# frankyeh/UNet-Studio

Hardware: AMD Instinct MI355X
Metric: voxels/sec 3D U-Net train step @128^3 bf16 (higher is better)
Workload: dtype bf16

## Files before the change

### include/unet_hip.h

```cpp
#ifndef UNET_HIP_H
#define UNET_HIP_H
#include <stddef.h>
#include <stdint.h>

#ifdef __cplusplus
extern "C" {
#endif

#define UNET_DTYPE_F32 0
#define UNET_DTYPE_BF16 1

#define UNET_IMPL_AUTO 0
#define UNET_IMPL_DIRECT 1

typedef struct unet_plan unet_plan;

const char* unet_last_error(void);
void unet_set_error(const char* msg);

int unet_init(int* n_devices);
int unet_device_info(int device, char* name, size_t name_len, size_t* total_mem, int* compute_units, int* gcn_arch_is_gfx950);

int unet_plan_create(const char* arch_dsl, int in_c, int out_c, int D, int H, int W, int dtype, int device, int impl,
                     unet_plan** out);
void unet_plan_destroy(unet_plan* plan);

int unet_plan_param_count(const unet_plan* plan, int* n);
int unet_plan_param_shape(const unet_plan* plan, int i, int64_t dims[5], int* ndim);
int unet_plan_param_name(const unet_plan* plan, int i, char* name, size_t name_len);
int unet_plan_param_decay(const unet_plan* plan, int i, int* decay);
int unet_plan_param_fan_in(const unet_plan* plan, int i, int64_t* fan_in, int* is_norm_weight);
int unet_plan_buffer_count(const unet_plan* plan, int* n);
int unet_plan_buffer_shape(const unet_plan* plan, int i, int64_t* numel);
int unet_plan_output_count(const unet_plan* plan, int* n);
int unet_plan_output_shape(const unet_plan* plan, int level, int64_t dims[5]);
int unet_plan_workspace_bytes(const unet_plan* plan, size_t* bytes);
int unet_plan_flops(const unet_plan* plan, double* fwd, double* bwd);
size_t unet_plan_describe(const unet_plan* plan, char* buf, size_t len);

int unet_plan_op_count(const unet_plan* plan, int* n);
int unet_plan_op_info(const unet_plan* plan, int i, int* kind, int* cin, int* cout, int* ks, int* stride, int64_t in_dims[3],
                      int64_t out_dims[3], char* name, size_t name_len);

#define UNET_PROF_CONV_FWD 0
#define UNET_PROF_DGRAD 1
#define UNET_PROF_WGRAD 2
#define UNET_PROF_NORM_FWD 3
#define UNET_PROF_NORM_BWD 4
#define UNET_PROF_OTHER 5
int unet_profile_begin(void);
int unet_profile_end(int max_records, int* op_index, int* category, float* ms, int* n_records);

#define UNET_MODE_PACKS_CURRENT 2
int unet_forward(const unet_plan* plan, const float* const* params, float* const* buffers, const float* x,
                 float* const* outs, void* workspace, int mode, void* stream);

int unet_backward(const unet_plan* plan, const float* const* params, const float* const* grad_outs,
                  float* const* grad_params, float* grad_x, void* workspace, void* stream);

int unet_plan_backward_buckets(const unet_plan* plan, int max_buckets, int* n_buckets, int* op_lo, int64_t* elem_lo);
int unet_backward_part(const unet_plan* plan, const float* const* params, const float* const* grad_outs, float* const* grad_params,
                       float* grad_x, void* workspace, int op_hi, int op_lo, void* stream);

int unet_loss_scratch_bytes(const unet_plan* plan, size_t* bytes);
int unet_loss(const unet_plan* plan, const float* const* outs, const int64_t* target, int cost_mask, int collapse_before,
              float* const* grad_outs, float* losses_out, void* scratch, void* stream);

int unet_forward_loss(const unet_plan* plan, const float* const* params, float* const* buffers, const float* x, float* const* outs,
                      const int64_t* target, int cost_mask, int collapse_before, float* const* grad_outs, float* losses_out,
                      void* loss_scratch, void* workspace, void* stream);
int unet_forward_loss_mode(const unet_plan* plan, const float* const* params, float* const* buffers, const float* x, float* const* outs,
                           const int64_t* target, int cost_mask, int collapse_before, float* const* grad_outs, float* losses_out,
                           void* loss_scratch, void* workspace, int mode, void* stream);

int unet_stream_create_cu_range(int device, int cu_first, int cu_count, void** stream);
int unet_stream_destroy(void* stream);
int unet_plan_side_cu_range(unet_plan* plan, int cu_first, int cu_count);

int unet_pack_filters(const unet_plan* plan, const float* const* params, void* workspace, int with_dgrad, int* made, void* stream);

#define UNET_SUM_MAX_BUFFERS 64
int unet_sum_buffers(const float* const* bufs, int n, float* out, int64_t count, int zero_inputs, void* stream);

int unet_sgd_step(const unet_plan* plan, float* params_flat, float* grads_flat, float* momentum_flat, float lr,
                  float momentum, int nesterov, float weight_decay, float clip_norm, float grad_scale, float* norm_out,
                  void* scratch, void* stream);

int unet_sgd_step_packed(const unet_plan* plan, float* params_flat, float* grads_flat, float* momentum_flat, float lr,
                         float momentum, int nesterov, float weight_decay, float clip_norm, float grad_scale, float* norm_out,
                         void* workspace, int with_dgrad, int* made, void* scratch, void* stream);

int unet_op_scratch_bytes(int cin, int cout, int D, int H, int W, size_t* bytes);
int unet_op_conv_choice(int dtype, int impl, int cin, int cout, int D, int H, int W, int ks, int stride, int transposed, int out[3]);
int unet_op_conv3d_fwd(int dtype, int impl, const void* x, const float* w, const float* b, void* y, int cin, int cout, int D,
                       int H, int W, int ks, int stride, void* scratch, void* stream);
int unet_op_conv3d_fwd_fused(int dtype, int impl, const void* x, const float* scale, const float* shift, int act, const float* w,
                             const float* b, void* y, float* stats, int cin, int cout, int D, int H, int W, int ks, int stride,
                             void* scratch, void* stream);
int unet_op_conv3d_pack(int dtype, const float* w, void* wpacked, int cin, int cout, int D, int H, int W, int ks, int stride,
                        void* stream);
int unet_op_conv3d_fwd_packed(int dtype, const void* x, const void* wpacked, const float* b, void* y, float* stats_partials,
                              int cin, int cout, int D, int H, int W, int ks, int stride, void* stream);
int unet_op_conv3d_bwd_data(int dtype, int impl, const void* dy, const float* w, void* dx, int cin, int cout, int D, int H,
                            int W, int ks, int stride, void* scratch, void* stream);
int unet_op_conv3d_fwd_norm(const void* x0, const void* x1, int cin0, int cin1, const float* w, const float* b, const float* gamma,
                            const float* beta, double eps, float* rm, float* rv, double momentum, int use_running, int act, void* y,
                            void* y_act, float* stat, int cout, int D, int H, int W, int stride, void* scratch, void* stream);
int unet_op_conv3d_bwd_data_norm(int transposed, const void* dy, const float* w, void* dx, int accumulate, const void* u, const float* stat,
                                 const float* gamma, int act, float* coef, float* dgamma, float* dbeta, int cin, int cout, int D, int H,
                                 int W, void* scratch, void* stream);
int unet_op_conv3d_bwd_weight(int dtype, int impl, const void* x, const void* dy, float* dw, float* db, int cin, int cout,
                              int D, int H, int W, int ks, int stride, void* scratch, void* stream);
int unet_op_convt_fwd(int dtype, int impl, const void* x, const float* w, const float* b, void* y, int cin, int cout, int D,
                      int H, int W, void* scratch, void* stream);
int unet_op_convt_bwd_data(int dtype, int impl, const void* dy, const float* w, void* dx, int cin, int cout, int D, int H,
                           int W, void* scratch, void* stream);
int unet_op_convt_bwd_weight(int dtype, int impl, const void* x, const void* dy, float* dw, float* db, int cin, int cout,
                             int D, int H, int W, void* scratch, void* stream);
int unet_op_pack_ndhwc(int dtype, const float* x_ncdhw, void* y_ndhwc, int C, int64_t S, void* stream);
int unet_op_unpack_ncdhw(int dtype, const void* x_ndhwc, float* y_ncdhw, int C, int64_t S, void* stream);

#define UNET_COMM_ID_BYTES 128
typedef struct unet_comm unet_comm;
int unet_comm_unique_id(void* id_bytes );
int unet_comm_create(int rank, int world, const void* id_bytes, int device, unet_comm** out);
int unet_comm_create_all(int n, const int* devices, unet_comm** out );
int unet_comm_destroy(unet_comm* comm);
int unet_comm_rank(const unet_comm* comm, int* rank, int* world);
int unet_allreduce_grads(unet_comm* comm, float* flat, int64_t elem_lo, int64_t elem_hi, void* stream);
int unet_allreduce_grads_all(unet_comm* const* comms, int n, float* const* flats, int64_t elem_lo, int64_t elem_hi, void* const* streams);
int unet_comm_broadcast(unet_comm* comm, float* buf, int64_t n, int root, void* stream);
int unet_comm_join(unet_comm* comm, void* stream);

#ifdef __cplusplus
}
#endif
#endif
```

### unet-studio_amd/csrc/conv_select.h

```cpp
#pragma once
#include "kernels.h"

namespace unet {

enum class Fwd : unsigned char { deep, mfma, head, first_mfma, first_f32_mfma, f32_mfma, direct };
enum class Dgrad : unsigned char { mfma, f32_mfma, direct };
enum class Wgrad : unsigned char { first_mfma, mfma, f32_mfma, small, direct };

struct ConvChoice {
    Fwd fwd = Fwd::direct;
    Dgrad dgrad = Dgrad::direct;
    Wgrad wgrad = Wgrad::direct;
    bool mfma_fwd() const { return fwd == Fwd::deep || fwd == Fwd::mfma; }
};

inline ConvChoice choose_conv(int dtype, int impl, const ConvGeom& g, const SrcDesc* src, int nsrc, bool is_head, bool transposed) {
    ConvChoice c;
    if (impl != UNET_IMPL_AUTO) return c;
    if (transposed) {
        if (mfma_convt_supported(dtype, g, src, nsrc)) c.fwd = Fwd::mfma, c.dgrad = Dgrad::mfma;
        else if (convt_f32_mfma_supported(dtype, g, src, nsrc)) c.fwd = Fwd::f32_mfma;
        if (mfma_convt_wgrad_supported(dtype, g, src, nsrc)) c.wgrad = Wgrad::mfma;
        return c;
    }
    if (is_head) { if (head_supported(g, nsrc)) c.fwd = Fwd::head; }
    else if (mfma_conv_fwd_supported(dtype, g, src, nsrc))
        c.fwd = deep_conv_applies(dtype, (int64_t)g.Do * g.Ho * g.Wo, g.Cin, g.Cout) ? Fwd::deep : Fwd::mfma;
    else if (conv_first_mfma_supported(dtype, g, src, nsrc)) c.fwd = Fwd::first_mfma;
    else if (conv_first_f32_mfma_supported(dtype, g, src, nsrc)) c.fwd = Fwd::first_f32_mfma;
    else if (conv_f32_mfma_supported(dtype, g, src, nsrc)) c.fwd = Fwd::f32_mfma;

    DstGrad dst[2];
    for (int k = 0; k < nsrc; ++k) dst[k].C = src[k].C;
    if (!is_head && mfma_conv_dgrad_supported(dtype, g, src, nsrc)) c.dgrad = Dgrad::mfma;
    else if (conv_f32_mfma_dgrad_supported(dtype, g, dst, nsrc)) c.dgrad = Dgrad::f32_mfma;

    if (conv_first_wgrad_mfma_supported(dtype, g, src, nsrc)) c.wgrad = Wgrad::first_mfma;
    else if (mfma_wgrad_supported(dtype, g, src, nsrc)) c.wgrad = Wgrad::mfma;
    else if (wgrad_f32_mfma_supported(dtype, g, src, nsrc)) c.wgrad = Wgrad::f32_mfma;
    else if (wgrad_small_supported(g, nsrc)) c.wgrad = Wgrad::small;
    return c;
}

}
```

### unet-studio_amd/csrc/engine.cpp

```cpp
#include <hip/hip_runtime.h>

#include <algorithm>
#include <atomic>
#include <cmath>
#include <cstdio>
#include <cstring>
#include <functional>
#include <stdexcept>
#include <string>
#include <mutex>
#include <random>
#include <unordered_map>
#include <vector>

#include "../../include/unet_hip.h"
#include "conv_select.h"
#include "graph.hpp"
#include "kernels.h"

using namespace unet;

namespace {

thread_local std::string g_err;
// ... 153 lines not shown
                if (op.src[k] != (int)t) continue;
                if (conv[i].fwd != Fwd::head) return false;
                ++readers;
            }
        }
        return readers > 0;
    }
    void layout() {
        choose_polite();
        conv.assign(g.ops.size(), ConvChoice());
        for (size_t i = 0; i < g.ops.size(); ++i) {
            const Op& op = g.ops[i];
            if (op.kind != OP_CONV && op.kind != OP_CONVT) continue;
            SrcDesc sd[2];
            src_chans(op, sd);
            conv[i] = choose_conv(dtype, impl, op_geom_of(op), sd, op.nsrc, op.out_level >= 0, op.kind == OP_CONVT);
        }
        size_t off = 0;
        auto take = [&](size_t bytes) { size_t o = off; off = align_up(off + bytes); return o; };
        t_off.assign(g.tensors.size(), SIZE_MAX);
        g_off.assign(g.tensors.size(), SIZE_MAX);
        n_consumers.assign(g.tensors.size(), 0);
        first_consumer.assign(g.tensors.size(), -1);
        for (size_t oi = 0; oi < g.ops.size(); ++oi) {
            const Op& op = g.ops[oi];
            for (int k = 0; k < op.nsrc && op.kind != OP_NORM; ++k)
                if (op.src[k] >= 0) { ++n_consumers[op.src[k]]; if (first_consumer[op.src[k]] < 0) first_consumer[op.src[k]] = (int)oi; }
        }
        a_off.assign(g.tensors.size(), SIZE_MAX);
        for (size_t i = 0; i < g.tensors.size(); ++i) {
            t_off[i] = take((size_t)g.tensors[i].numel() * elsize);
            if (g.tensors[i].needs_grad) g_off[i] = take((size_t)g.tensors[i].numel() * elsize);
            if (impl == UNET_IMPL_AUTO && (g.tensors[i].norm >= 0 || g.tensors[i].act != ACT_NONE) && !head_only(i))
                a_off[i] = take((size_t)g.tensors[i].numel() * elsize);
        }
        n_stat.resize(g.norms.size()); n_coef.resize(g.norms.size());
        size_t pmax = 0;
        for (size_t i = 0; i < g.norms.size(); ++i) {
            n_stat[i] = take(4 * (size_t)g.norms[i].C * 4);
            n_coef[i] = take(3 * (size_t)g.norms[i].C * 4);
            size_t pb = (size_t)stats_blocks(g.tensors[g.norms[i].tensor].voxels()) * g.norms[i].C * 2 * (dtype == UNET_DTYPE_F32 ? 8 : 4);
            if (pb > pmax) pmax = pb;
        }
        w_fwd.assign(g.ops.size(), SIZE_MAX); w_dgrad.assign(g.ops.size(), SIZE_MAX);
        wm_fwd.assign(g.ops.size(), SIZE_MAX); wm_dgrad.assign(g.ops.size(), SIZE_MAX);
        auto grow = [](size_t& m, size_t b) { if (b > m) m = b; };
        for (size_t i = 0; i < g.ops.size(); ++i) {
            const Op& op = g.ops[i];
            if (op.kind != OP_CONV && op.kind != OP_CONVT) continue;
            const ConvChoice& c = conv[i];
            const ConvGeom cg = op_geom_of(op);
            int k3 = op.kind == OP_CONV ? op.ks * op.ks * op.ks : 8;
            w_fwd[i] = take((size_t)k3 * op.cin * round_up(op.cout, 8) * 4);
            w_dgrad[i] = take((size_t)k3 * op.cout * round_up(op.cin, 8) * 4);
            if (op.kind == OP_CONVT) {
                if (c.mfma_fwd()) { wm_fwd[i] = take(mfma_convt_w_bytes(cg)); wm_dgrad[i] = take(mfma_convt_dgrad_w_bytes(cg)); }
                continue;
            }
            const bool stats = g.tensors[op.dst].norm >= 0;
            SrcDesc sd[2];
            src_chans(op, sd);
            if (c.mfma_fwd()) {
                wm_fwd[i] = take(mfma_conv_w_bytes(cg));
                if (stats) grow(pmax, (size_t)mfma_conv_blocks(cg) * op.cout * 2 * 4);
            }
            if (c.fwd == Fwd::first_f32_mfma && stats) grow(pmax, (size_t)conv_first_f32_mfma_blocks(cg) * op.cout * 2 * 8);
            if (c.fwd == Fwd::f32_mfma && stats) grow(pmax, (size_t)conv_f32_mfma_stat_rows(cg, sd) * op.cout * 2 * 8);
            if (c.dgrad == Dgrad::mfma) {
                wm_dgrad[i] = take(mfma_conv_dgrad_w_bytes(cg));
                if (op.stride == 2) grow(pmax, (size_t)s2_conv_dgrad_rows_max() * op.cin * 2 * 4);
            }
        }
        partial_bytes = pmax ? pmax : 256;
        partial_off = take(partial_bytes);
        size_t wmax = 0, hmax = 0;
        for (size_t i = 0; i < g.ops.size(); ++i) {
            const Op& op = g.ops[i];
            if (op.kind != OP_CONV && op.kind != OP_CONVT) continue;
            const ConvChoice& c = conv[i];
            const ConvGeom cg = op_geom_of(op);
            grow(wmax, wgrad_direct_scratch_bytes(cg, op.kind == OP_CONVT));
            if (op.kind == OP_CONVT) {
                if (c.wgrad == Wgrad::mfma) {
                    grow(wmax, mfma_convt_wgrad_scratch_bytes(cg));
                    grow(wmax, bias_grad_scratch_bytes(cg.Cout, (int64_t)cg.Do * cg.Ho * cg.Wo));
                }
                continue;
            }
            if (c.wgrad == Wgrad::mfma) grow(wmax, mfma_wgrad_scratch_bytes(cg, side_polite[i]));
            if (c.wgrad == Wgrad::f32_mfma) grow(wmax, wgrad_f32_mfma_scratch_bytes(cg));
            if (wgrad_small_supported(cg, op.nsrc)) grow(wmax, wgrad_small_scratch_bytes(cg));
            if (cg.Cin == 1 && (cg.Cout == 16 || cg.Cout == 32)) grow(wmax, conv_first_wgrad_mfma_scratch_bytes(cg));
            if (head_supported(cg, op.nsrc)) grow(hmax, head_bwd_scratch_bytes(cg));
        }
        wgrad_off = take(wmax ? wmax : 256);
        head_off = take(hmax ? hmax : 256);
        if (dtype == UNET_DTYPE_BF16 && impl == UNET_IMPL_AUTO) {
            deep_part_bytes = (size_t)8 << 20;
            deep_part_off = take(deep_part_bytes);
            deep_cnt_off = take((size_t)deep_ncnt * 4);
        }
        head_op_off.assign(g.ops.size(), SIZE_MAX);
        for (size_t i = 0; i < g.ops.size(); ++i)
            if (conv[i].fwd == Fwd::head) head_op_off[i] = take(head_bwd_scratch_bytes(op_geom_of(g.ops[i])));
        wz_off.assign(g.ops.size(), SIZE_MAX);
        for (size_t i = 0; i < g.ops.size(); ++i) {
            const Op& op = g.ops[i];
            const Wgrad w = conv[i].wgrad;
            if (op.out_level >= 0 || (w != Wgrad::first_mfma && w != Wgrad::mfma)) continue;
            const ConvGeom cg = op_geom_of(op);
            if (w == Wgrad::first_mfma) wz_off[i] = take(conv_first_wgrad_mfma_scratch_bytes(cg));
            else if (op.kind == OP_CONV) { if (!mfma_conv_wgrad_direct(cg)) wz_off[i] = take(mfma_wgrad_scratch_bytes(cg, side_polite[i])); }
            else if (!mfma_convt_wgrad_direct(cg)) wz_off[i] = take(mfma_convt_wgrad_scratch_bytes(cg));
        }
        ws_bytes = off;
        p_off.assign(g.params.size() + 1, 0);
        for (size_t i = 0; i < g.params.size(); ++i) {
            int64_t n = 1;
            for (auto d : g.params[i].shape) n *= d;
            p_off[i + 1] = p_off[i] + n;
        }
        wz_jobs.clear();
        wz_job_of_op.assign(g.ops.size(), -1);
        int wz_blk = 0;
        for (size_t i = 0; i < g.ops.size(); ++i) {
            if (wz_off[i] == SIZE_MAX) continue;
            const Op& op = g.ops[i];
            ConvGeom cg = op_geom_of(op);
            WgradReduceJob j;
            j.op = (int)i;
            j.slab_off = (long long)(wz_off[i] / 4);
            j.dw_off = p_off[op.weight];
            j.Cb = op.cout;
            if (op.kind == OP_CONVT) {
                j.nsplit = mfma_convt_wgrad_splits(cg);
                j.n = (long long)8 * op.cin * op.cout;
                j.bias_off = op.bias >= 0 ? j.slab_off + (long long)j.nsplit * j.n : -1;
                j.db_off = op.bias >= 0 ? p_off[op.bias] : -1;
            } else {
                j.nsplit = conv[i].wgrad == Wgrad::first_mfma ? conv_first_wgrad_splits(cg) : mfma_conv_wgrad_splits(cg, side_polite[i]);
                j.n = (long long)27 * op.cin * op.cout;
                j.bias_off = op.bias >= 0 ? j.slab_off + (long long)j.nsplit * j.n : -1;
                j.db_off = op.bias >= 0 ? p_off[op.bias] : -1;
            }
            wz_blk += wgrad_reduce_job_blocks(j, wz_blk);
            wz_job_of_op[i] = (int)wz_jobs.size();
            wz_jobs.push_back(j);
        }
        pack_jobs.clear();
        pack_blocks = 0;
        pack_split_op = -1; pack_split_blocks = 0; pack_fwd_blocks = 0;
        for (int which = 0; which < 2; ++which) {
            for (size_t i = 0; i < g.ops.size(); ++i) {
                const Op& op = g.ops[i];
                if (!conv[i].mfma_fwd()) continue;
                if (which == 0 && pack_split_op < 0 && g.tensors[op.dst].voxels() <= (int64_t)16 * 16 * 16) { pack_split_op = (int)i; pack_split_blocks = pack_blocks; }
                PackJob jb[2];
                int n = op.kind == OP_CONV ? mfma_conv_pack_jobs(op_geom_of(op), conv[i].dgrad == Dgrad::mfma, jb) : mfma_convt_pack_jobs(op_geom_of(op), jb);
                if (which >= n) continue;
                jb[which].src_off = p_off[op.weight];
                jb[which].dst_off = (int64_t)(which == 0 ? wm_fwd[i] : wm_dgrad[i]);
                jb[which].blk0 = pack_blocks;
                pack_blocks += jb[which].total;
                pack_jobs.push_back(jb[which]);
            }
            if (which == 0) pack_fwd_blocks = pack_blocks;
        }
        build_sgd_tiles();
    }

    void build_sgd_tiles() {
        sgd_tiles.clear();
        if (pack_jobs.empty()) return;
        const size_t np = g.params.size();
        std::vector<int> jf(np, -1), jd(np, -1), d0(np, 0), d1(np, 0), taps(np, 0);
        {
            size_t j = 0;
            for (int which = 0; which < 2; ++which)
                for (size_t i = 0; i < g.ops.size(); ++i) {
                    const Op& op = g.ops[i];
                    if (!conv[i].mfma_fwd()) continue;
                    const bool convt = op.kind != OP_CONV;
                    if (which >= (convt ? 2 : (conv[i].dgrad == Dgrad::mfma ? 2 : 1))) continue;
                    const ConvGeom cg = op_geom_of(op);
                    int& slot = which == 0 ? jf[op.weight] : jd[op.weight];
                    if (j >= pack_jobs.size() || pack_jobs[j].src_off != p_off[op.weight] || slot >= 0) return;
                    slot = (int)j++;
                    d0[op.weight] = convt ? cg.Cin : cg.Cout; d1[op.weight] = convt ? cg.Cout : cg.Cin; taps[op.weight] = convt ? 8 : 27;
                }
            if (j != pack_jobs.size()) return;
        }
        std::vector<int64_t> units(pack_jobs.size(), 0);
        bool ok = true;
        for (size_t i = 0; i < np && ok; ++i) {
            SgdTile t{};
            t.wd = g.params[i].decay ? 1.f : 0.f;
            t.job_fwd = jf[i]; t.job_dgrad = jd[i];
            const int64_t n = p_off[i + 1] - p_off[i];
            if (jf[i] < 0) {
                if (jd[i] >= 0) { ok = false; break; }
                constexpr int64_t chunk = 8192;
                for (int64_t o = 0; o < n; o += chunk) { t.off = p_off[i] + o; t.count = std::min(chunk, n - o); sgd_tiles.push_back(t); }
                continue;
            }
            if ((int64_t)d0[i] * d1[i] * taps[i] != n) { ok = false; break; }
            t.off = p_off[i]; t.D1 = d1[i]; t.T = taps[i];
            for (int a = 0; a < d0[i] && ok; a += SGD_TILE_MAX)
                for (int b = 0; b < d1[i] && ok; b += SGD_TILE_MAX) {
                    t.d0 = a; t.n0 = std::min(SGD_TILE_MAX, d0[i] - a); t.d1 = b; t.n1 = std::min(SGD_TILE_MAX, d1[i] - b);
                    t.count = (int64_t)t.n0 * t.n1 * t.T;
                    for (int j : {jf[i], jd[i]}) {
                        if (j < 0) continue;
                        const int64_t u = sgd_tile_units(t, pack_jobs[j]);
                        if (u < 0) ok = false; else units[j] += u;
                    }
                    sgd_tiles.push_back(t);
                }
        }
// ... 662 lines not shown

int unet_backward(const unet_plan* p, const float* const* params, const float* const* grad_outs, float* const* grad_params,
                  float* grad_x, void* workspace, void* stream) {
    try {
        if (!p || !params || !grad_params || !workspace) throw std::runtime_error("unet_backward: null argument");
        if (grad_x) throw std::runtime_error("unet_backward: grad_x must be NULL -- dL/dx is not computed (the input carries no gradient, as in train.cpp:619-628)");
        DeviceGuard dg(p->device);
        Exec ex(*p, workspace, stream);
        ex.backward(params, grad_outs, grad_params, grad_x);
        check_launch();
        return 0;
    } catch (const std::exception& e) { return fail(e.what()); }
}

int unet_backward_part(const unet_plan* p, const float* const* params, const float* const* grad_outs, float* const* grad_params,
                       float* grad_x, void* workspace, int op_hi, int op_lo, void* stream) {
    try {
        if (!p || !params || !grad_params || !workspace) throw std::runtime_error("unet_backward_part: null argument");
        if (op_lo < 0 || op_hi < op_lo) throw std::runtime_error("unet_backward_part: invalid op range");
        if (grad_x) throw std::runtime_error("unet_backward_part: grad_x must be NULL -- dL/dx is not computed");
        DeviceGuard dg(p->device);
        Exec ex(*p, workspace, stream);
        ex.backward(params, grad_outs, grad_params, grad_x, op_hi, op_lo);
        check_launch();
        return 0;
    } catch (const std::exception& e) { return fail(e.what()); }
}

int unet_plan_backward_buckets(const unet_plan* p, int max_buckets, int* n_buckets, int* op_lo, int64_t* elem_lo) {
    try {
        if (!p || !n_buckets || !op_lo || !elem_lo || max_buckets < 1) throw std::runtime_error("unet_plan_backward_buckets: bad argument");
        const Graph& g = p->g;
        const int nops = (int)g.ops.size();
        std::vector<int64_t> first(nops, INT64_MAX);
        bool monotone = true;
        int64_t prev = -1;
        for (int i = 0; i < nops; ++i) {
            const Op& op = g.ops[i];
            if (op.kind != OP_CONV && op.kind != OP_CONVT) continue;
            int64_t f = p->p_off[op.weight];
            if (op.bias >= 0 && p->p_off[op.bias] < f) f = p->p_off[op.bias];
            first[i] = f;
            if (f <= prev) monotone = false;
            prev = f;
            const Tensor& T = g.tensors[op.dst];
            if (T.norm >= 0) {
                const Norm& n = g.norms[T.norm];
                if (p->p_off[n.gamma] < f || p->p_off[n.beta] < f) monotone = false;
            }
        }
        int nb = 0;
        if (monotone && max_buckets > 1) {
            const double thr = (double)p->n_param_elems / ((double)max_buckets - 0.5);
            int64_t hi = p->n_param_elems;
            for (int i = nops - 1; i > 0 && nb < max_buckets - 1; --i) {
                if (first[i] == INT64_MAX) continue;
                if ((double)(hi - first[i]) >= thr) { op_lo[nb] = i; elem_lo[nb] = first[i]; hi = first[i]; ++nb; }
            }
        }
        op_lo[nb] = 0; elem_lo[nb] = 0; ++nb;
        *n_buckets = nb;
        return 0;
    } catch (const std::exception& e) { return fail(e.what()); }
}

int unet_plan_op_count(const unet_plan* p, int* n) { *n = (int)p->g.ops.size(); return 0; }
int unet_plan_op_info(const unet_plan* p, int i, int* kind, int* cin, int* cout, int* ks, int* stride, int64_t in_dims[3],
                      int64_t out_dims[3], char* name, size_t name_len) {
    if (i < 0 || i >= (int)p->g.ops.size()) return fail("op index out of range");
    const Op& op = p->g.ops[i];
    if (kind) *kind = (int)op.kind;
    if (cin) *cin = op.cin;
    if (cout) *cout = op.cout;
    if (ks) *ks = op.ks;
    if (stride) *stride = op.stride;
    const Tensor* a = op.nsrc > 0 && op.src[0] >= 0 ? &p->g.tensors[op.src[0]] : nullptr;
    const Tensor* o = op.dst >= 0 ? &p->g.tensors[op.dst] : nullptr;
    if (in_dims) { in_dims[0] = a ? a->D : 0; in_dims[1] = a ? a->H : 0; in_dims[2] = a ? a->W : 0; }
    if (out_dims) { out_dims[0] = o ? o->D : 0; out_dims[1] = o ? o->H : 0; out_dims[2] = o ? o->W : 0; }
    if (name && name_len) { std::strncpy(name, op.name.c_str(), name_len - 1); name[name_len - 1] = 0; }
    return 0;
}

int unet_profile_begin(void) {
    if (g_prof) return fail("unet_profile_begin: a profile is already open on this thread");
    g_prof = new ProfSink();
    return 0;
}
int unet_profile_end(int max_records, int* op_index, int* category, float* ms, int* n_records) {
    if (!g_prof) return fail("unet_profile_end: no open profile on this thread");
    ProfSink* ps = g_prof;
    g_prof = nullptr;
    int n = 0, rc = 0;
    for (auto& r : ps->recs) {
        float t = 0.f;
        hipError_t e = hipEventSynchronize(r.e1);
        if (e == hipSuccess) e = hipEventElapsedTime(&t, r.e0, r.e1);
        if (e != hipSuccess) rc = fail(std::string("unet_profile_end: ") + hipGetErrorString(e));
        if (r.op != -2 && n < max_records && op_index && category && ms) { op_index[n] = r.op; category[n] = r.cat; ms[n] = t; ++n; }
        (void)hipEventDestroy(r.e0); (void)hipEventDestroy(r.e1);
    }
    if (n_records) *n_records = n;
    delete ps;
    return rc;
}

int unet_loss_scratch_bytes(const unet_plan* p, size_t* bytes) { *bytes = p->loss_bytes; return 0; }

namespace {
struct LossRun {
    const unet_plan* p;
    const float* const* outs; const int64_t* target; float* const* grad_outs; float* losses_out;
    int C, oc, collapse, cost_mask;
    float inv;
    std::vector<int64_t*> tgt;
    std::vector<float*> lvl;
    float* partial[2];
    LossRun(const unet_plan* plan, const float* const* outs_, const int64_t* target_, int cost_mask_, int collapse_before, float* const* grad_outs_,
            float* losses_out_, void* scratch)
        : p(plan), outs(outs_), target(target_), grad_outs(grad_outs_), losses_out(losses_out_), collapse(collapse_before), cost_mask(cost_mask_) {
        if (!p || !outs || !target || !losses_out || !scratch) throw std::runtime_error("unet_loss: null argument");
        const Graph& g = p->g;
        C = g.out_c;
        if (collapse_before < 0 || collapse_before >= C) throw std::runtime_error("invalid collapse_before");
        oc = collapse_before ? C - collapse_before + 1 : C;
        const size_t nl = g.outputs.size();
        float wsum = 0.f;
        for (size_t k = 0; k < nl; ++k) wsum += 1.0f / (float)(1 << k);
        inv = 1.0f / wsum;
        char* sc = (char*)scratch;
        size_t off = 0;
        tgt.resize(nl); lvl.resize(nl);
        for (size_t l = 0; l < nl; ++l) {
            int64_t S = (int64_t)(g.D >> l) * (g.H >> l) * (g.W >> l);
            if (S <= 0) S = 1;
            tgt[l] = (int64_t*)(sc + off); off = align_up(off + (size_t)S * 8);
            lvl[l] = (float*)(sc + off); off = align_up(off + (size_t)(4 + 2 * C) * 4);
        }
        partial[0] = (float*)(sc + off); off = align_up(off + (size_t)1024 * (3 + 2 * C) * 4);
        partial[1] = (float*)(sc + off);
        int D = g.D, H = g.H, W = g.W;
        for (size_t k = 0; k < nl; ++k) {
            if (k > 0) {
                if ((D >> 1) <= 0 || (H >> 1) <= 0 || (W >> 1) <= 0) throw std::runtime_error("deep supervision target size became zero");
                D >>= 1; H >>= 1; W >>= 1;
            }
            const auto& o = g.outputs[k];
            if (o.C == 0 || !outs[k]) throw std::runtime_error("undefined deep supervision output at level " + std::to_string(k));
            if (o.C != C)
                throw std::runtime_error("output channel mismatch at level " + std::to_string(k) + ": tensor has " + std::to_string(o.C) +
                                         ", out_count is " + std::to_string(C));
            if (o.D != D || o.H != H || o.W != W) throw std::runtime_error("deep supervision output/target size mismatch at level " + std::to_string(k));
        }
    }
    size_t levels() const { return p->g.outputs.size(); }
    const int64_t* target_of(size_t k) const { return k == 0 ? target : tgt[k]; }
    int64_t voxels(size_t k) const { const auto& o = p->g.outputs[k]; return (int64_t)o.D * o.H * o.W; }
    void prepare(hipStream_t s) {
        HIP_OK(hipMemsetAsync(losses_out, 0, 4 * sizeof(float), s));
        const Graph& g = p->g;
        int D = g.D, H = g.H, W = g.W;
        for (size_t k = 1; k < levels(); ++k) {
            launch_target_half(target_of(k - 1), tgt[k], D, H, W, s);
            D >>= 1; H >>= 1; W >>= 1;
        }
    }
// ... 136 lines not shown
        if (!bufs || !out || n < 1 || n > UNET_SUM_MAX_BUFFERS || count < 0) throw std::runtime_error("unet_sum_buffers: bad argument");
        for (int k = 0; k < n; ++k)
            if (!bufs[k] || (reinterpret_cast<uintptr_t>(bufs[k]) & 15)) throw std::runtime_error("unet_sum_buffers: null or misaligned buffer");
        if (reinterpret_cast<uintptr_t>(out) & 15) throw std::runtime_error("unet_sum_buffers: misaligned output");
        if (count == 0) return 0;
        launch_sum_buffers(bufs, n, out, count, zero_inputs, (hipStream_t)stream);
        check_launch();
        return 0;
    } catch (const std::exception& e) { return fail(e.what()); }
}

int unet_sgd_step(const unet_plan* p, float* params, float* grads, float* mom, float lr, float momentum, int nesterov, float wd,
                  float clip_norm, float grad_scale, float* norm_out, void* scratch, void* stream) {
    try {
        if (!p || !params || !grads || !mom || !scratch) throw std::runtime_error("unet_sgd_step: null argument");
        if (!p->segs_dev) throw std::runtime_error("unet_sgd_step: plan was created without a device");
        DeviceGuard dg(p->device);
        hipStream_t s = (hipStream_t)stream;
        const int nblk = 1024;
        float* partial = (float*)scratch;
        launch_sumsq_partial(grads, p->n_param_elems, grad_scale, partial, nblk, s);
        launch_sgd(params, grads, mom, p->n_param_elems, p->segs_dev, p->nseg, partial, nblk, lr, momentum, nesterov, wd, clip_norm,
                   grad_scale, norm_out, s);
        check_launch();
        return 0;
    } catch (const std::exception& e) { return fail(e.what()); }
}

int unet_sgd_step_packed(const unet_plan* p, float* params, float* grads, float* mom, float lr, float momentum, int nesterov, float wd,
                         float clip_norm, float grad_scale, float* norm_out, void* workspace, int with_dgrad, int* made, void* scratch,
                         void* stream) {
    try {
        if (!p || !params || !grads || !mom || !scratch || !made) throw std::runtime_error("unet_sgd_step_packed: null argument");
        *made = 0;
        if (!p->tiles_dev || !p->jobs_dev || !workspace)
            return unet_sgd_step(p, params, grads, mom, lr, momentum, nesterov, wd, clip_norm, grad_scale, norm_out, scratch, stream);
        if ((reinterpret_cast<uintptr_t>(params) | reinterpret_cast<uintptr_t>(grads) | reinterpret_cast<uintptr_t>(mom)) & 15)
            throw std::runtime_error("unet_sgd_step_packed: misaligned buffer");
        DeviceGuard dg(p->device);
        hipStream_t s = (hipStream_t)stream;
        const int nblk = 1024;
        float* partial = (float*)scratch;
        launch_sumsq_partial(grads, p->n_param_elems, grad_scale, partial, nblk, s);
        launch_sgd_pack(params, grads, mom, p->tiles_dev, (int)p->sgd_tiles.size(), p->jobs_dev, workspace, with_dgrad,
                        p->deep_part_bytes ? (int*)((char*)workspace + p->deep_cnt_off) : nullptr, p->deep_ncnt, partial, nblk, lr, momentum,
                        nesterov, wd, clip_norm, grad_scale, norm_out, s);
        check_launch();
        *made = 1;
        return 0;
    } catch (const std::exception& e) { return fail(e.what()); }
}

struct OpScratch {
    size_t half, pack, partials;
    OpScratch(int cin, int cout)
        : half(align_up((size_t)27 * round_up(cin, 8) * round_up(cout, 8) * 4)), pack(2 * half),
          partials(pack + align_up((size_t)160 * round_up(cin, 32) * round_up(cout, 32))) {}
};
int unet_op_scratch_bytes(int cin, int cout, int D, int H, int W, size_t* bytes) {
    size_t b = OpScratch(cin, cout).partials + 4096;
    if (D > 0 && H > 0 && W > 0) {
        int64_t S = (int64_t)D * H * W;
        size_t blocks = (size_t)(S / 32 + 4096);
        b += align_up(blocks * cout * 2 * 8);
    }
    if ((int64_t)cin * cout <= 1024) {
        size_t w = ((size_t)1024 * 1024 + (size_t)1024 * cout) * 4 + 1024;
        if (w > b) b = w;
    }
    if (cout <= 8 || cin == 1) {
        size_t w = (size_t)512 * ((size_t)27 * cin * cout + cout) * 4 + 1024;
        if (w > b) b = w;
    }
    if (cin % 16 == 0 && cout % 16 == 0 && D > 0 && H > 0 && W > 0) {
        ConvGeom g;
        g.Cin = cin; g.Cout = cout; g.D = g.Do = D; g.H = g.Ho = H; g.W = g.Wo = W; g.ks = 3; g.stride = 1;
        b = std::max(b, wgrad_f32_mfma_scratch_bytes(g));
        size_t w = std::max(mfma_wgrad_scratch_bytes(g, 0), mfma_wgrad_scratch_bytes(g, 1));
        if (w > b) b = w;
        g.stride = 2; g.Do = (D - 1) / 2 + 1; g.Ho = (H - 1) / 2 + 1; g.Wo = (W - 1) / 2 + 1;
        w = std::max(mfma_wgrad_scratch_bytes(g, 0), mfma_wgrad_scratch_bytes(g, 1));
        if (w > b) b = w;
        g.Do = 2 * D; g.Ho = 2 * H; g.Wo = 2 * W;
        w = mfma_convt_wgrad_scratch_bytes(g);
        if (w > b) b = w;
    }
    *bytes = b;
    return 0;
}

static ConvGeom op_geom(int cin, int cout, int D, int H, int W, int ks, int stride, bool transposed) {
    ConvGeom g;
    g.Cin = cin; g.Cout = cout; g.D = D; g.H = H; g.W = W; g.ks = ks; g.stride = stride;
    if (transposed) { g.Do = 2 * D; g.Ho = 2 * H; g.Wo = 2 * W; }
    else {
        int pad = (ks - 1) / 2;
        g.Do = (D + 2 * pad - ks) / stride + 1; g.Ho = (H + 2 * pad - ks) / stride + 1; g.Wo = (W + 2 * pad - ks) / stride + 1;
    }
    return g;
}
static void op_pack(const float* w, int cin, int cout, int k3, bool transposed, void* scratch, float** wf, float** wd, hipStream_t s) {
    *wf = (float*)scratch; *wd = (float*)((char*)scratch + OpScratch(cin, cout).half);
    if (transposed) launch_pack_convt_w(w, *wf, *wd, cin, cout, s);
    else launch_pack_conv_w(w, *wf, *wd, cin, cout, k3, s);
}
#define OP_TRY(...) try { __VA_ARGS__; check_launch(); return 0; } catch (const std::exception& e) { return fail(e.what()); }
static DeepScratch op_deep() {
    static std::mutex mu;
    static std::unordered_map<int, DeepScratch> per_dev;
    int dev = 0;
    HIP_OK(hipGetDevice(&dev));
    std::lock_guard<std::mutex> lk(mu);
    auto it = per_dev.find(dev);
    if (it != per_dev.end()) return it->second;
    DeepScratch d;
    d.part_bytes = (size_t)8 << 20; d.ncnt = 4096;
    char* base = nullptr;
    HIP_OK(hipMalloc((void**)&base, d.part_bytes + (size_t)d.ncnt * 4));
    HIP_OK(hipMemset(base + d.part_bytes, 0, (size_t)d.ncnt * 4));
    d.part = (float*)base; d.cnt = (int*)(base + d.part_bytes);
    per_dev[dev] = d;
    return d;
}

int unet_op_conv_choice(int dtype, int impl, int cin, int cout, int D, int H, int W, int ks, int stride, int transposed, int out[3]) {
    try {
        if (!out) throw std::runtime_error("unet_op_conv_choice: null output");
        if (cin < 1 || cout < 1 || D < 1 || H < 1 || W < 1) throw std::runtime_error("unet_op_conv_choice: sizes must be positive");
        const ConvGeom g = transposed ? op_geom(cin, cout, D, H, W, 2, 2, true) : op_geom(cin, cout, D, H, W, ks, stride, false);
        SrcDesc sd; sd.C = cin;
        const ConvChoice c = choose_conv(dtype, impl, g, &sd, 1, false, transposed != 0);
        out[0] = (int)c.fwd; out[1] = (int)c.dgrad; out[2] = (int)c.wgrad;
        return 0;
    } catch (const std::exception& e) { return fail(e.what()); }
}

int unet_op_conv3d_fwd(int dtype, int impl, const void* x, const float* w, const float* b, void* y, int cin, int cout, int D, int H,
                       int W, int ks, int stride, void* scratch, void* stream) {
    OP_TRY({
        hipStream_t s = (hipStream_t)stream;
        ConvGeom g = op_geom(cin, cout, D, H, W, ks, stride, false);
        float *wf, *wd;
        SrcDesc sd; sd.ptr = x; sd.C = cin;
        const ConvChoice c = choose_conv(dtype, impl, g, &sd, 1, false, false);
        if (c.mfma_fwd()) {
            void* wm = (char*)scratch + OpScratch(cin, cout).pack;
            launch_mfma_pack_conv_w(w, wm, nullptr, g, s);
            if (!launch_deep_conv_fwd(g, &sd, 1, wm, b, y, nullptr, op_deep(), s)) launch_mfma_conv_fwd(g, &sd, 1, wm, b, y, nullptr, s);
        } else if (c.fwd == Fwd::first_mfma) {
            launch_conv_first_mfma(g, &sd, w, b, y, nullptr, s);
        } else if (c.fwd == Fwd::first_f32_mfma) {
            (void)launch_conv_first_f32_mfma(g, &sd, w, b, (float*)y, nullptr, s);
        } else {
            op_pack(w, cin, cout, ks * ks * ks, false, scratch, &wf, &wd, s);
            if (c.fwd == Fwd::f32_mfma) (void)launch_conv_f32_mfma(g, &sd, 1, wf, b, (float*)y, s);
            else launch_conv_fwd_direct(dtype, g, &sd, 1, wf, b, y, nullptr, s);
        }
    })
}
int unet_op_conv3d_fwd_fused(int dtype, int impl, const void* x, const float* scale, const float* shift, int act, const float* w,
                             const float* b, void* y, float* stats, int cin, int cout, int D, int H, int W, int ks, int stride,
                             void* scratch, void* stream) {
    OP_TRY({
        hipStream_t s = (hipStream_t)stream;
        ConvGeom g = op_geom(cin, cout, D, H, W, ks, stride, false);
        float *wf, *wd;
        SrcDesc sd; sd.ptr = x; sd.C = cin; sd.scale = scale; sd.shift = shift; sd.act = act;
// ... 44 lines not shown
        launch_mfma_conv_fwd(g, &sd, 1, wpacked, b, y, stats_partials, (hipStream_t)stream);
    })
}
int unet_op_conv3d_bwd_data(int dtype, int impl, const void* dy, const float* w, void* dx, int cin, int cout, int D, int H, int W,
                            int ks, int stride, void* scratch, void* stream) {
    OP_TRY({
        hipStream_t s = (hipStream_t)stream;
        ConvGeom g = op_geom(cin, cout, D, H, W, ks, stride, false);
        float *wf, *wd;
        DstGrad d; d.ptr = dx; d.C = cin; d.accumulate = 0;
        SrcDesc sd; sd.C = cin;
        const Dgrad c = choose_conv(dtype, impl, g, &sd, 1, false, false).dgrad;
        if (c == Dgrad::mfma) {
            void* wm = (char*)scratch + OpScratch(cin, cout).pack;
            launch_mfma_pack_conv_w(w, nullptr, wm, g, s);
            mfma_dgrad(g, false, dy, wm, &d, 1, nullptr, nullptr, op_deep(), s);
        } else {
            op_pack(w, cin, cout, ks * ks * ks, false, scratch, &wf, &wd, s);
            if (c == Dgrad::f32_mfma) launch_conv_f32_mfma_dgrad(g, (const float*)dy, wd, &d, 1, s);
            else launch_conv_dgrad_direct(dtype, g, dy, wd, &d, 1, s);
        }
    })
}
int unet_op_conv3d_fwd_norm(const void* x0, const void* x1, int cin0, int cin1, const float* w, const float* b, const float* gamma,
                            const float* beta, double eps, float* rm, float* rv, double momentum, int use_running, int act, void* y,
                            void* y_act, float* stat, int cout, int D, int H, int W, int stride, void* scratch, void* stream) {
    OP_TRY({
        hipStream_t s = (hipStream_t)stream;
        const int cin = cin0 + cin1, nsrc = x1 ? 2 : 1;
        ConvGeom g = op_geom(cin, cout, D, H, W, 3, stride, false);
        SrcDesc sd[2];
        sd[0].ptr = x0; sd[0].C = cin0;
        if (x1) { sd[1].ptr = x1; sd[1].C = cin1; }
        const ConvChoice c = choose_conv(UNET_DTYPE_BF16, UNET_IMPL_AUTO, g, sd, nsrc, false, false);
        if (!c.mfma_fwd() || (use_running && (!rm || !rv)))
            throw std::runtime_error("unet_op_conv3d_fwd_norm: shape not covered by the MFMA kernels, or eval mode without running statistics");
        const OpScratch L(cin, cout);
        void* wm = (char*)scratch + L.pack;
        float* part = (float*)((char*)scratch + L.partials);
        launch_mfma_pack_conv_w(w, wm, nullptr, g, s);
        const DeepNormFwd nf = {gamma, beta, eps, stat, rm, rv, momentum, use_running ? 1 : 0, act, y_act};
        if (!(c.fwd == Fwd::deep && launch_deep_conv_fwd(g, sd, nsrc, wm, b, y, &nf, op_deep(), s))) {
            const int rows = launch_mfma_conv_fwd(g, sd, nsrc, wm, b, y, use_running ? nullptr : part, s);
            norm_fwd_passes(UNET_DTYPE_BF16, y, cout, (int64_t)g.Do * g.Ho * g.Wo, part, rows, false, use_running != 0, gamma, beta, eps,
                            stat, rm, rv, act, y_act, s);
        }
    })
}
int unet_op_conv3d_bwd_data_norm(int transposed, const void* dy, const float* w, void* dx, int accumulate, const void* u, const float* stat,
                                 const float* gamma, int act, float* coef, float* dgamma, float* dbeta, int cin, int cout, int D, int H,
                                 int W, void* scratch, void* stream) {
    OP_TRY({
        hipStream_t s = (hipStream_t)stream;
        ConvGeom g = op_geom(cin, cout, D, H, W, transposed ? 2 : 3, transposed ? 2 : 1, transposed != 0);
        SrcDesc sd; sd.C = cin;
        if (choose_conv(UNET_DTYPE_BF16, UNET_IMPL_AUTO, g, &sd, 1, false, transposed != 0).dgrad != Dgrad::mfma)
            throw std::runtime_error("unet_op_conv3d_bwd_data_norm: shape not covered by the MFMA kernels");
        const OpScratch L(cin, cout);
        void* wm = (char*)scratch + L.pack;
        float* part = (float*)((char*)scratch + L.partials);
        DstGrad d; d.ptr = dx; d.C = cin; d.accumulate = accumulate ? 1 : 0;
        const DeepNormBwd nb = {u, stat, gamma, coef, dgamma, dbeta, act};
        if (transposed) launch_mfma_pack_convt_w(w, nullptr, wm, g, s);
        else launch_mfma_pack_conv_w(w, nullptr, wm, g, s);
        const DgradOutcome o = mfma_dgrad(g, transposed != 0, dy, wm, &d, 1, &nb, part, op_deep(), s);
        if (!o.norm_done) norm_bwd_passes(UNET_DTYPE_BF16, dx, u, cin, (int64_t)D * H * W, stat, act, gamma, coef, dgamma, dbeta, part, o.rows, false, s);
    })
}
int unet_op_conv3d_bwd_weight(int dtype, int impl, const void* x, const void* dy, float* dw, float* db, int cin, int cout, int D,
                              int H, int W, int ks, int stride, void* scratch, void* stream) {
    OP_TRY({
        hipStream_t s = (hipStream_t)stream;
        ConvGeom g = op_geom(cin, cout, D, H, W, ks, stride, false);
        SrcDesc sd; sd.ptr = x; sd.C = cin;
        switch (choose_conv(dtype, impl, g, &sd, 1, false, false).wgrad) {
            case Wgrad::first_mfma: launch_conv_first_wgrad_mfma(g, &sd, dy, dw, db, scratch, s); break;
            case Wgrad::mfma: launch_mfma_conv_wgrad(g, &sd, 1, dy, dw, db, scratch, s, false, env().op_polite ? 1 : 0); break;
            case Wgrad::f32_mfma: launch_wgrad_f32_mfma(g, &sd, 1, (const float*)dy, dw, db, scratch, s); break;
            case Wgrad::small: launch_conv_wgrad_small(dtype, g, &sd, 1, dy, dw, db, scratch, s); break;
            case Wgrad::direct: launch_conv_wgrad_direct(dtype, g, &sd, 1, dy, dw, db, nullptr, s);
        }
    })
}
int unet_op_convt_fwd(int dtype, int impl, const void* x, const float* w, const float* b, void* y, int cin, int cout, int D, int H,
                      int W, void* scratch, void* stream) {
    OP_TRY({
        hipStream_t s = (hipStream_t)stream;
        ConvGeom g = op_geom(cin, cout, D, H, W, 2, 2, true);
        float *wf, *wd;
        SrcDesc sd; sd.ptr = x; sd.C = cin;
        const Fwd f = choose_conv(dtype, impl, g, &sd, 1, false, true).fwd;
        if (f == Fwd::mfma) {
            void* wm = (char*)scratch + OpScratch(cin, cout).pack;
            launch_mfma_pack_convt_w(w, wm, nullptr, g, s);
            if (!launch_deep_convt_fwd(g, &sd, 1, wm, b, y, op_deep(), s)) launch_mfma_convt_fwd(g, &sd, 1, wm, b, y, s);
        } else {
            op_pack(w, cin, cout, 8, true, scratch, &wf, &wd, s);
            if (f == Fwd::f32_mfma) launch_convt_f32_mfma(g, &sd, wf, b, (float*)y, s);
            else launch_convt_fwd_direct(dtype, g, &sd, 1, wf, b, y, s);
        }
    })
}
int unet_op_convt_bwd_data(int dtype, int impl, const void* dy, const float* w, void* dx, int cin, int cout, int D, int H, int W,
                           void* scratch, void* stream) {
    OP_TRY({
        hipStream_t s = (hipStream_t)stream;
        ConvGeom g = op_geom(cin, cout, D, H, W, 2, 2, true);
        float *wf, *wd;
        DstGrad d; d.ptr = dx; d.C = cin; d.accumulate = 0;
        SrcDesc sd; sd.C = cin;
        if (choose_conv(dtype, impl, g, &sd, 1, false, true).dgrad == Dgrad::mfma) {
            void* wm = (char*)scratch + OpScratch(cin, cout).pack;
            launch_mfma_pack_convt_w(w, nullptr, wm, g, s);
            mfma_dgrad(g, true, dy, wm, &d, 1, nullptr, nullptr, op_deep(), s);
        } else {
            op_pack(w, cin, cout, 8, true, scratch, &wf, &wd, s);
            launch_convt_dgrad_direct(dtype, g, dy, wd, &d, 1, s);
        }
    })
}
int unet_op_convt_bwd_weight(int dtype, int impl, const void* x, const void* dy, float* dw, float* db, int cin, int cout, int D, int H,
                             int W, void* scratch, void* stream) {
    OP_TRY({
        ConvGeom g = op_geom(cin, cout, D, H, W, 2, 2, true);
        SrcDesc sd; sd.ptr = x; sd.C = cin;
        if (choose_conv(dtype, impl, g, &sd, 1, false, true).wgrad == Wgrad::mfma)
            launch_mfma_convt_wgrad(g, &sd, dy, dw, scratch, (hipStream_t)stream, false, db);
        else
            launch_convt_wgrad_direct(dtype, g, &sd, 1, dy, dw, db, nullptr, (hipStream_t)stream);
    })
}
int unet_op_pack_ndhwc(int dtype, const float* x, void* y, int C, int64_t S, void* stream) {
    OP_TRY({ launch_pack_input(dtype, x, y, C, S, (hipStream_t)stream); })
}
int unet_op_unpack_ncdhw(int dtype, const void* x, float* y, int C, int64_t S, void* stream) {
    OP_TRY({ launch_unpack_ncdhw(dtype, x, y, C, S, (hipStream_t)stream); })
}


static const char* augment_recipe_error(const UnetAugmentRecipe* r) {
    if (!r) return "unet_augment: null recipe";
    for (int d = 0; d < 3; ++d)
        if (r->dims[d] < 1) return "unet_augment: dims must be positive";
    if (r->channels < 1 || r->channels > UNET_AUG_MAX_CHANNELS) return "unet_augment: channels out of range (1..UNET_AUG_MAX_CHANNELS)";
    if (r->n_foci < 0 || r->n_foci > UNET_AUG_MAX_FOCI) return "unet_augment: n_foci out of range (0..UNET_AUG_MAX_FOCI)";
    if (r->trunc_top < 0 || r->trunc_bottom < 0) return "unet_augment: negative truncation";
    if (r->downsample)
        for (int d = 0; d < 3; ++d)
            if (r->low_dims[d] < 1 || r->low_dims[d] > r->dims[d]) return "unet_augment: low_dims must be in 1..dims";
    for (int k = 0; k < r->n_foci; ++k)
        if (!(r->foci_radius[k] > 0.f)) return "unet_augment: distortion radius must be positive";
    return nullptr;
}
int unet_augment_scratch_bytes(const UnetAugmentRecipe* recipe, size_t* bytes) {
    if (const char* e = augment_recipe_error(recipe)) return fail(e);
    if (!bytes) return fail("unet_augment_scratch_bytes: null output");
    *bytes = augment_scratch_bytes(*recipe);
    return 0;
}
int unet_augment_run(const UnetAugmentRecipe* recipe, float* image, float* label, void* scratch, size_t scratch_bytes, void* stream) {
    if (const char* e = augment_recipe_error(recipe)) return fail(e);
    if (!image || !label || !scratch) return fail("unet_augment_run: null device pointer");
    if (scratch_bytes < augment_scratch_bytes(*recipe)) return fail("unet_augment_run: scratch too small (see unet_augment_scratch_bytes)");
    OP_TRY({
        hipPointerAttribute_t at;
        HIP_OK(hipPointerGetAttributes(&at, image));
        DeviceGuard guard(at.device);
        launch_augment(*recipe, image, label, scratch, (hipStream_t)stream);
    })
}

static const char* simulate_recipe_error(const UnetSimulateRecipe* r) {
    if (!r) return "unet_simulate_modality: null recipe";
    for (int d = 0; d < 3; ++d)
        if (r->dims[d] < 1) return "unet_simulate_modality: dims must be positive";
    if (r->with_label && (r->max_label < 0 || r->max_label >= UNET_SIM_MAX_LABELS)) return "unet_simulate_modality: max_label out of range";
    for (int k = 0; k < UNET_SIM_TERMS; ++k)
        if (r->term_a[k] > 3 || r->term_b[k] > 3 || r->term_c[k] > 3 || r->term_d[k] > 3) return "unet_simulate_modality: exponents must be 0..3";
    return nullptr;
}
int unet_simulate_modality_scratch_bytes(const UnetSimulateRecipe* recipe, size_t* bytes) {
    if (const char* e = simulate_recipe_error(recipe)) return fail(e);
    if (!bytes) return fail("unet_simulate_modality_scratch_bytes: null output");
    *bytes = simulate_scratch_bytes(*recipe);
    return 0;
}
int unet_simulate_modality_run(const UnetSimulateRecipe* recipe, float* t1w, const float* label, void* scratch, size_t scratch_bytes,
                               void* stream) {
    if (const char* e = simulate_recipe_error(recipe)) return fail(e);
    if (!t1w || !scratch || (recipe->with_label && !label)) return fail("unet_simulate_modality_run: null device pointer");
    if (scratch_bytes < simulate_scratch_bytes(*recipe)) return fail("unet_simulate_modality_run: scratch too small");
    OP_TRY({
        hipPointerAttribute_t at;
        HIP_OK(hipPointerGetAttributes(&at, t1w));
        DeviceGuard guard(at.device);
        launch_simulate_modality(*recipe, t1w, label, scratch, (hipStream_t)stream);
    })
}

static const char* qc_args_error(int out_c, int64_t voxels, int collapse_before) {
    if (out_c < 1) return "unet_qc: out_c must be positive";
    if (collapse_before < 0 || collapse_before >= out_c) return "invalid collapse_before";
    if (voxels <= 0) return "unet_qc: voxels must be positive";
    if (voxels > ((int64_t)1 << 40)) return "unet_qc: too many voxels";
    return nullptr;
}
int unet_qc_scratch_bytes(int out_c, int64_t voxels, int collapse_before, size_t* bytes) {
    if (const char* e = qc_args_error(out_c, voxels, collapse_before)) return fail(e);
    if (!bytes) return fail("unet_qc_scratch_bytes: null output");
    *bytes = qc_scratch_bytes(out_c, voxels, collapse_before);
// ... 983 lines not shown
```

### unet-studio_amd/csrc/kernels.h

```cpp
#pragma once
#include <hip/hip_runtime.h>
#include <cstdint>

#include "../../include/unet_atlas.h"
#include "../../include/unet_augment.h"
#include "../../include/unet_components.h"
#include "../../include/unet_connectivity.h"
#include "../../include/unet_distance.h"
#include "../../include/unet_ensemble.h"
#include "../../include/unet_feed.h"
#include "../../include/unet_hip.h"
#include "../../include/unet_instances.h"
#include "../../include/unet_morph.h"
#include "../../include/unet_postproc.h"
#include "../../include/unet_preproc.h"
#include "../../include/unet_qc.h"
#include "../../include/unet_register.h"
#include "../../include/unet_space.h"
#include "../../include/unet_stats.h"
#include "../../include/unet_table.h"
#include "../../include/unet_mirror.h"
#include "../../include/unet_tiles.h"

namespace unet {
// ... 41 lines not shown
void launch_convt_wgrad_direct(int dtype, const ConvGeom& g, const SrcDesc* src, int nsrc, const void* dy, float* dw, float* db,
                               void* scratch, hipStream_t s);

int stats_blocks(int64_t S);
void launch_stats_partial(int dtype, const void* x, int C, int64_t S, float* partial, hipStream_t s);
void launch_norm_finalize(const float* partial, int nblk, int C, int64_t S, const float* gamma, const float* beta, double eps,
                          float* stat, float* running_mean, float* running_var, double momentum, hipStream_t s, bool dbl = false);
void launch_stats_sum(const float* partial, int nblk, int C, float* out, hipStream_t s, bool dbl = false);
void launch_norm_eval(int C, const float* gamma, const float* beta, const float* rm, const float* rv, double eps, float* stat,
                      hipStream_t s);

void launch_act_bwd(int dtype, void* g, const void* u, int act, int64_t n, hipStream_t s);
void launch_norm_bwd_partial(int dtype, void* g, const void* u, int C, int64_t S, const float* stat, int act, float* partial,
                             hipStream_t s);
void launch_norm_bwd_finalize(const float* partial, int nblk, int C, int64_t S, const float* gamma, const float* stat, float* coef,
                              float* dgamma, float* dbeta, hipStream_t s, bool dbl = false);
bool launch_norm_finalize_apply(int dtype, const float* partial, int nblk, int C, int64_t S, const float* gamma, const float* beta, double eps,
                                float* stat, float* running_mean, float* running_var, double momentum, const void* raw, int act, void* out,
                                hipStream_t s);
bool launch_norm_bwd_finalize_apply(int dtype, const float* partial, int nblk, int C, int64_t S, const float* gamma, const float* stat,
                                    float* coef, float* dgamma, float* dbeta, void* g, const void* u, int act, hipStream_t s);
void launch_norm_bwd_apply(int dtype, void* g, const void* u, int C, int64_t S, const float* stat, const float* coef, int act,
                           hipStream_t s);

void launch_maxpool_fwd(int dtype, SrcDesc src, void* out, int D, int H, int W, hipStream_t s);
void launch_maxpool_bwd(int dtype, SrcDesc src, const void* gout, DstGrad dst, int D, int H, int W, hipStream_t s);
void launch_upsample_fwd(int dtype, SrcDesc src, void* out, int D, int H, int W, hipStream_t s);
void launch_upsample_bwd(int dtype, const void* gout, DstGrad dst, int D, int H, int W, hipStream_t s);
void launch_materialize(int dtype, const SrcDesc* src, int nsrc, void* out, int64_t S, hipStream_t s);
void launch_apply_view(int dtype, SrcDesc src, void* out, int64_t S, hipStream_t s);
void launch_materialize_bwd(int dtype, const void* gout, const DstGrad* dst, int ndst, int64_t S, hipStream_t s);
void launch_export_bwd(int dtype, const float* g_ncdhw, DstGrad dst, int64_t S, hipStream_t s);
void launch_unpack_ncdhw(int dtype, const void* g, float* out_ncdhw, int C, int64_t S, hipStream_t s);

void launch_target_half(const int64_t* t, int64_t* o, int D, int H, int W, hipStream_t s);
int loss_blocks(int64_t S);
void launch_loss_partial(const float* logits, const int64_t* target, int C, int64_t S, int collapse, float* partial, hipStream_t s);
void launch_loss_finalize(const float* partial, int nblk, int oc, float level_weight, int cost_mask, float* level_out, float* totals,
                          int set_stats, hipStream_t s);
void launch_loss_grad(const float* logits, const int64_t* target, int C, int64_t S, int collapse, const float* level_out,
                      float level_weight, int cost_mask, float* dlogits, hipStream_t s);

void launch_sum_buffers(const float* const* bufs, int n, float* out, int64_t count, int zero_inputs, hipStream_t s);

struct SgdSeg { int64_t offset, count; float wd; };
void launch_sumsq_partial(const float* g, int64_t n, float scale, float* partial, int nblk, hipStream_t s);
void launch_sgd(float* p, float* g, float* m, int64_t n, const SgdSeg* segs_dev, int nseg, const float* partial, int nblk,
                float lr, float momentum, int nesterov, float weight_decay, float clip_norm, float grad_scale, float* norm_out,
                hipStream_t s);

struct PackJob;
struct SgdTile { int64_t off, count; float wd; int job_fwd, job_dgrad, D1, T, d0, n0, d1, n1, pad; };
constexpr int SGD_TILE_MAX = 32;
int64_t sgd_tile_units(const SgdTile& t, const PackJob& job);
void launch_sgd_pack(float* p, float* g, float* m, const SgdTile* tiles_dev, int ntiles, const PackJob* jobs_dev, void* ws, int with_dgrad,
                     int* zero, int nzero, const float* partial, int nblk, float lr, float momentum, int nesterov, float weight_decay,
                     float clip_norm, float grad_scale, float* norm_out, hipStream_t s);

struct PackJob { int64_t src_off, dst_off, total, blk0; int Ci, Co, CK, T, mode, A, B, pad; };
enum PackMode {
    PK_CONV_FWD = 0,
    PK_CONV_DGRAD = 1,
    PK_CONVT_DGRAD = 2,
    PK_CONVT_FWD = 3,
    PK_CONV_S2_DGRAD = 4
};
int mfma_conv_pack_jobs(const ConvGeom& g, bool want_dgrad, PackJob* out2);
int mfma_convt_pack_jobs(const ConvGeom& g, PackJob* out2);
void launch_mfma_pack_batched(const float* params_base, void* ws, const PackJob* jobs_dev, int njobs, int64_t nblocks, hipStream_t s,
                              int64_t blk_base = 0, int max_grid = 0, int* zero = nullptr, int nzero = 0);
bool mfma_conv_fwd_supported(int dtype, const ConvGeom& g, const SrcDesc* src, int nsrc);
size_t mfma_conv_w_bytes(const ConvGeom& g);
void launch_mfma_pack_conv_w(const float* w, void* w_mfma_fwd, void* w_mfma_dgrad, const ConvGeom& g, hipStream_t s);
int launch_mfma_conv_fwd(const ConvGeom& g, const SrcDesc* src, int nsrc, const void* w_mfma, const float* bias, void* out,
                         float* stats_partial, hipStream_t s);
bool conv_first_mfma_supported(int dtype, const ConvGeom& g, const SrcDesc* src, int nsrc);
int conv_first_mfma_blocks(const ConvGeom& g);
int launch_conv_first_mfma(const ConvGeom& g, const SrcDesc* src, const float* w, const float* bias, void* out, float* stats_partial,
                           hipStream_t s);
int mfma_conv_blocks(const ConvGeom& g);
bool mfma_wgrad_z_supported(int dtype, const ConvGeom& g, const SrcDesc* src, int nsrc);
size_t mfma_wgrad_z_scratch_bytes(const ConvGeom& g, int polite = 0);
int mfma_wgrad_z_splits(const ConvGeom& g, int polite = 0);
int launch_mfma_wgrad_z(const ConvGeom& g, const SrcDesc* src, int nsrc, const void* dy, bool want_bias, void* scratch, hipStream_t s,
                        int polite = 0);
void wgrad_reduce(const float* slab, const float* bias_slab, int nsplit, int64_t n, int Cb, float* dw, float* db, hipStream_t s);
struct WgradReduceJob { long long slab_off, bias_off, dw_off, db_off, n; int nsplit, Cb, ly, blk0, nblk, op; };
int wgrad_reduce_job_blocks(WgradReduceJob& j, int blk0);
void launch_wgrad_reduce_batched(const WgradReduceJob* jobs_dev, int job0, int njobs, int blk_base, int nblocks, const void* ws, float* gflat,
                                 hipStream_t s);
bool mfma_wgrad_supported(int dtype, const ConvGeom& g, const SrcDesc* src, int nsrc);
size_t mfma_wgrad_scratch_bytes(const ConvGeom& g, int polite = 0);
int mfma_conv_wgrad_splits(const ConvGeom& g, int polite = 0);
int mfma_convt_wgrad_splits(const ConvGeom& g);
bool mfma_conv_wgrad_direct(const ConvGeom& g);
bool mfma_convt_wgrad_direct(const ConvGeom& g);
int conv_first_wgrad_splits(const ConvGeom& g);
void launch_mfma_conv_wgrad(const ConvGeom& g, const SrcDesc* src, int nsrc, const void* dy, float* dw, float* db, void* scratch,
                            hipStream_t s, bool defer_reduce = false, int polite = 0);
bool head_supported(const ConvGeom& g, int nsrc);
size_t head_bwd_scratch_bytes(const ConvGeom& g);
void launch_head_fwd(int dtype, const ConvGeom& g, const SrcDesc& src, const float* w, const float* bias, void* y, float* out_ncdhw,
                     hipStream_t s);
void launch_head_bwd(int dtype, const ConvGeom& g, const SrcDesc& src, const float* dy_ncdhw, const void* dy_cl, const float* w,
                     DstGrad dst, float* dw, float* db, void* scratch, hipStream_t s, bool defer_reduce = false);
void launch_head_bwd_reduce(const ConvGeom& g, float* dw, float* db, const void* scratch, hipStream_t s);
bool conv_first_wgrad_mfma_supported(int dtype, const ConvGeom& g, const SrcDesc* src, int nsrc);
size_t conv_first_wgrad_mfma_scratch_bytes(const ConvGeom& g);
struct NormBwdFuse { const void* u; const float* stat; const float* coef; int act; };
void launch_conv_first_wgrad_mfma(const ConvGeom& g, const SrcDesc* src, const void* dy, float* dw, float* db, void* scratch, hipStream_t s,
                                  bool defer_reduce = false, const NormBwdFuse* nb_fuse = nullptr);
bool wgrad_small_supported(const ConvGeom& g, int nsrc);
size_t wgrad_small_scratch_bytes(const ConvGeom& g);
void launch_conv_wgrad_small(int dtype, const ConvGeom& g, const SrcDesc* src, int nsrc, const void* dy, float* dw, float* db,
                             void* scratch, hipStream_t s);
bool mfma_convt_wgrad_supported(int dtype, const ConvGeom& g, const SrcDesc* src, int nsrc);
size_t mfma_convt_wgrad_scratch_bytes(const ConvGeom& g);
void launch_mfma_convt_wgrad(const ConvGeom& g, const SrcDesc* src, const void* dy, float* dw, void* scratch, hipStream_t s,
                             bool defer_reduce = false, float* db = nullptr, int polite = 0);
int launch_colsum_partial8(int dtype, const void* x, int C, int64_t S, float* partial, hipStream_t s);
size_t bias_grad_scratch_bytes(int C, int64_t S);
void launch_bias_grad(int dtype, const void* dy, int C, int64_t S, float* db, void* scratch, hipStream_t s);
bool mfma_conv_dgrad_supported(int dtype, const ConvGeom& g, const SrcDesc* src, int nsrc);
size_t mfma_conv_dgrad_w_bytes(const ConvGeom& g);
struct DgradOutcome {
    bool served = false;
    bool norm_done = false;
    int rows = 0;
    bool operator==(const DgradOutcome& o) const { return served == o.served && norm_done == o.norm_done && rows == o.rows; }
};
struct BnBwdStats { const void* u; const float* stat; float* partial; int act, C; };
DgradOutcome mfma_conv_dgrad_outcome(const ConvGeom& g, const DstGrad* dst, int ndst, bool norm);
DgradOutcome launch_mfma_conv_dgrad(const ConvGeom& g, const void* dy, const void* w_mfma_dgrad, const DstGrad* dst, int ndst, hipStream_t s,
                                    const BnBwdStats* bn = nullptr);
int launch_s2_conv_fwd(const ConvGeom& g, const SrcDesc* src, int nsrc, const void* w_mfma, const float* bias, void* out, float* stats_partial,
                       hipStream_t s);
DgradOutcome s2_conv_dgrad_outcome(const ConvGeom& g, const DstGrad* dst, int ndst, bool norm);
DgradOutcome launch_s2_conv_dgrad(const ConvGeom& g, const void* dy, const void* w_s2_dgrad, const DstGrad* dst, int ndst, hipStream_t s,
                                  const BnBwdStats* bn);
int s2_conv_dgrad_rows_max();
bool launch_s2_convt_fwd(const ConvGeom& g, const SrcDesc* src, int nsrc, const void* w_mfma, const float* bias, void* out, hipStream_t s);
bool launch_s2_convt_dgrad(const ConvGeom& g, const void* dy, const void* w_mfma_dgrad, const DstGrad* dst, int ndst, hipStream_t s);
int s2_wgrad_splits(int Ca, int Cb, int cD, int cH, int cW);
int launch_s2_wgrad(int ks, const void* fine, const void* fine2, int C0, int Ca, int fD, int fH, int fW, const void* coarse, int Cb, int cD, int cH,
                    int cW, bool want_bias, int bias_from_a, void* scratch, hipStream_t s, int polite);
constexpr int64_t DEEP_MAX_VOXELS = 512;
struct DeepScratch { float* part = nullptr; size_t part_bytes = 0; int* cnt = nullptr; int ncnt = 0; };
struct DeepNormFwd {
    const float* gamma; const float* beta; double eps; float* stat; float* rm; float* rv; double momentum; int use_running; int act;
    void* act_out;
};
struct DeepNormBwd {
    const void* u; const float* stat; const float* gamma; float* coef; float* dgamma; float* dbeta; int act;
};
bool deep_conv_applies(int dtype, int64_t out_voxels, int cin, int cout);
bool launch_deep_conv_fwd(const ConvGeom& g, const SrcDesc* src, int nsrc, const void* w_mfma, const float* bias, void* out,
                          const DeepNormFwd* nf, const DeepScratch& sc, hipStream_t s);
bool launch_deep_convt_fwd(const ConvGeom& g, const SrcDesc* src, int nsrc, const void* w_mfma, const float* bias, void* out,
                           const DeepScratch& sc, hipStream_t s);
DgradOutcome deep_dgrad_outcome(const ConvGeom& g, bool transposed, const DstGrad* dst, int ndst, bool norm, const DeepScratch& sc);
DgradOutcome launch_deep_dgrad(const ConvGeom& g, bool transposed, const void* dy, const void* w_mfma_dgrad, const DstGrad* dst, int ndst,
                               const DeepNormBwd* nb, const DeepScratch& sc, hipStream_t s);
bool mfma_convt_supported(int dtype, const ConvGeom& g, const SrcDesc* src, int nsrc);
size_t mfma_convt_w_bytes(const ConvGeom& g);
size_t mfma_convt_dgrad_w_bytes(const ConvGeom& g);
void launch_mfma_pack_convt_w(const float* w, void* w_mfma_fwd, void* w_mfma_dgrad, const ConvGeom& g, hipStream_t s);
void launch_mfma_convt_fwd(const ConvGeom& g, const SrcDesc* src, int nsrc, const void* w_mfma, const float* bias, void* out, hipStream_t s);
void launch_mfma_convt_dgrad(const ConvGeom& g, const void* dy, const void* w_mfma_dgrad, const DstGrad* dst, int ndst, hipStream_t s);

bool conv_f32_mfma_supported(int dtype, const ConvGeom& g, const SrcDesc* src, int nsrc);
int conv_f32_mfma_stat_rows(const ConvGeom& g, const SrcDesc* src);
int launch_conv_f32_mfma(const ConvGeom& g, const SrcDesc* src, int nsrc, const float* w_fwd, const float* bias, float* out,
                         hipStream_t s, double* stats_partial = nullptr);
bool conv_first_f32_mfma_supported(int dtype, const ConvGeom& g, const SrcDesc* src, int nsrc);
int conv_first_f32_mfma_blocks(const ConvGeom& g);
int launch_conv_first_f32_mfma(const ConvGeom& g, const SrcDesc* src, const float* w, const float* bias, float* out, double* stats_partial,
                               hipStream_t s);
bool convt_f32_mfma_supported(int dtype, const ConvGeom& g, const SrcDesc* src, int nsrc);
void launch_convt_f32_mfma(const ConvGeom& g, const SrcDesc* src, const float* w_fwd, const float* bias, float* out, hipStream_t s);
bool wgrad_f32_mfma_supported(int dtype, const ConvGeom& g, const SrcDesc* src, int nsrc);
size_t wgrad_f32_mfma_scratch_bytes(const ConvGeom& g);
void launch_wgrad_f32_mfma(const ConvGeom& g, const SrcDesc* src, int nsrc, const float* dy, float* dw, float* db, void* scratch,
                           hipStream_t s);
void slab_reduce_public(const float* slab, int nsplit, int64_t n, float* out, hipStream_t s);
bool conv_f32_mfma_dgrad_supported(int dtype, const ConvGeom& g, const DstGrad* dst, int ndst);
void launch_conv_f32_mfma_dgrad(const ConvGeom& g, const float* dy, const float* w_dgrad, const DstGrad* dst, int ndst, hipStream_t s);

size_t augment_scratch_bytes(const UnetAugmentRecipe& r);
void launch_augment(const UnetAugmentRecipe& r, float* image, float* label, void* scratch, hipStream_t st);
size_t simulate_scratch_bytes(const UnetSimulateRecipe& r);
void launch_simulate_modality(const UnetSimulateRecipe& r, float* t1w, const float* label, void* scratch, hipStream_t st);

size_t qc_scratch_bytes(int out_c, int64_t S, int collapse);
void launch_qc_counts(const float* logits, const float* label, const float* image0, int out_c, int64_t S, int collapse, int shift,
                      uint64_t* counts, void* scratch, hipStream_t s);

size_t feed_scratch_bytes(int64_t S);
void launch_feed_label_max(const float* label, int64_t S, int* out_max, void* scratch, hipStream_t s);
void launch_feed_prepare(const float* image0, float* label, int64_t S, int normalize, int shift, int* label_max, void* scratch,
                         hipStream_t s);
void launch_feed_target(const float* label, int64_t S, int normalize, int64_t* target, void* scratch, hipStream_t s);

size_t postproc_scratch_bytes(int planes, int64_t S);
void launch_postproc_softmax(const float* logits, int C, int64_t S, float thr, float* lp, float* fg, uint16_t* lab, hipStream_t s);
void launch_postproc_argmax_planes(const float* lp, int np, int64_t S, const float* fg, float thr, uint16_t* lab, hipStream_t s);
void launch_postproc_defragment(int W, int H, int D, int each, float thr, double ratio, float* fg, float* lp, int np, uint16_t* lab,
                                void* scratch, hipStream_t s);
void launch_postproc_plane_op(int op, float t, int W, int H, int D, float* lp, int np, void* scratch, hipStream_t s);

int64_t space_bricks(int w, int h, int d);
size_t space_scratch_bytes(int64_t dst_voxels, int channels);
void launch_space_resample(const float* src, int sw, int sh, int sd, float* dst, int dw, int dh, int dd, int channels,
                           const UnetSpaceMap& map, int mode, int normalize, void* scratch, hipStream_t s);
void launch_space_postproc(const float* logits, int C, int mw, int mh, int md, const UnetSpaceMap& map, int nw, int nh, int nd, float thr,
                           float* lp, float* fg, uint16_t* lab, hipStream_t s);

void launch_tiles_blend(const float* tiles, int C, int tw, int th, int td, const UnetTilePlan& plan, int cw, int ch, int cd, float* canvas,
                        hipStream_t s);
void launch_tiles_postproc(const float* tiles, int C, int tw, int th, int td, const UnetTilePlan& plan, int cw, int ch, int cd, float thr,
                           float* lp, float* fg, uint16_t* lab, hipStream_t s);

void launch_mirror_combine(const float* stack, int C, int W, int H, int D, int n_members, const int* masks, int swap_axis, const int* pairs,
                           int n_pairs, float* mean, uint8_t* agreement, hipStream_t s);
void launch_mirror_postproc(const float* stack, int C, int W, int H, int D, int n_members, const int* masks, int swap_axis,
                            const int* pairs, int n_pairs, float thr, float* lp, float* fg, uint16_t* lab, uint8_t* agreement,
                            hipStream_t s);
// ... 87 lines not shown
```

### unet-studio_amd/csrc/kernels_mfma_s2_wgrad.hip

```cpp
#include <cstdio>
#include <cstdlib>
#include <type_traits>

#include "mfma_util.h"

namespace unet {

__device__ __attribute__((aligned(16))) unsigned g_s2w_zero[4] = {0u, 0u, 0u, 0u};

typedef __attribute__((ext_vector_type(4))) short ws16x4;
typedef __attribute__((address_space(3))) ws16x4 wlds_s16x4;
__device__ __forceinline__ bf16x8 wtr_read2(const char* p0, const char* p1) {
    ws16x4 a = __builtin_amdgcn_ds_read_tr16_b64_v4i16((wlds_s16x4*)p0);
    ws16x4 b = __builtin_amdgcn_ds_read_tr16_b64_v4i16((wlds_s16x4*)p1);
    return __builtin_bit_cast(bf16x8, __builtin_shufflevector(a, b, 0, 1, 2, 3, 4, 5, 6, 7));
}

struct S2WgradArgs {
    const void* fine;
    const void* fine2;
    int C0;
    const void* coarse;
    int Ca, Cb;
    int fD, fH, fW, cD, cH, cW;
    float* slab;
    float* bias_slab;
    int bias_from_a;
    int cols_x, cols_y, nseg, zlen;
};

#define S2W_DMA(src, dst)                                                                                                    \
    do {                                                                                                                     \
        unsigned keep_;                                                                                                      \
        asm volatile("s_mov_b32 %0, m0\n\ts_mov_b32 m0, %2\n\ts_nop 0\n\tglobal_load_lds_dwordx4 %1, off\n\ts_mov_b32 m0, %0" \
                     : "=&s"(keep_) : "v"(src), "s"(__builtin_amdgcn_readfirstlane((int)(dst))) : "memory");                      \
    } while (0)

template <int KS, int PA, int PB, int WK>
__global__ void __launch_bounds__(256, 2) k_s2_wgrad(S2WgradArgs a) {
    constexpr int T = KS * KS * KS, PAD = KS == 3 ? 1 : 0, P = PA * PB;
    static_assert(P * WK == 4, "four waves");
    constexpr int R = WK == 1 ? 2 : 1, BYC = WK * R;
    constexpr int HYF = 2 * BYC + PAD, NODD = KS == 3 ? 33 : 32, HXF = NODD + 32;
    constexpr int FVS = PA * 32, CVS = PB * 32;
    constexpr int FSLOT = HYF * HXF * FVS, CSLOT = BYC * 32 * CVS;
    constexpr int NF = KS == 3 ? 5 : 4, NC = 2;
    constexpr int FUNITS = HYF * HXF * PA * 2, CUNITS = BYC * 32 * PB * 2;
    constexpr int ITF = (FUNITS + 255) / 256, ITC = (CUNITS + 255) / 256;
    constexpr int GA = PA * 2, GB = PB * 2;
    constexpr int LDS_BYTES = NF * FSLOT + NC * CSLOT;
    extern __shared__ __attribute__((aligned(16))) char smem[];
    char* const fring = smem;
    char* const cring = smem + NF * FSLOT;

    const int tid = threadIdx.x, lane = tid & 63, il = lane & 15, gq = lane >> 4, q4 = il >> 2, p4 = il & 3;
    const int wave = __builtin_amdgcn_readfirstlane(tid >> 6), pw = wave % P, kw = wave / P, ia = pw / PB, ib = pw % PB;
    const int CBG = (a.Cb / 16) / PB;
    const int caB = ((int)blockIdx.y / CBG) * PA, cbB = ((int)blockIdx.y % CBG) * PB;
    const unsigned lds0 = (unsigned)(size_t)(__attribute__((address_space(3))) char*)smem;

    const int item = xcd_remap((int)blockIdx.x, (int)gridDim.x);
    const int ncols = a.cols_x * a.cols_y, seg = item / ncols, col = item % ncols;
    const int x0 = (col % a.cols_x) * 32, y0 = (col / a.cols_x) * BYC;
    const int zs = seg * a.zlen, ze = zs + a.zlen < a.cD ? zs + a.zlen : a.cD, len = ze - zs;

    f32x4 acc[T];
#pragma unroll
    for (int t = 0; t < T; ++t) acc[t] = f32x4{0.f, 0.f, 0.f, 0.f};
    float bsum[8];
#pragma unroll
    for (int e = 0; e < 8; ++e) bsum[e] = 0.f;
    const bool do_bias_b = a.bias_slab != nullptr && !a.bias_from_a && caB == 0;
    const bool do_bias_a = a.bias_slab != nullptr && a.bias_from_a && cbB == 0;

    unsigned foff[ITF], coff[ITC];
    unsigned fpiece[ITF], cpiece[ITC];
    const int fch = caB * 16 + (tid % GA) * 8;
    const bool f2 = a.fine2 != nullptr && fch >= a.C0;
    const char* const fptr = (const char*)(f2 ? a.fine2 : a.fine);
    const int fC = a.fine2 ? (f2 ? a.Ca - a.C0 : a.C0) : a.Ca, fc0 = f2 ? fch - a.C0 : fch;
#pragma unroll
    for (int it = 0; it < ITF; ++it) {
        const int u = it * 256 + tid, hv = u / GA, hy = hv / HXF, sl = hv % HXF;
        const int t = sl < NODD ? 2 * sl : 2 * (sl - NODD) + 1;
        const int gy = 2 * y0 - PAD + hy, gx = 2 * x0 - PAD + t;
        const bool ok = u < FUNITS && (unsigned)gy < (unsigned)a.fH && (unsigned)gx < (unsigned)a.fW;
// ... 90 lines not shown
            for (int t = 0; t < T; ++t) {
                __builtin_amdgcn_sched_barrier(0);
                acc[t] = __builtin_amdgcn_mfma_f32_16x16x32_bf16(ring[t % RD], Bf, acc[t], 0, 0, 0);
                __builtin_amdgcn_sched_barrier(0);
                if (t + RD < T) ring[t % RD] = afrag(t + RD);
            }
        }
    }
    asm volatile("s_waitcnt vmcnt(0)" ::: "memory");
    __syncthreads();

    constexpr int TCH = (P * T * 1024 <= LDS_BYTES) ? T : ((P * 9 * 1024 <= LDS_BYTES && T % 9 == 0) ? 9 : (T % 3 == 0 ? 3 : 1));
    static_assert(P * TCH * 1024 <= LDS_BYTES && T % TCH == 0, "reduction scratch");
    float* red = (float*)smem;
    if constexpr (WK > 1) {
#pragma unroll 1
        for (int kk = 1; kk < WK; ++kk) {
#pragma unroll
            for (int c0 = 0; c0 < T; c0 += TCH) {
                if (kw == kk) {
#pragma unroll
                    for (int t = 0; t < TCH; ++t) *(f32x4*)(red + ((pw * TCH + t) * 64 + lane) * 4) = acc[c0 + t];
                }
                __syncthreads();
                if (kw == 0) {
#pragma unroll
                    for (int t = 0; t < TCH; ++t) {
                        const f32x4 o = *(const f32x4*)(red + ((pw * TCH + t) * 64 + lane) * 4);
                        acc[c0 + t][0] += o[0]; acc[c0 + t][1] += o[1]; acc[c0 + t][2] += o[2]; acc[c0 + t][3] += o[3];
                    }
                }
                __syncthreads();
            }
        }
    }
    {
        constexpr int RP = 16 * T + 4;
        static_assert(16 * RP * 4 <= LDS_BYTES, "slab staging");
        float* stg = (float*)smem;
#pragma unroll 1
        for (int pr = 0; pr < P; ++pr) {
            __syncthreads();
            if (kw == 0 && pw == pr) {
#pragma unroll
                for (int t = 0; t < T; ++t)
#pragma unroll
                    for (int r = 0; r < 4; ++r) stg[il * RP + (gq * 4 + r) * T + t] = acc[t][r];
            }
            __syncthreads();
            float* base = a.slab + (size_t)blockIdx.x * T * a.Ca * a.Cb + ((size_t)(cbB + pr % PB) * 16 * a.Ca + (size_t)(caB + pr / PB) * 16) * T;
            for (int q = tid; q < 16 * 4 * T; q += 256) {
                const int row = q / (4 * T), c4 = q % (4 * T);
                *(f32x4*)(base + (size_t)row * a.Ca * T + c4 * 4) = *(const f32x4*)(stg + row * RP + c4 * 4);
            }
        }
    }
    if (do_bias_a || do_bias_b) {
        const int G = do_bias_a ? GA : GB;
#pragma unroll
        for (int e = 0; e < 8; ++e) {
            float v = bsum[e];
            for (int m = G; m < 64; m <<= 1) v += __shfl_xor(v, m);
            bsum[e] = v;
        }
        __syncthreads();
        float* bred = (float*)smem;
        if (lane < G) {
#pragma unroll
            for (int e = 0; e < 8; ++e) bred[(wave * G + lane) * 8 + e] = bsum[e];
        }
        __syncthreads();
        if (tid < G * 8) {
            const int u = tid / 8, e = tid % 8;
            float sacc = 0.f;
#pragma unroll
            for (int w = 0; w < 4; ++w) sacc += bred[(w * G + u) * 8 + e];
            const int C = do_bias_a ? a.Ca : a.Cb, tB = do_bias_a ? caB : cbB;
            a.bias_slab[(size_t)blockIdx.x * C + (tB + (u >> 1)) * 16 + (u & 1) * 8 + e] = sacc;
        }
    }
}

struct S2WCfg { int pa, pb, wk, byc, cols_x, cols_y, nseg, zlen, gx, gy; };
static bool s2w_cfg(int Ca, int Cb, int cD, int cH, int cW, S2WCfg& c) {
    if (sliding_window_off() || Ca % 16 || Cb % 16 || cW < 24 || cD < 4) return false;
    if ((size_t)(2 * cH + 1) * (2 * cW + 1) * Ca * 2 >= ((size_t)1 << 31) || (size_t)cH * cW * Cb * 2 >= ((size_t)1 << 31)) return false;
    const int cat = Ca / 16, cbt = Cb / 16;
    if (cat % 2 == 0 && cbt % 2 == 0) { c.pa = 2; c.pb = 2; c.wk = 1; }
    else if (cbt % 2 == 0) { c.pa = 1; c.pb = 2; c.wk = 2; }
    else if (cat % 2 == 0) { c.pa = 2; c.pb = 1; c.wk = 2; }
    else return false;
    c.byc = 2;
    c.cols_x = (cW + 31) / 32; c.cols_y = (cH + c.byc - 1) / c.byc;
    c.gy = (cat / c.pa) * (cbt / c.pb);
    const int cols = c.cols_x * c.cols_y;
    int want = 512 / c.gy;
    if (want < 1) want = 1;
    int nseg = (want + cols - 1) / cols;
    if (nseg < 1) nseg = 1;
    int zlen = (cD + nseg - 1) / nseg;
    if (zlen < 4) zlen = 4;
    if (zlen > cD) zlen = cD;
    c.nseg = (cD + zlen - 1) / zlen; c.zlen = zlen;
    c.gx = cols * c.nseg;
    return true;
}
int s2_wgrad_splits(int Ca, int Cb, int cD, int cH, int cW) {
    S2WCfg c;
    return s2w_cfg(Ca, Cb, cD, cH, cW, c) ? c.gx : 0;
}
template <int KS, int PA, int PB, int WK>
static void launch_s2w_t(const S2WgradArgs& a, const S2WCfg& c, hipStream_t s, int polite) {
    constexpr int PAD = KS == 3 ? 1 : 0, R = WK == 1 ? 2 : 1, BYC = WK * R, HYF = 2 * BYC + PAD, HXF = (KS == 3 ? 33 : 32) + 32;
    constexpr int lds = (KS == 3 ? 5 : 4) * HYF * HXF * PA * 32 + 2 * BYC * 32 * PB * 32;
    static_assert(BYC == 2 && lds <= 160 * 1024, "footprint / LDS");
    static std::atomic<uint64_t> attr_done{0};
    const int want = lds > 83000 ? lds : polite_lds(lds, 1);
    set_max_lds_once(attr_done, (const void*)k_s2_wgrad<KS, PA, PB, WK>, want);
    k_s2_wgrad<KS, PA, PB, WK><<<dim3((unsigned)c.gx, (unsigned)c.gy), 256, polite_lds(lds, polite), s>>>(a);
}
int launch_s2_wgrad(int ks, const void* fine, const void* fine2, int C0, int Ca, int fD, int fH, int fW, const void* coarse, int Cb, int cD, int cH,
                    int cW, bool want_bias, int bias_from_a, void* scratch, hipStream_t s, int polite) {
    S2WCfg c;
    if (!s2w_cfg(Ca, Cb, cD, cH, cW, c)) return 0;
    S2WgradArgs a;
    a.fine = fine; a.fine2 = fine2; a.C0 = C0; a.coarse = coarse; a.Ca = Ca; a.Cb = Cb; a.fD = fD; a.fH = fH; a.fW = fW; a.cD = cD; a.cH = cH; a.cW = cW;
    const int T = ks * ks * ks;
    a.slab = (float*)scratch;
    a.bias_slab = want_bias ? a.slab + (size_t)c.gx * T * Ca * Cb : nullptr;
    a.bias_from_a = bias_from_a;
    a.cols_x = c.cols_x; a.cols_y = c.cols_y; a.nseg = c.nseg; a.zlen = c.zlen;
    if (ks == 3) {
        if (c.pa == 2 && c.pb == 2) launch_s2w_t<3, 2, 2, 1>(a, c, s, polite);
        else if (c.pb == 2) launch_s2w_t<3, 1, 2, 2>(a, c, s, polite);
        else launch_s2w_t<3, 2, 1, 2>(a, c, s, polite);
    } else {
        if (c.pa == 2 && c.pb == 2) launch_s2w_t<2, 2, 2, 1>(a, c, s, polite);
        else if (c.pb == 2) launch_s2w_t<2, 1, 2, 2>(a, c, s, polite);
        else launch_s2w_t<2, 2, 1, 2>(a, c, s, polite);
    }
    return c.gx;
}

}
```

### unet-studio_amd/csrc/kernels_mfma_wgrad.hip

```cpp
#include <type_traits>
#include "mfma_util.h"

namespace unet {

typedef __attribute__((ext_vector_type(4))) short s16x4;
typedef __attribute__((address_space(3))) s16x4 lds_s16x4;

struct MfmaWgradArgs {
    ConvGeom g;
    SrcDesc asrc[2];
    int nasrc;
    SrcDesc bsrc;
    float* slab;
    float* bias_slab;
    int tiles_x, tiles_y, tiles_z;
    int direct;
    int bias_from_a;
};

__device__ __forceinline__ bf16x8 tr_read2(const char* p0, const char* p1) {
    s16x4 a = __builtin_amdgcn_ds_read_tr16_b64_v4i16((lds_s16x4*)p0);
    s16x4 b = __builtin_amdgcn_ds_read_tr16_b64_v4i16((lds_s16x4*)p1);
    return __builtin_bit_cast(bf16x8, __builtin_shufflevector(a, b, 0, 1, 2, 3, 4, 5, 6, 7));
}

template <int S, int KD, int PAD, int BZ, int BY, int BX, int PI, int PJ>
__global__ void __launch_bounds__(256, 2) k_mfma_wgrad(MfmaWgradArgs a) {
    constexpr int HZ = (BZ - 1) * S + KD, HY = (BY - 1) * S + KD, HX = (BX - 1) * S + KD;
    constexpr int NVA = HZ * HY * HX, NVB = BZ * BY * BX, T = KD * KD * KD;
    constexpr int PLANE_A = NVA * 32, PLANE_B = NVB * 32, B_OFF = PI * PLANE_A;
    constexpr int P = PI * PJ, WPP = 4 / P;
    constexpr int GPR = BX / 4;
    constexpr int KSTEPS = NVB / 32;
    static_assert(P == 1 || P == 2 || P == 4, "pairs per block");
    static_assert(NVB % 32 == 0 && BX % 4 == 0, "tile must hold whole K-steps");
    extern __shared__ __attribute__((aligned(16))) char smem[];

    const ConvGeom& g = a.g;
    const int tid = threadIdx.x, wave = tid >> 6, lane = tid & 63, il = lane & 15, gq = lane >> 4;
    const int q4 = il >> 2, p4 = il & 3;
    const int pw = wave % P, kw = wave / P;
    const int it_ = pw / PJ, jt = pw % PJ;
    const int COTB = (g.Cout / 16) / PJ;
    const int ciB = (blockIdx.y / COTB) * PI, coB = (blockIdx.y % COTB) * PJ;
    const int ntiles = a.tiles_x * a.tiles_y * a.tiles_z;
    const int C0 = a.asrc[0].C;

    constexpr bool TS = P == 1;
    constexpr int TW = (T + 3) / 4, NACC = TS ? TW : T;
    f32x4 acc[NACC];
#pragma unroll
    for (int t = 0; t < NACC; ++t) acc[t] = f32x4{0.f, 0.f, 0.f, 0.f};
    float bsum[8];
#pragma unroll
    for (int e = 0; e < 8; ++e) bsum[e] = 0.f;

    constexpr int GA = PI * 2, GB = PJ * 2;
    const int ua = tid % GA, ub = tid % GB;
    const int ca = (ciB + (ua >> 1)) * 16 + (ua & 1) * 8;
    const int sa = (a.nasrc > 1 && ca >= C0) ? 1 : 0;
    const int cla = ca - (sa ? C0 : 0);
    const int aC = sa ? a.asrc[1].C : C0;
    const char* abase = (const char*)(sa ? a.asrc[1].ptr : a.asrc[0].ptr) + (size_t)cla * 2;
    const int cb = (coB + (ub >> 1)) * 16 + (ub & 1) * 8;
    const char* bbase = (const char*)a.bsrc.ptr + (size_t)cb * 2;
    const bool do_bias = a.bias_slab != nullptr && ciB == 0 && !a.bias_from_a;
    const bool do_bias_a = a.bias_slab != nullptr && coB == 0 && a.bias_from_a;

    constexpr int UNITS_A = NVA * GA, ITERS_A = (UNITS_A + 255) / 256;
    constexpr int UNITS_B = NVB * GB, ITERS_B = (UNITS_B + 255) / 256;
    static_assert(HZ <= 16 && HY <= 32 && HX <= 64, "staging unit packing");
    int ua_pk[ITERS_A], ub_pk[ITERS_B];
    unsigned ua_vox[ITERS_A], ub_vox[ITERS_B];
#pragma unroll
    for (int itr = 0; itr < ITERS_A; ++itr) {
        const int u = tid + itr * 256, hv = u / GA;
        const int hz = hv / (HY * HX), hr = hv % (HY * HX), hy = hr / HX, hx = hr % HX;
        const int lds_off = (ua >> 1) * PLANE_A + hv * 32 + (ua & 1) * 16;
        ua_pk[itr] = u < UNITS_A ? (hz | (hy << 4) | (hx << 9) | ((lds_off >> 4) << 15)) : -1;
        ua_vox[itr] = (unsigned)((hz * g.H + hy) * g.W + hx);
    }
#pragma unroll
    for (int itr = 0; itr < ITERS_B; ++itr) {
// ... 82 lines not shown
        }
    };

    const char* pa = smem + it_ * PLANE_A + p4 * 8;
    const char* pb = smem + B_OFF + jt * PLANE_B + p4 * 8;
    constexpr bool PREF = KD == 2 || (S == 1 && PI == 1 && ITERS_A + ITERS_B <= 8);
    auto ts_phase = [&](auto wc) {
        constexpr int W = decltype(wc)::value;
        constexpr int NTW = (T - W + 3) / 4, NIT = KSTEPS * NTW, RD = 4;
        const int lr = gq / GPR, lxg = gq % GPR;
        const char* pal = pa + ((lr * S) * HX + (4 * lxg + q4) * S) * 32;
        const char* pbl = pb + (lr * BX + 4 * lxg + q4) * 32;
        auto aoff = [](int s, int r, int t) {
            const int cr = (8 * s + 4 * r) / GPR, z = cr / BY, y = cr % BY;
            return ((z * S * HY + y * S) * HX) * 32 + (((t / (KD * KD)) * HY + (t / KD) % KD) * HX + t % KD) * 32;
        };
        auto boff = [](int s, int r) {
            const int cr = (8 * s + 4 * r) / GPR, z = cr / BY, y = cr % BY;
            return ((z * BY + y) * BX) * 32;
        };
        bf16x8 ring[RD], bfr[2];
        bfr[0] = tr_read2(pbl + boff(0, 0), pbl + boff(0, 1));
#pragma unroll
        for (int n = 0; n < RD; ++n)
            if (n < NIT) ring[n] = tr_read2(pal + aoff(n / NTW, 0, W + 4 * (n % NTW)), pal + aoff(n / NTW, 1, W + 4 * (n % NTW)));
#pragma unroll
        for (int n = 0; n < NIT; ++n) {
            const int s = n / NTW, i = n % NTW;
            if (i == 0 && s + 1 < KSTEPS) bfr[(s + 1) & 1] = tr_read2(pbl + boff(s + 1, 0), pbl + boff(s + 1, 1));
            __builtin_amdgcn_sched_barrier(0);
            acc[i] = __builtin_amdgcn_mfma_f32_16x16x32_bf16(ring[n % RD], bfr[s & 1], acc[i], 0, 0, 0);
            __builtin_amdgcn_sched_barrier(0);
            if (n + RD < NIT) {
                const int m = n + RD;
                ring[m % RD] = tr_read2(pal + aoff(m / NTW, 0, W + 4 * (m % NTW)), pal + aoff(m / NTW, 1, W + 4 * (m % NTW)));
            }
        }
    };
    if (PREF && (int)blockIdx.x < ntiles) prefetch(blockIdx.x, std::false_type{});
    for (int tile = blockIdx.x; tile < ntiles; tile += gridDim.x) {
        __syncthreads();
        if constexpr (PREF) commit(); else prefetch(tile, std::true_type{});
        __syncthreads();
        if (PREF && tile + (int)gridDim.x < ntiles) prefetch(tile + gridDim.x, std::false_type{});
        if constexpr (TS) {
            switch (wave) {
                case 0: ts_phase(std::integral_constant<int, 0>{}); break;
                case 1: ts_phase(std::integral_constant<int, 1>{}); break;
                case 2: ts_phase(std::integral_constant<int, 2>{}); break;
                default: ts_phase(std::integral_constant<int, 3>{}); break;
            }
            continue;
        }
        if constexpr (!TS) {
#pragma unroll 1
        for (int s = kw; s < KSTEPS; s += WPP) {
            int ao[2], bo[2];
#pragma unroll
            for (int r = 0; r < 2; ++r) {
                int grp = 8 * s + 4 * r + gq;
                int row = grp / GPR, xg = grp % GPR;
                int z = row / BY, y = row % BY, x = 4 * xg + q4;
                ao[r] = ((z * S * HY + y * S) * HX + x * S) * 32;
                bo[r] = ((z * BY + y) * BX + x) * 32;
            }
            const bf16x8 bfrag = tr_read2(pb + bo[0], pb + bo[1]);
            bf16x8 abuf[2];
            abuf[0] = tr_read2(pa + ao[0], pa + ao[1]);
#pragma unroll
            for (int t = 0; t < T; ++t) {
                if (t + 1 < T) {
                    const int t1 = t + 1, toff = (((t1 / (KD * KD)) * HY + (t1 / KD) % KD) * HX + t1 % KD) * 32;
                    abuf[t1 & 1] = tr_read2(pa + ao[0] + toff, pa + ao[1] + toff);
                }
                __builtin_amdgcn_sched_barrier(0);
                acc[t] = __builtin_amdgcn_mfma_f32_16x16x32_bf16(abuf[t & 1], bfrag, acc[t], 0, 0, 0);
                __builtin_amdgcn_sched_barrier(0);
            }
        }
        }
    }

    constexpr int RP = 16 * T + 4, ROW4 = 4 * T;
    if constexpr (TS) {
        __syncthreads();
        float* stg = (float*)smem;
#pragma unroll
        for (int i = 0; i < TW; ++i)
            if (wave + 4 * i < T) {
#pragma unroll
                for (int r = 0; r < 4; ++r) stg[il * RP + (gq * 4 + r) * T + wave + 4 * i] = acc[i][r];
            }
        __syncthreads();
        float* base = a.slab + (size_t)blockIdx.x * T * g.Cin * g.Cout + ((size_t)coB * 16 * g.Cin + (size_t)ciB * 16) * T;
        if (a.direct) {
            if ((reinterpret_cast<uintptr_t>(base) & 15) == 0) {
                for (int q = tid; q < 16 * ROW4; q += 256) {
                    const int row = q / ROW4, c4 = q % ROW4;
                    f32x4* d = (f32x4*)(base + (size_t)row * g.Cin * T + c4 * 4);
                    const f32x4 o = *d, v = *(const f32x4*)(stg + row * RP + c4 * 4);
                    *d = f32x4{o[0] + v[0], o[1] + v[1], o[2] + v[2], o[3] + v[3]};
                }
            } else {
                for (int q = tid; q < 16 * 16 * T; q += 256) {
                    const int row = q / (16 * T), c = q % (16 * T);
                    base[(size_t)row * g.Cin * T + c] += stg[row * RP + c];
                }
            }
        } else {
        for (int q = tid; q < 16 * ROW4; q += 256) {
            const int row = q / ROW4, c4 = q % ROW4;
            *(f32x4*)(base + (size_t)row * g.Cin * T + c4 * 4) = *(const f32x4*)(stg + row * RP + c4 * 4);
        }
        }
    }
    if constexpr (!TS) {
    __syncthreads();
    float* red = (float*)smem;
#pragma unroll 1
    for (int kk = 1; kk < WPP; ++kk) {
        if (kw == kk) {
#pragma unroll
            for (int t = 0; t < T; ++t) *(f32x4*)(red + ((pw * T + t) * 64 + lane) * 4) = acc[t];
        }
        __syncthreads();
        if (kw == 0) {
#pragma unroll
            for (int t = 0; t < T; ++t) {
                f32x4 o = *(const f32x4*)(red + ((pw * T + t) * 64 + lane) * 4);
                acc[t][0] += o[0]; acc[t][1] += o[1]; acc[t][2] += o[2]; acc[t][3] += o[3];
            }
        }
        __syncthreads();
    }
    {
        float* stg = (float*)smem;
#pragma unroll 1
        for (int pr = 0; pr < P; ++pr) {
            __syncthreads();
            if (kw == 0 && pw == pr) {
#pragma unroll
                for (int t = 0; t < T; ++t)
#pragma unroll
                    for (int r = 0; r < 4; ++r) stg[il * RP + (gq * 4 + r) * T + t] = acc[t][r];
            }
            __syncthreads();
            float* base = a.slab + (size_t)blockIdx.x * T * g.Cin * g.Cout +
                          ((size_t)(coB + pr % PJ) * 16 * g.Cin + (size_t)(ciB + pr / PJ) * 16) * T;
            for (int q = tid; q < 16 * ROW4; q += 256) {
                const int row = q / ROW4, c4 = q % ROW4;
                *(f32x4*)(base + (size_t)row * g.Cin * T + c4 * 4) = *(const f32x4*)(stg + row * RP + c4 * 4);
            }
        }
    }
    }
    if (do_bias || do_bias_a) {
        const int GU = do_bias_a ? GA : GB;
#pragma unroll
        for (int e = 0; e < 8; ++e) {
            float v = bsum[e];
            for (int m = GU; m < 64; m <<= 1) v += __shfl_xor(v, m);
            bsum[e] = v;
        }
        __syncthreads();
        float* bred = (float*)smem;
        if (lane < GU) {
#pragma unroll
            for (int e = 0; e < 8; ++e) bred[(wave * GU + lane) * 8 + e] = bsum[e];
        }
        __syncthreads();
        if (tid < GU * 8) {
            int u = tid / 8, e = tid % 8;
            float sacc = 0.f;
#pragma unroll
            for (int w = 0; w < 4; ++w) sacc += bred[(w * GU + u) * 8 + e];
            const int nC = do_bias_a ? g.Cin : g.Cout;
            int c = ((do_bias_a ? ciB : coB) + (u >> 1)) * 16 + (u & 1) * 8 + e;
            if (a.direct) a.bias_slab[c] += sacc;
            else a.bias_slab[(size_t)blockIdx.x * nC + c] = sacc;
        }
    }
}

template <int LX, int LY>
__global__ void __launch_bounds__(256) k_mfma_wgrad_reduce(const float* __restrict__ slab, const float* __restrict__ bias_slab, int nsplit,
                                                           int64_t n, int Cb, float* __restrict__ dw, float* __restrict__ db) {
    static_assert(LX * LY == 256, "block shape");
    __shared__ double red[LY > 1 ? LY : 1][LX][4];
    const int64_t ntot = n + (db && bias_slab ? Cb : 0);
    const int lx = threadIdx.x % LX, ly = threadIdx.x / LX;
    const int64_t i = ((int64_t)blockIdx.x * LX + lx) * 4;
    double s0 = 0.0, s1 = 0.0, s2 = 0.0, s3 = 0.0;
    if (i < ntot) {
        const float* base = i < n ? slab + i : bias_slab + (i - n);
        const int64_t stride = i < n ? n : Cb;
        int k = ly;
        for (; k + 7 * LY < nsplit; k += 8 * LY) {
            float4 v[8];
#pragma unroll
            for (int u = 0; u < 8; ++u) v[u] = *(const float4*)(base + (int64_t)(k + u * LY) * stride);
#pragma unroll
            for (int u = 0; u < 8; ++u) { s0 += v[u].x; s1 += v[u].y; s2 += v[u].z; s3 += v[u].w; }
        }
        for (; k < nsplit; k += LY) {
            const float4 v = *(const float4*)(base + (int64_t)k * stride);
            s0 += v.x; s1 += v.y; s2 += v.z; s3 += v.w;
        }
    }
    if (LY > 1) {
        red[ly][lx][0] = s0; red[ly][lx][1] = s1; red[ly][lx][2] = s2; red[ly][lx][3] = s3;
        __syncthreads();
        if (ly == 0) {
            s0 = s1 = s2 = s3 = 0.0;
#pragma unroll
            for (int k = 0; k < LY; ++k) { s0 += red[k][lx][0]; s1 += red[k][lx][1]; s2 += red[k][lx][2]; s3 += red[k][lx][3]; }
        }
    }
    if (ly == 0 && i < ntot) {
        float* d = i < n ? dw + i : db + (i - n);
        d[0] += (float)s0; d[1] += (float)s1; d[2] += (float)s2; d[3] += (float)s3;
    }
}
void wgrad_reduce(const float* slab, const float* bias_slab, int nsplit, int64_t n, int Cb, float* dw, float* db, hipStream_t s) {
    const int64_t ntot = n + (db && bias_slab ? Cb : 0), quads = (ntot + 3) / 4;
    if (nsplit <= 8) k_mfma_wgrad_reduce<256, 1><<<cdiv64(quads, 256), 256, 0, s>>>(slab, bias_slab, nsplit, n, Cb, dw, db);
    else if (nsplit <= 64) k_mfma_wgrad_reduce<64, 4><<<cdiv64(quads, 64), 256, 0, s>>>(slab, bias_slab, nsplit, n, Cb, dw, db);
    else k_mfma_wgrad_reduce<16, 16><<<cdiv64(quads, 16), 256, 0, s>>>(slab, bias_slab, nsplit, n, Cb, dw, db);
}

__global__ void __launch_bounds__(256) k_wgrad_reduce_batched(const WgradReduceJob* __restrict__ jobs, int job0, int njobs, int blk_base,
                                                              const float* __restrict__ ws, float* __restrict__ gflat) {
    __shared__ double red[256][4];
    __shared__ int sj;
    if (threadIdx.x == 0) {
        const int b = (int)blockIdx.x + blk_base;
// ... 188 lines not shown
            const int rz = row / TY, ry = row % TY;
            const int roff = (rz * HY + ry) * TX * 2;
            bf16x8 af[2];
#pragma unroll
            for (int rt = 0; rt < 2; ++rt) af[rt] = *(const bf16x8*)(sm + abase[rt] + roff);
            if (ones_row) af[1] = ones;
#pragma unroll
            for (int n = 0; n < NT; ++n) {
                unsigned d[4];
                const char* pb = sm + DY_OFF + (row * TX + gq * 8) * VSB + (n * 16 + j) * 2;
#pragma unroll
                for (int e = 0; e < 4; ++e) {
                    const unsigned lo = *(const unsigned short*)(pb + (2 * e) * VSB), hi = *(const unsigned short*)(pb + (2 * e + 1) * VSB);
                    d[e] = lo | (hi << 16);
                }
                const bf16x8 bf = __builtin_bit_cast(bf16x8, make_uint4(d[0], d[1], d[2], d[3]));
#pragma unroll
                for (int rt = 0; rt < 2; ++rt) acc[rt][n] = __builtin_amdgcn_mfma_f32_16x16x32_bf16(af[rt], bf, acc[rt][n], 0, 0, 0);
            }
        }
    }
    __syncthreads();
    float* red = (float*)sm;
#pragma unroll
    for (int rt = 0; rt < 2; ++rt)
#pragma unroll
        for (int n = 0; n < NT; ++n) *(f32x4*)(red + (((wave * 2 + rt) * NT + n) * 64 + lane) * 4) = acc[rt][n];
    __syncthreads();
    const int O = 27 * g.Cout;
    float* sl = a.slab + (size_t)blockIdx.x * O;
    for (int e = tid; e < 2 * NT * 256; e += 256) {
        float v = 0.f;
#pragma unroll
        for (int w = 0; w < 4; ++w) v += red[w * 2 * NT * 256 + e];
        const int reg = e & 3, l2 = (e >> 2) & 63, rn = e >> 8, n = rn % NT, rt = rn / NT;
        const int tap = rt * 16 + 4 * (l2 >> 4) + reg, co = n * 16 + (l2 & 15);
        if (tap < 27) sl[co * 27 + tap] = v;
        else if (tap == 27) a.bslab[(size_t)blockIdx.x * g.Cout + co] = v;
    }
}
bool conv_first_wgrad_mfma_supported(int dtype, const ConvGeom& g, const SrcDesc* src, int nsrc) {
    return dtype == 1 && nsrc == 1 && g.Cin == 1 && g.ks == 3 && g.stride == 1 && (g.Cout == 16 || g.Cout == 32) && !src[0].scale &&
           src[0].act == 0;
}
static int first_wgrad_blocks(const ConvGeom& g) {
    int tiles = ((g.W + 31) / 32) * ((g.H + 7) / 8) * ((g.D + 1) / 2);
    return tiles < 512 ? tiles : 512;
}
size_t conv_first_wgrad_mfma_scratch_bytes(const ConvGeom& g) { return (size_t)first_wgrad_blocks(g) * (27 * g.Cout + g.Cout) * 4 + 256; }
int conv_first_wgrad_splits(const ConvGeom& g) { return first_wgrad_blocks(g); }
void launch_conv_first_wgrad_mfma(const ConvGeom& g, const SrcDesc* src, const void* dy, float* dw, float* db, void* scratch, hipStream_t s,
                                  bool defer_reduce, const NormBwdFuse* nb_fuse) {
    FirstWgradArgs a;
    a.g = g; a.x = src[0].ptr; a.dy = dy; a.slab = (float*)scratch;
    a.u = nb_fuse ? nb_fuse->u : nullptr; a.stat = nb_fuse ? nb_fuse->stat : nullptr; a.coef = nb_fuse ? nb_fuse->coef : nullptr;
    a.act = nb_fuse ? nb_fuse->act : 0;
    a.tiles_x = (g.W + 31) / 32; a.tiles_y = (g.H + 7) / 8; a.tiles_z = (g.D + 1) / 2;
    const int nb = first_wgrad_blocks(g);
    const int64_t O = 27 * g.Cout;
    a.bslab = a.slab + (size_t)nb * O;
    if (nb_fuse) {
        if (g.Cout == 16) k_wgrad_first_mfma<1, true><<<nb, 256, 0, s>>>(a);
        else k_wgrad_first_mfma<2, true><<<nb, 256, 0, s>>>(a);
    } else {
        if (g.Cout == 16) k_wgrad_first_mfma<1, false><<<nb, 256, 0, s>>>(a);
        else k_wgrad_first_mfma<2, false><<<nb, 256, 0, s>>>(a);
    }
    if (!defer_reduce) wgrad_reduce(a.slab, db ? a.bslab : nullptr, nb, O, g.Cout, dw, db, s);
}

static bool chan16(const ConvGeom& g, const SrcDesc* src, int nsrc) {
    if (g.Cin % 16 || g.Cout % 16) return false;
    for (int s = 0; s < nsrc; ++s)
        if (src[s].C % 16 || src[s].scale || src[s].act) return false;
    return true;
}
bool mfma_wgrad_supported(int dtype, const ConvGeom& g, const SrcDesc* src, int nsrc) {
    return dtype == 1 && g.ks == 3 && (g.stride == 1 || g.stride == 2) && chan16(g, src, nsrc);
}
bool mfma_convt_wgrad_supported(int dtype, const ConvGeom& g, const SrcDesc* src, int nsrc) {
    return dtype == 1 && nsrc == 1 && chan16(g, src, nsrc);
}

struct WgradCfg { int bz, by, bx, pi, pj, nsplit, gy, direct, polite = 0; };
static bool wgrad_direct_cfg(int kind, int bD, int bH, int bW, WgradCfg& c) {
    if (bD != bH || bH != bW) return false;
    if (bW == 4) { c.bz = 4; c.by = 4; c.bx = 4; }
    else if (bW == 8 && kind == 0) { c.bz = 8; c.by = 8; c.bx = 8; }
    else if (bW == 8) { c.bz = 2; c.by = 8; c.bx = 8; }
    else return false;
    c.pi = c.pj = 1; c.nsplit = 1; c.direct = 1;
    return true;
}
static WgradCfg wgrad_cfg(int kind, int Ca, int Cb, int bD, int bH, int bW) {
    WgradCfg c;
    c.direct = 0;
    int cat = Ca / 16, cbt = Cb / 16;
    if (wgrad_direct_cfg(kind, bD, bH, bW, c)) { c.gy = cat * cbt; return c; }
    if (kind == 0) {
        c.pi = cat % 2 == 0 ? 2 : 1; c.pj = cbt % 2 == 0 ? 2 : 1;
        if (bW >= 12) { c.pi = 1; c.pj = 1; }
        if (bW >= 12) { c.bz = 2; c.by = 8; c.bx = 16; }
        else if (bW > 4) { c.bz = 4; c.by = 8; c.bx = 8; }
        else { c.bz = 4; c.by = 8; c.bx = 4; }
    } else {
        c.pi = 1; c.pj = cbt % 4 == 0 ? 4 : (cbt % 2 == 0 ? 2 : 1);
        if (bW >= 12) { c.bz = 2; c.by = 4; c.bx = 16; }
        else if (bW > 4) { c.bz = 2; c.by = 8; c.bx = 8; }
        else { c.bz = 4; c.by = 8; c.bx = 4; }
    }
    c.gy = (cat / c.pi) * (cbt / c.pj);
    int tiles = ((bW + c.bx - 1) / c.bx) * ((bH + c.by - 1) / c.by) * ((bD + c.bz - 1) / c.bz);
    int want = 512 / c.gy;
    if (want < 1) want = 1;
    c.nsplit = tiles < want ? tiles : want;
    return c;
}
static int s2w_rows_conv(const ConvGeom& g) { return (g.ks == 3 && g.stride == 2) ? s2_wgrad_splits(g.Cin, g.Cout, g.Do, g.Ho, g.Wo) : 0; }
static int s2w_rows_convt(const ConvGeom& g) { return s2_wgrad_splits(g.Cout, g.Cin, g.D, g.H, g.W); }
size_t mfma_wgrad_scratch_bytes(const ConvGeom& g, int polite) {
    if (size_t z = mfma_wgrad_z_scratch_bytes(g, polite)) return z;
    if (int r = s2w_rows_conv(g)) return ((size_t)r * 27 * g.Cin * g.Cout + (size_t)r * g.Cout) * 4 + 256;
    WgradCfg c = wgrad_cfg(g.stride == 1 ? 0 : 1, g.Cin, g.Cout, g.Do, g.Ho, g.Wo);
    return ((size_t)c.nsplit * 27 * g.Cin * g.Cout + (size_t)c.nsplit * g.Cout) * 4 + 256;
}
size_t mfma_convt_wgrad_scratch_bytes(const ConvGeom& g) {
    if (int r = s2w_rows_convt(g)) return ((size_t)r * 8 * g.Cin * g.Cout + (size_t)r * g.Cout) * 4 + 256;
    WgradCfg c = wgrad_cfg(2, g.Cout, g.Cin, g.D, g.H, g.W);
    return ((size_t)c.nsplit * 8 * g.Cin * g.Cout + (size_t)c.nsplit * g.Cout) * 4 + 256;
}

template <int S, int KD, int PAD, int BZ, int BY, int BX, int PI, int PJ>
static void launch_wgrad_cfg(const MfmaWgradArgs& a0, const WgradCfg& c, hipStream_t s) {
    MfmaWgradArgs a = a0;
    a.tiles_x = (a.g.Wo + BX - 1) / BX; a.tiles_y = (a.g.Ho + BY - 1) / BY; a.tiles_z = (a.g.Do + BZ - 1) / BZ;
    constexpr int HZ = (BZ - 1) * S + KD, HY = (BY - 1) * S + KD, HX = (BX - 1) * S + KD, T = KD * KD * KD;
    constexpr size_t tile_lds = (size_t)PI * HZ * HY * HX * 32 + (size_t)PJ * BZ * BY * BX * 32;
    constexpr size_t red_lds = PI * PJ < 4 ? (size_t)(PI * PJ) * T * 64 * 16 : 0;
    constexpr size_t stg_lds = (size_t)16 * (16 * T + 4) * 4;
    constexpr size_t lds0 = tile_lds > red_lds ? (tile_lds > 8192 ? tile_lds : 8192) : red_lds;
    constexpr size_t lds = lds0 > stg_lds ? lds0 : stg_lds;
    static_assert(lds <= 80 * 1024, "two blocks per CU");
    static std::atomic<uint64_t> attr_done{0};
    const int lds_launch = polite_lds((int)lds, c.polite);
    set_max_lds_once(attr_done, (const void*)k_mfma_wgrad<S, KD, PAD, BZ, BY, BX, PI, PJ>, polite_lds((int)lds, 1));
    dim3 grid((unsigned)c.nsplit, (unsigned)c.gy);
    a.direct = c.direct;
    k_mfma_wgrad<S, KD, PAD, BZ, BY, BX, PI, PJ><<<grid, 256, lds_launch, s>>>(a);
}
template <int S, int KD, int PAD, int BZ, int BY, int BX>
static void launch_wgrad_p(const MfmaWgradArgs& a, const WgradCfg& c, hipStream_t s) {
    if constexpr (S == 1) {
        if (c.pi == 2 && c.pj == 2) launch_wgrad_cfg<S, KD, PAD, BZ, BY, BX, 2, 2>(a, c, s);
        else if (c.pi == 2) launch_wgrad_cfg<S, KD, PAD, BZ, BY, BX, 2, 1>(a, c, s);
        else if (c.pj == 2) launch_wgrad_cfg<S, KD, PAD, BZ, BY, BX, 1, 2>(a, c, s);
        else launch_wgrad_cfg<S, KD, PAD, BZ, BY, BX, 1, 1>(a, c, s);
    } else {
        if (c.pj == 4) launch_wgrad_cfg<S, KD, PAD, BZ, BY, BX, 1, 4>(a, c, s);
        else if (c.pj == 2) launch_wgrad_cfg<S, KD, PAD, BZ, BY, BX, 1, 2>(a, c, s);
        else launch_wgrad_cfg<S, KD, PAD, BZ, BY, BX, 1, 1>(a, c, s);
    }
}

int mfma_conv_wgrad_splits(const ConvGeom& g, int polite) {
    if (int z = mfma_wgrad_z_splits(g, polite)) return z;
    if (int r = s2w_rows_conv(g)) return r;
    return wgrad_cfg(g.stride == 1 ? 0 : 1, g.Cin, g.Cout, g.Do, g.Ho, g.Wo).nsplit;
}
int mfma_convt_wgrad_splits(const ConvGeom& g) {
    if (int r = s2w_rows_convt(g)) return r;
    return wgrad_cfg(2, g.Cout, g.Cin, g.D, g.H, g.W).nsplit;
}
bool mfma_conv_wgrad_direct(const ConvGeom& g) {
    if (mfma_wgrad_z_splits(g) || s2w_rows_conv(g)) return false;
    return wgrad_cfg(g.stride == 1 ? 0 : 1, g.Cin, g.Cout, g.Do, g.Ho, g.Wo).direct != 0;
}
bool mfma_convt_wgrad_direct(const ConvGeom& g) { return !s2w_rows_convt(g) && wgrad_cfg(2, g.Cout, g.Cin, g.D, g.H, g.W).direct != 0; }
void launch_mfma_conv_wgrad(const ConvGeom& g, const SrcDesc* src, int nsrc, const void* dy, float* dw, float* db, void* scratch,
                            hipStream_t s, bool defer_reduce, int polite) {
    if (mfma_wgrad_z_supported(1, g, src, nsrc)) {
        const int ns = launch_mfma_wgrad_z(g, src, nsrc, dy, db != nullptr, scratch, s, polite);
        const float* slab = (const float*)scratch;
        if (!defer_reduce)
            wgrad_reduce(slab, db ? slab + (size_t)ns * 27 * g.Cin * g.Cout : nullptr, ns, (int64_t)27 * g.Cin * g.Cout, g.Cout, dw, db, s);
        return;
    }
    if (s2w_rows_conv(g)) {
        const int ns = launch_s2_wgrad(3, src[0].ptr, nsrc > 1 ? src[1].ptr : nullptr, src[0].C, g.Cin, g.D, g.H, g.W, dy, g.Cout, g.Do, g.Ho, g.Wo,
                                       db != nullptr, 0, scratch, s, polite);
        const float* slab = (const float*)scratch;
        if (!defer_reduce)
            wgrad_reduce(slab, db ? slab + (size_t)ns * 27 * g.Cin * g.Cout : nullptr, ns, (int64_t)27 * g.Cin * g.Cout, g.Cout, dw, db, s);
        return;
    }
    WgradCfg c = wgrad_cfg(g.stride == 1 ? 0 : 1, g.Cin, g.Cout, g.Do, g.Ho, g.Wo);
    c.polite = polite;
    MfmaWgradArgs a;
    a.g = g; a.nasrc = nsrc; a.asrc[0] = src[0]; if (nsrc > 1) a.asrc[1] = src[1];
    a.bsrc = SrcDesc(); a.bsrc.ptr = dy; a.bsrc.C = g.Cout;
    a.bias_from_a = 0;
    a.slab = (float*)scratch;
    a.bias_slab = db ? a.slab + (size_t)c.nsplit * 27 * g.Cin * g.Cout : nullptr;
    a.tiles_x = a.tiles_y = a.tiles_z = 0;
    if (c.direct) {
        a.slab = dw; a.bias_slab = db;
        if (g.stride == 1 && c.bx == 4) launch_wgrad_cfg<1, 3, 1, 4, 4, 4, 1, 1>(a, c, s);
        else if (g.stride == 1) launch_wgrad_cfg<1, 3, 1, 8, 8, 8, 1, 1>(a, c, s);
        else if (c.bx == 4) launch_wgrad_cfg<2, 3, 1, 4, 4, 4, 1, 1>(a, c, s);
        else launch_wgrad_cfg<2, 3, 1, 2, 8, 8, 1, 1>(a, c, s);
        return;
    }
    if (g.stride == 1) {
        if (g.Wo >= 12) launch_wgrad_p<1, 3, 1, 2, 8, 16>(a, c, s);
        else if (g.Wo > 4) launch_wgrad_p<1, 3, 1, 4, 8, 8>(a, c, s);
        else launch_wgrad_p<1, 3, 1, 4, 8, 4>(a, c, s);
    } else {
        if (g.Wo >= 12) launch_wgrad_p<2, 3, 1, 2, 4, 16>(a, c, s);
        else if (g.Wo > 4) launch_wgrad_p<2, 3, 1, 2, 8, 8>(a, c, s);
        else launch_wgrad_p<2, 3, 1, 4, 8, 4>(a, c, s);
    }
    if (!defer_reduce) wgrad_reduce(a.slab, a.bias_slab, c.nsplit, (int64_t)27 * g.Cin * g.Cout, g.Cout, dw, db, s);
}

void launch_mfma_convt_wgrad(const ConvGeom& g, const SrcDesc* src, const void* dy, float* dw, void* scratch, hipStream_t s, bool defer_reduce,
                             float* db, int polite) {
    if (s2w_rows_convt(g)) {
        const int ns = launch_s2_wgrad(2, dy, nullptr, g.Cout, g.Cout, g.Do, g.Ho, g.Wo, src[0].ptr, g.Cin, g.D, g.H, g.W, db != nullptr, 1, scratch, s, polite);
        const float* slab = (const float*)scratch;
        if (!defer_reduce)
            wgrad_reduce(slab, db ? slab + (size_t)ns * 8 * g.Cin * g.Cout : nullptr, ns, (int64_t)8 * g.Cin * g.Cout, g.Cout, dw, db, s);
        return;
    }
    WgradCfg c = wgrad_cfg(2, g.Cout, g.Cin, g.D, g.H, g.W);
    c.polite = polite;
    MfmaWgradArgs a;
    a.bias_from_a = 1;
    a.g.Cin = g.Cout; a.g.Cout = g.Cin; a.g.D = g.Do; a.g.H = g.Ho; a.g.W = g.Wo; a.g.Do = g.D; a.g.Ho = g.H; a.g.Wo = g.W;
    a.g.ks = 2; a.g.stride = 2;
    a.nasrc = 1; a.asrc[0] = SrcDesc(); a.asrc[0].ptr = dy; a.asrc[0].C = g.Cout;
    a.bsrc = src[0];
    a.slab = (float*)scratch;
    a.bias_slab = db ? a.slab + (size_t)c.nsplit * 8 * g.Cin * g.Cout : nullptr;
    a.tiles_x = a.tiles_y = a.tiles_z = 0;
    if (c.direct) {
        a.slab = dw; a.bias_slab = db;
        if (c.bx == 4) launch_wgrad_cfg<2, 2, 0, 4, 4, 4, 1, 1>(a, c, s);
        else launch_wgrad_cfg<2, 2, 0, 2, 8, 8, 1, 1>(a, c, s);
        return;
    }
    if (g.W >= 12) launch_wgrad_p<2, 2, 0, 2, 4, 16>(a, c, s);
    else if (g.W > 4) launch_wgrad_p<2, 2, 0, 2, 8, 8>(a, c, s);
    else launch_wgrad_p<2, 2, 0, 4, 8, 4>(a, c, s);
    if (!defer_reduce) wgrad_reduce(a.slab, a.bias_slab, c.nsplit, (int64_t)8 * g.Cin * g.Cout, g.Cout, dw, db, s);
}

}
```

### unet-studio_amd/csrc/kernels_mfma_wgrad_z.hip

```cpp
#include <cstdio>
#include <type_traits>

#include "mfma_util.h"
#ifndef WZ_RD
#define WZ_RD 4
#endif

namespace unet {

typedef __attribute__((ext_vector_type(4))) short zs16x4;
typedef __attribute__((address_space(3))) zs16x4 zlds_s16x4;

struct WgradZArgs {
    ConvGeom g;
    SrcDesc asrc[2];
    int nasrc;
    const void* dy;
    float* slab;
    float* bias_slab;
    int cols_x, cols_y, nseg, zlen;
};

__device__ __forceinline__ bf16x8 ztr_read2(const char* p0, const char* p1) {
    zs16x4 a = __builtin_amdgcn_ds_read_tr16_b64_v4i16((zlds_s16x4*)p0);
    zs16x4 b = __builtin_amdgcn_ds_read_tr16_b64_v4i16((zlds_s16x4*)p1);
    return __builtin_bit_cast(bf16x8, __builtin_shufflevector(a, b, 0, 1, 2, 3, 4, 5, 6, 7));
}

template <int BX, int WK, int PA, int PB>
__global__ void __launch_bounds__(64 * WK * PA * PB, (WK * PA * PB) == 4 ? 2 : 2) k_mfma_wgrad_z(WgradZArgs a) {
    constexpr int NW = WK * PA * PB, NT = 64 * NW, P = PA * PB;
    constexpr int RPK = 32 / BX;
    constexpr int R = 2;
    constexpr int BY = R * WK * RPK, HY = BY + 2, HX = BX + 2;
    constexpr int AROW = HX * 32, APLANE = HY * AROW, BROW = BX * 32, BPLANE = BY * BROW;
    constexpr int BUF = PA * APLANE + PB * BPLANE;
    constexpr int T = 27;
    constexpr int NA = RPK * (R - 1) + 3;
    static_assert(BX == 32 || BX == 16, "row width");
    extern __shared__ __attribute__((aligned(16))) char smem[];

    const ConvGeom& g = a.g;
    const int tid = threadIdx.x, wave = tid >> 6, lane = tid & 63, il = lane & 15, gq = lane >> 4;
    const int q4 = il >> 2, p4 = il & 3;
    const int pw = wave % P, kw = wave / P;
    const int ia = pw / PB, ib = pw % PB;
    const int CBG = (g.Cout / 16) / PB;
    const int caB = ((int)blockIdx.y / CBG) * PA, cbB = ((int)blockIdx.y % CBG) * PB;
    const int C0 = a.asrc[0].C;

    const int item = xcd_remap((int)blockIdx.x, (int)gridDim.x);
    const int ncols = a.cols_x * a.cols_y;
    const int seg = item / ncols, col = item % ncols;
    const int x0 = (col % a.cols_x) * BX, y0 = (col / a.cols_x) * BY;
    const int zs = seg * a.zlen, ze = zs + a.zlen < g.D ? zs + a.zlen : g.D, len = ze - zs;

    f32x4 acc[T];
#pragma unroll
    for (int t = 0; t < T; ++t) acc[t] = f32x4{0.f, 0.f, 0.f, 0.f};
    float bsum[8];
#pragma unroll
    for (int e = 0; e < 8; ++e) bsum[e] = 0.f;

    constexpr int GA = PA * 2, GB = PB * 2;
    static_assert(NT % GA == 0 && NT % GB == 0, "fixed staging roles");
    const int ua = tid % GA, ub = tid % GB;
    const int ca = (caB + (ua >> 1)) * 16 + (ua & 1) * 8;
    const int sa = (a.nasrc > 1 && ca >= C0) ? 1 : 0;
    const int aC = sa ? a.asrc[1].C : C0;
    const char* abase = (const char*)(sa ? a.asrc[1].ptr : a.asrc[0].ptr) + (size_t)(ca - (sa ? C0 : 0)) * 2;
    const int cb = (cbB + (ub >> 1)) * 16 + (ub & 1) * 8;
    const char* bbase = (const char*)a.dy + (size_t)cb * 2;
    const bool do_bias = a.bias_slab != nullptr && caB == 0;
    const unsigned avs = (unsigned)aC * 2, bvs = (unsigned)g.Cout * 2;
    const size_t aplane_b = (size_t)g.H * g.W * avs, bplane_b = (size_t)g.H * g.W * bvs;

    constexpr int UNITS_A = PA * HY * HX * 2, ITERS_A = (UNITS_A + NT - 1) / NT;
    constexpr int UNITS_B = PB * BY * BX * 2, ITERS_B = (UNITS_B + NT - 1) / NT;
    int la[ITERS_A], lb[ITERS_B];
    unsigned ga[ITERS_A], gb[ITERS_B];
    unsigned amask = 0, bmask = 0;
#pragma unroll
    for (int it = 0; it < ITERS_A; ++it) {
        const int u = tid + it * NT, hv = u / GA, hy = hv / HX, hx = hv % HX;
        const int gy = y0 - 1 + hy, gx = x0 - 1 + hx;
// ... 157 lines not shown
            step(c0, c1, c0, n);
            if (n + 1 > len + 1) break;
            step(c1, c2, c1, n + 1);
            if (n + 2 > len + 1) break;
            step(c2, c0, c2, n + 2);
        }
    }
    asm volatile("s_waitcnt vmcnt(0)" ::: "memory");

    constexpr int LDS_BYTES = 2 * BUF;
    constexpr int TCH = (P * 27 * 1024 <= LDS_BYTES) ? 27 : ((P * 9 * 1024 <= LDS_BYTES) ? 9 : 3);
    static_assert(P * TCH * 1024 <= LDS_BYTES, "reduction scratch");
    float* red = (float*)smem;
    if constexpr (WK > 1) {
#pragma unroll 1
        for (int kk = 1; kk < WK; ++kk) {
#pragma unroll
            for (int c0 = 0; c0 < T; c0 += TCH) {
                if (kw == kk) {
#pragma unroll
                    for (int t = 0; t < TCH; ++t) *(f32x4*)(red + ((pw * TCH + t) * 64 + lane) * 4) = acc[c0 + t];
                }
                __syncthreads();
                if (kw == 0) {
#pragma unroll
                    for (int t = 0; t < TCH; ++t) {
                        const f32x4 o = *(const f32x4*)(red + ((pw * TCH + t) * 64 + lane) * 4);
                        acc[c0 + t][0] += o[0]; acc[c0 + t][1] += o[1]; acc[c0 + t][2] += o[2]; acc[c0 + t][3] += o[3];
                    }
                }
                __syncthreads();
            }
        }
    }
    {
        constexpr int RP = 436;
        static_assert(16 * RP * 4 <= LDS_BYTES, "slab staging");
        float* stg = (float*)smem;
        const bool store = a.nseg >= 0;
#pragma unroll 1
        for (int pr = 0; pr < P; ++pr) {
            __syncthreads();
            if (kw == 0 && pw == pr) {
#pragma unroll
                for (int t = 0; t < T; ++t)
#pragma unroll
                    for (int r = 0; r < 4; ++r) stg[il * RP + (gq * 4 + r) * T + t] = acc[t][r];
            }
            __syncthreads();
            float* base = a.slab + (size_t)blockIdx.x * T * g.Cin * g.Cout +
                          ((size_t)(cbB + pr % PB) * 16 * g.Cin + (size_t)(caB + pr / PB) * 16) * T;
            if (store)
                for (int q = tid; q < 16 * 108; q += NT) {
                    const int row = q / 108, c4 = q % 108;
                    *(f32x4*)(base + (size_t)row * g.Cin * T + c4 * 4) = *(const f32x4*)(stg + row * RP + c4 * 4);
                }
        }
    }
    if (do_bias) {
#pragma unroll
        for (int e = 0; e < 8; ++e) {
            float v = bsum[e];
#pragma unroll
            for (int m = GB; m < 64; m <<= 1) v += __shfl_xor(v, m);
            bsum[e] = v;
        }
        __syncthreads();
        float* bred = (float*)smem;
        if (lane < GB) {
#pragma unroll
            for (int e = 0; e < 8; ++e) bred[(wave * GB + lane) * 8 + e] = bsum[e];
        }
        __syncthreads();
        if (tid < GB * 8) {
            const int u = tid / 8, e = tid % 8;
            float sacc = 0.f;
#pragma unroll
            for (int w = 0; w < NW; ++w) sacc += bred[(w * GB + u) * 8 + e];
            a.bias_slab[(size_t)blockIdx.x * g.Cout + (cbB + (u >> 1)) * 16 + (u & 1) * 8 + e] = sacc;
        }
    }
}

struct WgradZCfg { int bx, wk, pa, pb, by, cols_x, cols_y, nseg, zlen, gx, gy; };

static bool wgrad_z_cfg(const ConvGeom& g, WgradZCfg& c, int polite = 0) {
    if (sliding_window_off() || g.ks != 3 || g.stride != 1 || g.Cin % 16 || g.Cout % 16) return false;
    if (g.W < 24 || g.D < 4) return false;
    const int cat = g.Cin / 16, cbt = g.Cout / 16;
    c.bx = 32;
    if (cat % 2 == 0 && cbt % 2 == 0) { c.pa = 2; c.pb = 2; c.wk = 2; }
    else if (cat % 2 == 0) { c.pa = 2; c.pb = 1; c.wk = 4; }
    else if (cbt % 2 == 0) { c.pa = 1; c.pb = 2; c.wk = 4; }
    else { c.pa = 1; c.pb = 1; c.wk = 4; }
    if ((int64_t)g.D * g.H * g.W <= (int64_t)32768) { c.pa = 1; c.pb = 1; c.wk = 4; }
    else if (polite) {
        if (cat % 2 == 0) { c.pa = 2; c.pb = 1; c.wk = 2; }
        else if (cbt % 2 == 0) { c.pa = 1; c.pb = 2; c.wk = 2; }
        else { c.pa = 1; c.pb = 1; c.wk = 4; }
    }
    c.by = 2 * c.wk;
    c.cols_x = (g.W + c.bx - 1) / c.bx; c.cols_y = (g.H + c.by - 1) / c.by;
    c.gy = (cat / c.pa) * (cbt / c.pb);
    const int cols = c.cols_x * c.cols_y;
    const int nwaves = c.wk * c.pa * c.pb;
    int want = nwaves == 4 ? (polite ? 256 : 512) : 256;
    want /= c.gy;
    if (want < 1) want = 1;
    int nseg = (want + cols - 1) / cols;
    if (nseg < 1) nseg = 1;
    int zlen = (g.D + nseg - 1) / nseg;
    if (zlen < 4) zlen = 4;
    if (zlen > g.D) zlen = g.D;
    c.nseg = (g.D + zlen - 1) / zlen; c.zlen = zlen;
    c.gx = cols * c.nseg;
    return true;
}
bool mfma_wgrad_z_supported(int dtype, const ConvGeom& g, const SrcDesc* src, int nsrc) {
    WgradZCfg c;
    if (dtype != 1 || !wgrad_z_cfg(g, c)) return false;
    for (int s = 0; s < nsrc; ++s)
        if (src[s].C % 16 || src[s].scale || src[s].act) return false;
    return true;
}
int mfma_wgrad_z_splits(const ConvGeom& g, int polite) {
    WgradZCfg c;
    return wgrad_z_cfg(g, c, polite) ? c.gx : 0;
}
size_t mfma_wgrad_z_scratch_bytes(const ConvGeom& g, int polite) {
    WgradZCfg c;
    if (!wgrad_z_cfg(g, c, polite)) return 0;
    return ((size_t)c.gx * 27 * g.Cin * g.Cout + (size_t)c.gx * g.Cout) * 4 + 256;
}

template <int BX, int WK, int PA, int PB>
static void launch_wz(const WgradZArgs& a, const WgradZCfg& c, hipStream_t s, int polite) {
    constexpr int RPK = 32 / BX, BY = 2 * WK * RPK, HY = BY + 2, HX = BX + 2;
    constexpr int lds = 2 * (PA * HY * HX * 32 + PB * BY * BX * 32);
    static_assert(lds <= 80 * 1024, "LDS budget");
    static_assert(WK * PA * PB == 8, "the 4-wave work splits run on k_mfma_wgrad_zd");
    static std::atomic<uint64_t> attr_done{0};
    set_max_lds_once(attr_done, (const void*)k_mfma_wgrad_z<BX, WK, PA, PB>, lds);
    (void)polite;
    k_mfma_wgrad_z<BX, WK, PA, PB><<<dim3((unsigned)c.gx, (unsigned)c.gy), 64 * WK * PA * PB, lds, s>>>(a);
}

int launch_mfma_wgrad_z(const ConvGeom& g, const SrcDesc* src, int nsrc, const void* dy, bool want_bias, void* scratch, hipStream_t s,
                        int polite) {
    WgradZCfg c;
    if (!wgrad_z_cfg(g, c, polite)) return 0;
    WgradZArgs a;
    a.g = g; a.nasrc = nsrc; a.asrc[0] = src[0]; if (nsrc > 1) a.asrc[1] = src[1];
    a.dy = dy;
    a.slab = (float*)scratch;
    a.bias_slab = want_bias ? a.slab + (size_t)c.gx * 27 * g.Cin * g.Cout : nullptr;
    a.cols_x = c.cols_x; a.cols_y = c.cols_y; a.nseg = c.nseg; a.zlen = c.zlen;
    if (launch_wgrad_zd(g, src, nsrc, dy, a.slab, a.bias_slab, c.wk, c.pa, c.pb, c.cols_x, c.cols_y, c.nseg, c.zlen, c.gx, c.gy, s, polite)) return c.gx;
    if (c.pa == 2 && c.pb == 2) launch_wz<32, 2, 2, 2>(a, c, s, polite);
    else if (c.pa == 2) launch_wz<32, 4, 2, 1>(a, c, s, polite);
    else launch_wz<32, 4, 1, 2>(a, c, s, polite);
    return c.gx;
}

}
```

### unet-studio_amd/csrc/kernels_mfma_wgrad_zd.hip

```cpp
#include <cstdio>
#include <cstdlib>
#include <type_traits>

#include "mfma_util.h"

namespace unet {

__device__ __attribute__((aligned(16))) unsigned g_wzd_zero[4] = {0u, 0u, 0u, 0u};

typedef __attribute__((ext_vector_type(4))) short zd16x4;
typedef __attribute__((address_space(3))) zd16x4 zdlds_s16x4;
__device__ __forceinline__ bf16x8 zdtr_read2(const char* p0, const char* p1) {
    zd16x4 a = __builtin_amdgcn_ds_read_tr16_b64_v4i16((zdlds_s16x4*)p0);
    zd16x4 b = __builtin_amdgcn_ds_read_tr16_b64_v4i16((zdlds_s16x4*)p1);
    return __builtin_bit_cast(bf16x8, __builtin_shufflevector(a, b, 0, 1, 2, 3, 4, 5, 6, 7));
}

struct WgradZdArgs {
    ConvGeom g;
    SrcDesc asrc[2];
    int nasrc;
    const void* dy;
    float* slab;
    float* bias_slab;
    int cols_x, cols_y, nseg, zlen;
};

#define WZD_DMA(src, dst)                                                                                                    \
    do {                                                                                                                     \
        unsigned keep_;                                                                                                      \
        asm volatile("s_mov_b32 %0, m0\n\ts_mov_b32 m0, %2\n\ts_nop 0\n\tglobal_load_lds_dwordx4 %1, off\n\ts_mov_b32 m0, %0" \
                     : "=&s"(keep_) : "v"(src), "s"(__builtin_amdgcn_readfirstlane((int)(dst))) : "memory");                 \
    } while (0)

template <int WK, int PA, int PB>
__global__ void __launch_bounds__(256, 2) k_mfma_wgrad_zd(WgradZdArgs a) {
    constexpr int P = PA * PB, T = 27, BX = 32, R = 2, BY = R * WK, HY = BY + 2, HX = BX + 2;
    static_assert(WK * P == 4, "four waves");
    constexpr int NVA = HY * HX, NVB = BY * BX;
    constexpr int APLANE = NVA * 32, BPLANE = NVB * 32, BUF = PA * APLANE + PB * BPLANE;
    constexpr int NB = 4, PF = 3;
    constexpr int UA = PA * NVA * 2, UB = PB * NVB * 2;
    constexpr int UPWA = (UA + 3) / 4, UPWB = (UB + 3) / 4, ITA = (UPWA + 63) / 64, ITB = (UPWB + 63) / 64;
    constexpr int PP = ITA + ITB, WAITN = (PF - 1) * PP;
    static_assert(3 * UPWA + (ITA - 1) * 64 < UA && 3 * UPWB + (ITB - 1) * 64 < UB, "every wave issues every piece");
    static_assert(UPWB % 2 == 0 && (PB == 1 || (NVB * 2) % UPWB == 0), "a thread's dy units are all of one (tile, half)");
    constexpr bool FULLA = UA == 4 * UPWA && UPWA % 64 == 0, FULLB = UB == 4 * UPWB && UPWB % 64 == 0;
    extern __shared__ __attribute__((aligned(16))) char smem[];

    const ConvGeom& g = a.g;
    const int tid = threadIdx.x, lane = tid & 63, il = lane & 15, gq = lane >> 4, q4 = il >> 2, p4 = il & 3;
    const int wave = __builtin_amdgcn_readfirstlane(tid >> 6), pw = wave % P, kw = wave / P, ia = pw / PB, ib = pw % PB;
    const int CBG = (g.Cout / 16) / PB;
    const int caB = ((int)blockIdx.y / CBG) * PA, cbB = ((int)blockIdx.y % CBG) * PB;
    const int C0 = a.asrc[0].C;
    const unsigned lds0 = (unsigned)(size_t)(__attribute__((address_space(3))) char*)smem;

    const int item = xcd_remap((int)blockIdx.x, (int)gridDim.x);
    const int ncols = a.cols_x * a.cols_y, seg = item / ncols, col = item % ncols;
    const int x0 = (col % a.cols_x) * BX, y0 = (col / a.cols_x) * BY;
    const int zs = seg * a.zlen, ze = zs + a.zlen < g.D ? zs + a.zlen : g.D, len = ze - zs;

    f32x4 acc[T];
#pragma unroll
    for (int t = 0; t < T; ++t) acc[t] = f32x4{0.f, 0.f, 0.f, 0.f};
    float bsum[8];
#pragma unroll
    for (int e = 0; e < 8; ++e) bsum[e] = 0.f;
    const bool do_bias = a.bias_slab != nullptr && caB == 0;

    const char* abase[ITA];
    const char* bbase[ITB];
    size_t aplane[ITA];
    bool aact[ITA], bact[ITB];
    unsigned apiece[ITA], bpiece[ITB];
#pragma unroll
    for (int it = 0; it < ITA; ++it) {
        const int u = wave * UPWA + it * 64 + lane, tile = u / (NVA * 2), hv = (u >> 1) % NVA, half = u & 1, hy = hv / HX, hx = hv % HX;
        const int gy = y0 - 1 + hy, gx = x0 - 1 + hx, c = (caB + tile) * 16 + half * 8;
        const int sa = (a.nasrc > 1 && c >= C0) ? 1 : 0, aC = sa ? a.asrc[1].C : C0;
        aact[it] = it * 64 + lane < UPWA && u < UA;
        const bool ok = aact[it] && (unsigned)gy < (unsigned)g.H && (unsigned)gx < (unsigned)g.W;
        abase[it] = ok ? (const char*)(sa ? a.asrc[1].ptr : a.asrc[0].ptr) + (((size_t)gy * g.W + gx) * aC + (c - (sa ? C0 : 0))) * 2 : nullptr;
        aplane[it] = (size_t)g.H * g.W * aC * 2;
        apiece[it] = (unsigned)__builtin_amdgcn_readfirstlane((wave * UPWA + it * 64) * 16);
    }
#pragma unroll
    for (int it = 0; it < ITB; ++it) {
        const int u = wave * UPWB + it * 64 + lane, tile = u / (NVB * 2), tv = (u >> 1) % NVB, half = u & 1, ty = tv / BX, tx = tv % BX;
        const int gy = y0 + ty, gx = x0 + tx;
        bact[it] = it * 64 + lane < UPWB && u < UB;
        const bool ok = bact[it] && gy < g.H && gx < g.W;
        bbase[it] = ok ? (const char*)a.dy + (((size_t)gy * g.W + gx) * g.Cout + (cbB + tile) * 16 + half * 8) * 2 : nullptr;
        bpiece[it] = (unsigned)__builtin_amdgcn_readfirstlane((PA * APLANE + (wave * UPWB + it * 64) * 16));
    }
    const size_t bplane = (size_t)g.H * g.W * g.Cout * 2;
    auto request = [&](int k) {
        const int pz = zs - 1 + k, bz = zs + k;
        const bool ain = (unsigned)pz < (unsigned)g.D && k <= len + 1, bin = bz < ze;
        const unsigned buf = lds0 + (unsigned)(k % NB) * BUF;
#pragma unroll
        for (int it = 0; it < ITA; ++it) {
            const char* src = (ain && abase[it]) ? abase[it] + (size_t)pz * aplane[it] : (const char*)g_wzd_zero;
            if (FULLA || it + 1 < ITA || aact[it]) WZD_DMA(src, buf + apiece[it]);
        }
#pragma unroll
        for (int it = 0; it < ITB; ++it) {
            const char* src = (bin && bbase[it]) ? bbase[it] + (size_t)bz * bplane : (const char*)g_wzd_zero;
// ... 38 lines not shown
                    const int ky = ai - j;
                    if (ky >= 0 && ky <= 2)
                        acc[kz * 9 + ky * 3 + kx] = __builtin_amdgcn_mfma_f32_16x16x32_bf16(ring[i % RD], Bq[(PH + (3 - kz)) % 3][j], acc[kz * 9 + ky * 3 + kx], 0, 0, 0);
                }
            __builtin_amdgcn_sched_barrier(0);
            if (i + RD < NREAD) {
                const int m = i + RD;
                ring[m % RD] = zdtr_read2(pa0 + ((m / 3) * HX + m % 3) * 32, pa1 + ((m / 3) * HX + m % 3) * 32);
            }
        }
    };
    auto bias_add = [&](const char* buf) {
#pragma unroll
        for (int it = 0; it < ITB; ++it) {
            if (bact[it]) {
                const uint4 v = *(const uint4*)(buf + PA * APLANE + (size_t)(wave * UPWB + it * 64 + lane) * 16);
                bsum[0] += bf_lo(v.x); bsum[1] += bf_hi(v.x); bsum[2] += bf_lo(v.y); bsum[3] += bf_hi(v.y);
                bsum[4] += bf_lo(v.z); bsum[5] += bf_hi(v.z); bsum[6] += bf_lo(v.w); bsum[7] += bf_hi(v.w);
            }
        }
    };

    const std::integral_constant<int, 0> c0;
    const std::integral_constant<int, 1> c1;
    const std::integral_constant<int, 2> c2;
#pragma unroll
    for (int k = 0; k < PF; ++k) request(k);
    auto step = [&](auto ph, int n) {
        asm volatile("s_waitcnt vmcnt(%0)\n\ts_barrier" :: "n"(WAITN) : "memory");
        request(n + PF);
        const char* buf = smem + (n % NB) * BUF;
        if (do_bias && n < len) bias_add(buf);
        compute(ph, buf, n < len);
    };
    for (int n = 0; n <= len + 1; n += 3) {
        step(c0, n);
        if (n + 1 > len + 1) break;
        step(c1, n + 1);
        if (n + 2 > len + 1) break;
        step(c2, n + 2);
    }
    asm volatile("s_waitcnt vmcnt(0)\n\ts_barrier" ::: "memory");

    constexpr int LDS_BYTES = NB * BUF;
    constexpr int TCH = (P * 27 * 1024 <= LDS_BYTES) ? 27 : ((P * 9 * 1024 <= LDS_BYTES) ? 9 : 3);
    static_assert(P * TCH * 1024 <= LDS_BYTES, "reduction scratch");
    float* red = (float*)smem;
    if constexpr (WK > 1) {
#pragma unroll 1
        for (int kk = 1; kk < WK; ++kk) {
#pragma unroll
            for (int t0 = 0; t0 < T; t0 += TCH) {
                if (kw == kk) {
#pragma unroll
                    for (int t = 0; t < TCH; ++t) *(f32x4*)(red + ((pw * TCH + t) * 64 + lane) * 4) = acc[t0 + t];
                }
                __syncthreads();
                if (kw == 0) {
#pragma unroll
                    for (int t = 0; t < TCH; ++t) {
                        const f32x4 o = *(const f32x4*)(red + ((pw * TCH + t) * 64 + lane) * 4);
                        acc[t0 + t][0] += o[0]; acc[t0 + t][1] += o[1]; acc[t0 + t][2] += o[2]; acc[t0 + t][3] += o[3];
                    }
                }
                __syncthreads();
            }
        }
    }
    {
        constexpr int RP = 436;
        static_assert(16 * RP * 4 <= LDS_BYTES, "slab staging");
        float* stg = (float*)smem;
#pragma unroll 1
        for (int pr = 0; pr < P; ++pr) {
            __syncthreads();
            if (kw == 0 && pw == pr) {
#pragma unroll
                for (int t = 0; t < T; ++t)
#pragma unroll
                    for (int r = 0; r < 4; ++r) stg[il * RP + (gq * 4 + r) * T + t] = acc[t][r];
            }
            __syncthreads();
            float* base = a.slab + (size_t)blockIdx.x * T * g.Cin * g.Cout + ((size_t)(cbB + pr % PB) * 16 * g.Cin + (size_t)(caB + pr / PB) * 16) * T;
            for (int q = tid; q < 16 * 108; q += 256) {
                const int row = q / 108, c4 = q % 108;
                *(f32x4*)(base + (size_t)row * g.Cin * T + c4 * 4) = *(const f32x4*)(stg + row * RP + c4 * 4);
            }
        }
    }
    if (do_bias) {
#pragma unroll
        for (int e = 0; e < 8; ++e) {
            float v = bsum[e];
#pragma unroll
            for (int m = 2; m < 64; m <<= 1) v += __shfl_xor(v, m);
            bsum[e] = v;
        }
        __syncthreads();
        float* bred = (float*)smem;
        if (lane < 2) {
#pragma unroll
            for (int e = 0; e < 8; ++e) bred[(wave * 2 + lane) * 8 + e] = bsum[e];
        }
        __syncthreads();
        if (tid < PB * 16) {
            const int tile = tid / 16, half = (tid / 8) & 1, e = tid % 8;
            float sacc = 0.f;
#pragma unroll
            for (int w = 0; w < 4; ++w)
                if ((w * UPWB) / (NVB * 2) == tile) sacc += bred[(w * 2 + half) * 8 + e];
            a.bias_slab[(size_t)blockIdx.x * g.Cout + (cbB + tile) * 16 + half * 8 + e] = sacc;
        }
    }
}

template <int WK, int PA, int PB>
static void launch_zd_t(const WgradZdArgs& a, int gx, int gy, hipStream_t s, int polite) {
    constexpr int BY = 2 * WK, lds = 4 * (PA * (BY + 2) * 34 * 32 + PB * BY * 32 * 32);
    static_assert(lds <= 80 * 1024, "two blocks per CU");
    static std::atomic<uint64_t> attr_done{0};
    set_max_lds_once(attr_done, (const void*)k_mfma_wgrad_zd<WK, PA, PB>, polite_lds(lds, 1));
    k_mfma_wgrad_zd<WK, PA, PB><<<dim3((unsigned)gx, (unsigned)gy), 256, polite_lds(lds, polite), s>>>(a);
}
bool launch_wgrad_zd(const ConvGeom& g, const SrcDesc* src, int nsrc, const void* dy, float* slab, float* bias_slab, int wk, int pa, int pb, int cols_x,
                     int cols_y, int nseg, int zlen, int gx, int gy, hipStream_t s, int polite) {
    if (wk * pa * pb != 4) return false;
    for (int k = 0; k < nsrc; ++k) if ((size_t)g.H * g.W * src[k].C * 2 >= ((size_t)1 << 40)) return false;
    WgradZdArgs a;
    a.g = g; a.nasrc = nsrc; a.asrc[0] = src[0]; if (nsrc > 1) a.asrc[1] = src[1];
    a.dy = dy; a.slab = slab; a.bias_slab = bias_slab;
    a.cols_x = cols_x; a.cols_y = cols_y; a.nseg = nseg; a.zlen = zlen;
    if (wk == 2 && pa == 2) launch_zd_t<2, 2, 1>(a, gx, gy, s, polite);
    else if (wk == 2) launch_zd_t<2, 1, 2>(a, gx, gy, s, polite);
    else launch_zd_t<4, 1, 1>(a, gx, gy, s, polite);
    return true;
}

}
```

### unet-studio_amd/csrc/mfma_util.h

```cpp
#pragma once
#include <atomic>
#include <cstdint>
#include <cstdlib>

#include "device_util.h"

namespace unet {

inline void set_max_lds_once(std::atomic<uint64_t>& done, const void* fn, int bytes) {
    int dev = 0;
    (void)hipGetDevice(&dev);
    const uint64_t bit = 1ull << (dev & 63);
    if (done.load(std::memory_order_acquire) & bit) return;
    (void)hipFuncSetAttribute(fn, hipFuncAttributeMaxDynamicSharedMemorySize, bytes);
    done.fetch_or(bit, std::memory_order_release);
}

inline int polite_lds(int lds, int polite) {
    constexpr int want = 83000;
    return (polite && want > lds) ? want : lds;
}
inline bool sliding_window_off() {
    static const bool off = getenv("UNET_NO_SLIDING_WINDOW") != nullptr;
    return off;
}

typedef __attribute__((ext_vector_type(8))) __bf16 bf16x8;
typedef __attribute__((ext_vector_type(4))) float f32x4;

__device__ __forceinline__ unsigned pack_bf16x2(float lo, float hi) {
    return (unsigned)__bfloat16_as_ushort(__float2bfloat16(lo)) | ((unsigned)__bfloat16_as_ushort(__float2bfloat16(hi)) << 16);
}
__device__ __forceinline__ float bf_lo(unsigned w) { return __uint_as_float(w << 16); }
__device__ __forceinline__ float bf_hi(unsigned w) { return __uint_as_float(w & 0xffff0000u); }

__device__ __forceinline__ int xcd_remap(int b, int n) {
    int q = n >> 3, r = n & 7, x = b & 7;
    return (x < r ? x * (q + 1) : r * (q + 1) + (x - r) * q) + (b >> 3);
}

__device__ __forceinline__ uint4 transform8(uint4 v, bool xf, const float* sc, const float* sh, int act) {
    if (!(xf || act)) return v;
    unsigned wv[4] = {v.x, v.y, v.z, v.w};
#pragma unroll
    for (int e = 0; e < 4; ++e) {
        float lo = bf_lo(wv[e]), hi = bf_hi(wv[e]);
        if (xf) { lo = fmaf(lo, sc[2 * e], sh[2 * e]); hi = fmaf(hi, sc[2 * e + 1], sh[2 * e + 1]); }
        lo = act_f(lo, act); hi = act_f(hi, act);
        wv[e] = pack_bf16x2(lo, hi);
    }
    return make_uint4(wv[0], wv[1], wv[2], wv[3]);
}

struct MfmaConvArgs {
    ConvGeom g;
    SrcDesc src[2];
    int nsrc;
    const void* w;
    const float* bias;
    void* out[2];
    int outC[2];
    int out_acc[2];
    int nout;
    float* stats;
    int tiles_x, tiles_y, tiles_z;
    int sc_C;
    int oD, oH, oW;
    const void* bn_u = nullptr;
    const float* bn_stat = nullptr;
    float* bn_partial = nullptr;
    int bn_act = 0, bn_C = 0;
};

struct ZWork { int nseg, zlen, cols_x, cols_y; };
inline int z_split(ZWork& zw, int planes, int gy, int min_zlen) {
    const int cols = zw.cols_x * zw.cols_y;
    int want = 512 / gy;
    if (want < 1) want = 1;
    const int nseg = (want + cols - 1) / cols;
    int zlen = (planes + nseg - 1) / nseg;
    if (zlen < min_zlen) zlen = min_zlen;
    if (zlen > planes) zlen = planes;
    zw.nseg = (planes + zlen - 1) / zlen; zw.zlen = zlen;
    const int items = cols * zw.nseg;
    return items < want ? items : want;
}
int launch_conv_z16(const MfmaConvArgs& a, hipStream_t s);
int conv_z16_blocks(const MfmaConvArgs& a, ZWork* zw = nullptr);
int launch_conv_z32(const MfmaConvArgs& a, hipStream_t s);
bool launch_wgrad_zd(const ConvGeom& g, const SrcDesc* src, int nsrc, const void* dy, float* slab, float* bias_slab, int wk, int pa, int pb, int cols_x,
                     int cols_y, int nseg, int zlen, int gx, int gy, hipStream_t s, int polite);

}
```

### unet-studio_amd/engine.py

```python
import ctypes as C
import os

_HERE = os.path.dirname(os.path.abspath(__file__))
LIB_PATH = os.environ.get("UNET_HIP_LIBRARY") or os.path.join(_HERE, "libunet_hip.so")

DTYPE_F32, DTYPE_BF16 = 0, 1
IMPL_AUTO, IMPL_DIRECT = 0, 1

if not os.path.exists(LIB_PATH):
    raise ImportError(
        "libunet_hip.so not found at %s: build it first (python -c 'import __graft_entry__ as g; g.build()' "
        "or unet-studio_amd/csrc/build.sh); there is no CPU fallback" % LIB_PATH)

import torch

lib = C.CDLL(LIB_PATH)

_vp, _i, _sz, _f = C.c_void_p, C.c_int, C.c_size_t, C.c_float
_pp = C.POINTER(C.c_void_p)


def _sig(name, res, *args):
    fn = getattr(lib, name)
    fn.restype = res
    fn.argtypes = list(args)
    return fn


_sig("unet_last_error", C.c_char_p)
_sig("unet_init", _i, C.POINTER(_i))
_sig("unet_device_info", _i, _i, C.c_char_p, _sz, C.POINTER(_sz), C.POINTER(_i), C.POINTER(_i))
_sig("unet_plan_create", _i, C.c_char_p, _i, _i, _i, _i, _i, _i, _i, _i, C.POINTER(_vp))
_sig("unet_plan_destroy", None, _vp)
_sig("unet_plan_param_count", _i, _vp, C.POINTER(_i))
_sig("unet_plan_param_shape", _i, _vp, _i, C.POINTER(C.c_int64), C.POINTER(_i))
_sig("unet_plan_param_name", _i, _vp, _i, C.c_char_p, _sz)
_sig("unet_plan_param_decay", _i, _vp, _i, C.POINTER(_i))
_sig("unet_plan_param_fan_in", _i, _vp, _i, C.POINTER(C.c_int64), C.POINTER(_i))
_sig("unet_plan_buffer_count", _i, _vp, C.POINTER(_i))
_sig("unet_plan_buffer_shape", _i, _vp, _i, C.POINTER(C.c_int64))
_sig("unet_plan_output_count", _i, _vp, C.POINTER(_i))
_sig("unet_plan_output_shape", _i, _vp, _i, C.POINTER(C.c_int64))
_sig("unet_plan_workspace_bytes", _i, _vp, C.POINTER(_sz))
_sig("unet_plan_flops", _i, _vp, C.POINTER(C.c_double), C.POINTER(C.c_double))
_sig("unet_plan_describe", _sz, _vp, C.c_char_p, _sz)
_sig("unet_plan_op_count", _i, _vp, C.POINTER(_i))
_sig("unet_plan_op_info", _i, _vp, _i, C.POINTER(_i), C.POINTER(_i), C.POINTER(_i), C.POINTER(_i), C.POINTER(_i), C.POINTER(C.c_int64),
     C.POINTER(C.c_int64), C.c_char_p, _sz)
_sig("unet_profile_begin", _i)
_sig("unet_profile_end", _i, _i, C.POINTER(_i), C.POINTER(_i), C.POINTER(_f), C.POINTER(_i))
_sig("unet_forward", _i, _vp, _pp, _pp, _vp, _pp, _vp, _i, _vp)
_sig("unet_backward", _i, _vp, _pp, _pp, _pp, _vp, _vp, _vp)
_sig("unet_backward_part", _i, _vp, _pp, _pp, _pp, _vp, _vp, _i, _i, _vp)
_sig("unet_plan_backward_buckets", _i, _vp, _i, C.POINTER(_i), C.POINTER(_i), C.POINTER(C.c_int64))
_sig("unet_loss_scratch_bytes", _i, _vp, C.POINTER(_sz))
_sig("unet_loss", _i, _vp, _pp, _vp, _i, _i, _pp, _vp, _vp, _vp)
_sig("unet_forward_loss", _i, _vp, _pp, _pp, _vp, _pp, _vp, _i, _i, _pp, _vp, _vp, _vp, _vp)
_sig("unet_forward_loss_mode", _i, _vp, _pp, _pp, _vp, _pp, _vp, _i, _i, _pp, _vp, _vp, _vp, _i, _vp)
_sig("unet_sum_buffers", _i, _pp, _i, _vp, C.c_int64, _i, _vp)
_sig("unet_stream_create_cu_range", _i, _i, _i, _i, _vp)
_sig("unet_stream_destroy", _i, _vp)
_sig("unet_plan_side_cu_range", _i, _vp, _i, _i)
_sig("unet_pack_filters", _i, _vp, _vp, _vp, _i, _vp, _vp)
_sig("unet_sgd_step", _i, _vp, _vp, _vp, _vp, _f, _f, _i, _f, _f, _f, _vp, _vp, _vp)
_sig("unet_sgd_step_packed", _i, _vp, _vp, _vp, _vp, _f, _f, _i, _f, _f, _f, _vp, _vp, _i, _vp, _vp, _vp)
_sig("unet_set_error", None, C.c_char_p)
_sig("unet_comm_unique_id", _i, _vp)
_sig("unet_comm_create", _i, _i, _i, _vp, _i, C.POINTER(_vp))
_sig("unet_comm_create_all", _i, _i, C.POINTER(_i), C.POINTER(_vp))
_sig("unet_comm_destroy", _i, _vp)
_sig("unet_comm_rank", _i, _vp, C.POINTER(_i), C.POINTER(_i))
_sig("unet_allreduce_grads", _i, _vp, _vp, C.c_int64, C.c_int64, _vp)
_sig("unet_allreduce_grads_all", _i, _pp, _i, _pp, C.c_int64, C.c_int64, _pp)
_sig("unet_comm_broadcast", _i, _vp, _vp, C.c_int64, _i, _vp)
_sig("unet_comm_join", _i, _vp, _vp)
_sig("unet_op_scratch_bytes", _i, _i, _i, _i, _i, _i, C.POINTER(_sz))
_sig("unet_op_conv_choice", _i, _i, _i, _i, _i, _i, _i, _i, _i, _i, _i, C.POINTER(_i))
_sig("unet_op_conv3d_fwd", _i, _i, _i, _vp, _vp, _vp, _vp, _i, _i, _i, _i, _i, _i, _i, _vp, _vp)
_sig("unet_op_conv3d_pack", _i, _i, _vp, _vp, _i, _i, _i, _i, _i, _i, _i, _vp)
_sig("unet_op_conv3d_fwd_packed", _i, _i, _vp, _vp, _vp, _vp, _vp, _i, _i, _i, _i, _i, _i, _i, _vp)
_sig("unet_op_conv3d_fwd_fused", _i, _i, _i, _vp, _vp, _vp, _i, _vp, _vp, _vp, _vp, _i, _i, _i, _i, _i, _i, _i, _vp, _vp)
_sig("unet_op_conv3d_bwd_data", _i, _i, _i, _vp, _vp, _vp, _i, _i, _i, _i, _i, _i, _i, _vp, _vp)
_sig("unet_op_conv3d_fwd_norm", _i, _vp, _vp, _i, _i, _vp, _vp, _vp, _vp, C.c_double, _vp, _vp, C.c_double, _i, _i, _vp, _vp, _vp,
     _i, _i, _i, _i, _i, _vp, _vp)
_sig("unet_op_conv3d_bwd_data_norm", _i, _i, _vp, _vp, _vp, _i, _vp, _vp, _vp, _i, _vp, _vp, _vp, _i, _i, _i, _i, _i, _vp, _vp)
_sig("unet_op_conv3d_bwd_weight", _i, _i, _i, _vp, _vp, _vp, _vp, _i, _i, _i, _i, _i, _i, _i, _vp, _vp)
_sig("unet_op_convt_fwd", _i, _i, _i, _vp, _vp, _vp, _vp, _i, _i, _i, _i, _i, _vp, _vp)
_sig("unet_op_convt_bwd_data", _i, _i, _i, _vp, _vp, _vp, _i, _i, _i, _i, _i, _vp, _vp)
_sig("unet_op_convt_bwd_weight", _i, _i, _i, _vp, _vp, _vp, _vp, _i, _i, _i, _i, _i, _vp, _vp)
_sig("unet_op_pack_ndhwc", _i, _i, _vp, _vp, _i, C.c_int64, _vp)
_sig("unet_op_unpack_ncdhw", _i, _i, _vp, _vp, _i, C.c_int64, _vp)

EXPORTS = [
    "unet_last_error", "unet_init", "unet_device_info", "unet_plan_create", "unet_plan_destroy", "unet_plan_param_count",
    "unet_plan_param_shape", "unet_plan_param_name", "unet_plan_param_decay", "unet_plan_param_fan_in", "unet_plan_buffer_count",
    "unet_plan_buffer_shape", "unet_plan_output_count", "unet_plan_output_shape", "unet_plan_workspace_bytes",
    "unet_plan_flops", "unet_plan_describe", "unet_plan_op_count", "unet_plan_op_info", "unet_profile_begin", "unet_profile_end", "unet_forward", "unet_backward", "unet_backward_part", "unet_plan_backward_buckets", "unet_loss_scratch_bytes", "unet_loss", "unet_forward_loss", "unet_forward_loss_mode", "unet_sum_buffers",
    "unet_sgd_step", "unet_sgd_step_packed", "unet_pack_filters", "unet_stream_create_cu_range", "unet_stream_destroy", "unet_plan_side_cu_range", "unet_set_error", "unet_comm_unique_id", "unet_comm_create", "unet_comm_create_all", "unet_comm_destroy", "unet_comm_rank",
    "unet_allreduce_grads", "unet_allreduce_grads_all", "unet_comm_broadcast", "unet_comm_join", "unet_op_scratch_bytes", "unet_op_conv_choice", "unet_op_conv3d_fwd", "unet_op_conv3d_fwd_fused", "unet_op_conv3d_pack", "unet_op_conv3d_fwd_packed", "unet_op_conv3d_bwd_data", "unet_op_conv3d_fwd_norm", "unet_op_conv3d_bwd_data_norm", "unet_op_conv3d_bwd_weight",
    "unet_op_convt_fwd", "unet_op_convt_bwd_data", "unet_op_convt_bwd_weight", "unet_op_pack_ndhwc", "unet_op_unpack_ncdhw",
]


MODE_PACKS_CURRENT = 2


class UNetError(RuntimeError):
    """What the C++ host rethrows as std::runtime_error (unet.cpp:53,66,88,117)."""


def check(rc):
    if rc != 0:
        raise UNetError(lib.unet_last_error().decode("utf-8", "replace"))


def scratch(buf, need, device):
    if buf is None or buf.nbytes < need:
        buf = torch.empty(need, dtype=torch.uint8, device=device)
    return buf


def stream(t_or_device, stream=None):
    if stream is not None:
        return stream
    return torch.cuda.current_stream(t_or_device.device if torch.is_tensor(t_or_device) else t_or_device).cuda_stream


def ptr_array(ptrs):
    arr = (C.c_void_p * max(1, len(ptrs)))()
    for i, p in enumerate(ptrs):
        arr[i] = p
    return arr


def size_query(fn, *args):
    n = C.c_size_t()
    check(fn(*args, C.byref(n)))
    return n.value


def u32_array(values):
    return (C.c_uint32 * max(1, len(values)))(*values)


def listed_classes(who, classes, n_classes):
    classes = list(range(1, int(n_classes))) if classes is None else [int(v) for v in classes]
    for v in classes:
        if not 0 <= v < 1 << 32:
            raise UNetError("%s: listed class %d is not in [1, %d]" % (who, v, int(n_classes) - 1))
    return classes


class Plan:

    def __init__(self, arch, in_c, out_c, size, dtype=DTYPE_BF16, device=0, impl=IMPL_AUTO):
        self.handle = C.c_void_p()
        self._pid = os.getpid()
        D, H, W = size
        check(lib.unet_plan_create(arch.encode(), in_c, out_c, D, H, W, dtype, device, impl, C.byref(self.handle)))
        self.arch, self.in_c, self.out_c, self.size, self.dtype, self.device = arch, in_c, out_c, (D, H, W), dtype, device
        n = C.c_int()
        check(lib.unet_plan_param_count(self.handle, C.byref(n)))
        self.param_shapes, self.param_decay, self.param_fan_in, self.param_is_norm_weight, self.param_names = [], [], [], [], []
        dims, nd, dec, fan, isn = (C.c_int64 * 5)(), C.c_int(), C.c_int(), C.c_int64(), C.c_int()
        for i in range(n.value):
            check(lib.unet_plan_param_shape(self.handle, i, dims, C.byref(nd)))
            self.param_shapes.append(tuple(dims[k] for k in range(nd.value)))
            nm = C.create_string_buffer(128)
            check(lib.unet_plan_param_name(self.handle, i, nm, 128))
            self.param_names.append(nm.value.decode())
            check(lib.unet_plan_param_decay(self.handle, i, C.byref(dec)))
            self.param_decay.append(bool(dec.value))
            check(lib.unet_plan_param_fan_in(self.handle, i, C.byref(fan), C.byref(isn)))
            self.param_fan_in.append(fan.value)
            self.param_is_norm_weight.append(bool(isn.value))
        check(lib.unet_plan_buffer_count(self.handle, C.byref(n)))
        self.buffer_numel = []
        ne = C.c_int64()
        for i in range(n.value):
            check(lib.unet_plan_buffer_shape(self.handle, i, C.byref(ne)))
            self.buffer_numel.append(ne.value)
        check(lib.unet_plan_output_count(self.handle, C.byref(n)))
# ... 109 lines not shown
```

Baseline: 809.9 million.

## Size wgrad split grids by CU fill and add direct one-range gradient accumulation

Replaces the fixed block-count heuristic for splitting weight-gradient voxel ranges with a shared helper that targets a CU-fill count that depends on whether the launch is polite (side-stream). It also adds a direct mode where a single-range wgrad launch adds straight into the gradient and bias buffers instead of writing a scratch slab that is later reduced. Together these aim to cut slab write/read traffic and reduce passes while keeping the GPU filled. It also adds introspection APIs (unet_plan_wgrad_grid, unet_op_wgrad_split, a concat-source wgrad op) and a profiling script. The risks are fewer splits for small layers and read-modify-write on the gradient.

After: 810.7 million (median of 2 runs). Within noise of the previous version (+0.1%).

```diff
diff --git a/include/unet_hip.h b/include/unet_hip.h
--- a/include/unet_hip.h
+++ b/include/unet_hip.h
@@ -41,6 +41,7 @@
 int unet_plan_op_count(const unet_plan* plan, int* n);
 int unet_plan_op_info(const unet_plan* plan, int i, int* kind, int* cin, int* cout, int* ks, int* stride, int64_t in_dims[3],
                       int64_t out_dims[3], char* name, size_t name_len);
+int unet_plan_wgrad_grid(const unet_plan* plan, int i, int out[6]);
 
 #define UNET_PROF_CONV_FWD 0
 #define UNET_PROF_DGRAD 1
@@ -111,6 +112,9 @@
                                  int W, void* scratch, void* stream);
 int unet_op_conv3d_bwd_weight(int dtype, int impl, const void* x, const void* dy, float* dw, float* db, int cin, int cout,
                               int D, int H, int W, int ks, int stride, void* scratch, void* stream);
+int unet_op_conv3d_bwd_weight_cat(int dtype, int impl, const void* x0, int cin0, const void* x1, int cin1, const void* dy, float* dw,
+                                  float* db, int cout, int D, int H, int W, int ks, int stride, void* scratch, void* stream);
+int unet_op_wgrad_split(int dtype, int cin, int cout, int D, int H, int W, int ks, int stride, int transposed, int polite, int out[4]);
 int unet_op_convt_fwd(int dtype, int impl, const void* x, const float* w, const float* b, void* y, int cin, int cout, int D,
                       int H, int W, void* scratch, void* stream);
 int unet_op_convt_bwd_data(int dtype, int impl, const void* dy, const float* w, void* dx, int cin, int cout, int D, int H,
diff --git a/profiles/wgrad_slab_table.py b/profiles/wgrad_slab_table.py
--- /dev/null
+++ b/profiles/wgrad_slab_table.py
@@ -0,0 +1,35 @@
+#!/usr/bin/env python3
+import ctypes as C
+import os
+import sys
+
+ROOT = os.path.dirname(os.path.dirname(os.path.abspath(__file__)))
+sys.path.insert(0, ROOT)
+import unet_studio_amd as U
+
+n = int(sys.argv[1]) if len(sys.argv) > 1 else 128
+cin = int(sys.argv[2]) if len(sys.argv) > 2 else 1
+m = U.UNet3d(cin, 6, U.default_feature(6), device="cuda:0", dtype="bf16", seed=0)
+plan = m.plan_for((n, n, n))
+KERNEL = {1: "k_mfma_wgrad_z(d)", 2: "k_s2_wgrad", 3: "k_mfma_wgrad"}
+print("%-42s %-12s %-18s %-10s %6s %10s %5s %12s" % ("op", "output", "kernel", "grid", "polite", "operand MB", "rows", "slab w+r MB"))
+tot_rows = tot_slab = tot_direct = 0
+for i, o in enumerate(plan.ops()):
+    g = (C.c_int * 6)()
+    U.engine.check(U.engine.lib.unet_plan_wgrad_grid(plan.handle, i, g))
+    kern, ranges, groups, direct, polite, rows = tuple(g)
+    if not kern:
+        continue
+    vi = o["in_dims"][0] * o["in_dims"][1] * o["in_dims"][2]
+    vo = o["out_dims"][0] * o["out_dims"][1] * o["out_dims"][2]
+    operands = 2.0 * (vi * o["cin"] + vo * o["cout"])
+    taps = 8 if o["kind"] == 2 else 27
+    row = 4.0 * (taps * o["cin"] * o["cout"] + o["cout"])
+    slab = 0.0 if direct else 2.0 * ranges * row
+    assert direct or rows in (0, ranges), (o["name"], rows, ranges)
+    tot_rows += 0 if direct else ranges
+    tot_slab += slab
+    tot_direct += 1 if direct else 0
+    print("%-42s %-12s %-18s %-10s %6d %10.1f %5s %12.1f" % (o["name"], "%dx%dx%d" % tuple(o["out_dims"]), KERNEL[kern], "%dx%d" % (ranges, groups),
+                                                          polite, operands / 1e6, "add" if direct else ranges, slab / 1e6))
+print("slab rows %d, slab bytes written + read %.1f MB per step; %d ops add into the gradient themselves" % (tot_rows, tot_slab / 1e6, tot_direct))
diff --git a/unet-studio_amd/csrc/conv_select.h b/unet-studio_amd/csrc/conv_select.h
--- a/unet-studio_amd/csrc/conv_select.h
+++ b/unet-studio_amd/csrc/conv_select.h
@@ -42,4 +42,14 @@
     return c;
 }
 
+constexpr int kWgradCUs = 256;
+inline int wgrad_fill_blocks(int polite, int per_cu) { return polite ? kWgradCUs : kWgradCUs * per_cu; }
+inline int wgrad_voxel_ranges(int groups, int max_ranges, int fill) {
+    int want = fill / groups;
+    if (want > max_ranges) want = max_ranges;
+    return want < 1 ? 1 : want;
 }
+inline bool wgrad_rows_outweigh_operands(int ranges, long long row_bytes, long long operand_bytes) { return 2 * ranges * row_bytes > operand_bytes; }
+inline bool wgrad_one_range(int columns, long long operand_bytes, long long row_bytes) { return columns == 1 && row_bytes > operand_bytes; }
+
+}
diff --git a/unet-studio_amd/csrc/engine.cpp b/unet-studio_amd/csrc/engine.cpp
--- a/unet-studio_amd/csrc/engine.cpp
+++ b/unet-studio_amd/csrc/engine.cpp
@@ -259,7 +259,7 @@
             grow(wmax, wgrad_direct_scratch_bytes(cg, op.kind == OP_CONVT));
             if (op.kind == OP_CONVT) {
                 if (c.wgrad == Wgrad::mfma) {
-                    grow(wmax, mfma_convt_wgrad_scratch_bytes(cg));
+                    grow(wmax, mfma_convt_wgrad_scratch_bytes(cg, side_polite[i]));
                     grow(wmax, bias_grad_scratch_bytes(cg.Cout, (int64_t)cg.Do * cg.Ho * cg.Wo));
                 }
                 continue;
@@ -287,8 +287,8 @@
             if (op.out_level >= 0 || (w != Wgrad::first_mfma && w != Wgrad::mfma)) continue;
             const ConvGeom cg = op_geom_of(op);
             if (w == Wgrad::first_mfma) wz_off[i] = take(conv_first_wgrad_mfma_scratch_bytes(cg));
-            else if (op.kind == OP_CONV) { if (!mfma_conv_wgrad_direct(cg)) wz_off[i] = take(mfma_wgrad_scratch_bytes(cg, side_polite[i])); }
-            else if (!mfma_convt_wgrad_direct(cg)) wz_off[i] = take(mfma_convt_wgrad_scratch_bytes(cg));
+            else if (op.kind == OP_CONV) { if (!mfma_conv_wgrad_direct(cg, side_polite[i])) wz_off[i] = take(mfma_wgrad_scratch_bytes(cg, side_polite[i])); }
+            else if (!mfma_convt_wgrad_direct(cg, side_polite[i])) wz_off[i] = take(mfma_convt_wgrad_scratch_bytes(cg, side_polite[i]));
         }
         ws_bytes = off;
         p_off.assign(g.params.size() + 1, 0);
@@ -310,7 +310,7 @@
             j.dw_off = p_off[op.weight];
             j.Cb = op.cout;
             if (op.kind == OP_CONVT) {
-                j.nsplit = mfma_convt_wgrad_splits(cg);
+                j.nsplit = mfma_convt_wgrad_splits(cg, side_polite[i]);
                 j.n = (long long)8 * op.cin * op.cout;
                 j.bias_off = op.bias >= 0 ? j.slab_off + (long long)j.nsplit * j.n : -1;
                 j.db_off = op.bias >= 0 ? p_off[op.bias] : -1;
@@ -1139,6 +1139,20 @@
     return 0;
 }
 
+int unet_plan_wgrad_grid(const unet_plan* p, int i, int out[6]) {
+    if (i < 0 || i >= (int)p->g.ops.size()) return fail("op index out of range");
+    if (!out) return fail("unet_plan_wgrad_grid: null output");
+    const Op& op = p->g.ops[i];
+    for (int k = 0; k < 6; ++k) out[k] = 0;
+    if ((op.kind != OP_CONV && op.kind != OP_CONVT) || p->conv[i].wgrad != Wgrad::mfma) return 0;
+    const ConvGeom cg = p->op_geom_of(op);
+    const int polite = p->side_polite[i];
+    const WgradGrid w = op.kind == OP_CONVT ? mfma_convt_wgrad_grid(cg, polite) : mfma_conv_wgrad_grid(cg, polite);
+    out[0] = w.kernel; out[1] = w.ranges; out[2] = w.groups; out[3] = w.direct; out[4] = polite;
+    out[5] = p->wz_job_of_op[i] >= 0 ? p->wz_jobs[p->wz_job_of_op[i]].nsplit : 0;
+    return 0;
+}
+
 int unet_profile_begin(void) {
     if (g_prof) return fail("unet_profile_begin: a profile is already open on this thread");
     g_prof = new ProfSink();
@@ -1441,7 +1455,7 @@
         w = std::max(mfma_wgrad_scratch_bytes(g, 0), mfma_wgrad_scratch_bytes(g, 1));
         if (w > b) b = w;
         g.Do = 2 * D; g.Ho = 2 * H; g.Wo = 2 * W;
-        w = mfma_convt_wgrad_scratch_bytes(g);
+        w = std::max(mfma_convt_wgrad_scratch_bytes(g, 0), mfma_convt_wgrad_scratch_bytes(g, 1));
         if (w > b) b = w;
     }
     *bytes = b;
@@ -1652,6 +1666,36 @@
         }
     })
 }
+int unet_op_conv3d_bwd_weight_cat(int dtype, int impl, const void* x0, int cin0, const void* x1, int cin1, const void* dy, float* dw,
+                                  float* db, int cout, int D, int H, int W, int ks, int stride, void* scratch, void* stream) {
+    OP_TRY({
+        if (cin0 < 1 || cin1 < 1 || !x0 || !x1) throw std::runtime_error("unet_op_conv3d_bwd_weight_cat: two sources of at least one channel");
+        hipStream_t s = (hipStream_t)stream;
+        ConvGeom g = op_geom(cin0 + cin1, cout, D, H, W, ks, stride, false);
+        SrcDesc sd[2];
+        sd[0].ptr = x0; sd[0].C = cin0; sd[1].ptr = x1; sd[1].C = cin1;
+        switch (choose_conv(dtype, impl, g, sd, 2, false, false).wgrad) {
+            case Wgrad::first_mfma: throw std::runtime_error("unet_op_conv3d_bwd_weight_cat: a first conv has one source");
+            case Wgrad::mfma: launch_mfma_conv_wgrad(g, sd, 2, dy, dw, db, scratch, s, false, env().op_polite ? 1 : 0); break;
+            case Wgrad::f32_mfma: launch_wgrad_f32_mfma(g, sd, 2, (const float*)dy, dw, db, scratch, s); break;
+            case Wgrad::small: launch_conv_wgrad_small(dtype, g, sd, 2, dy, dw, db, scratch, s); break;
+            case Wgrad::direct: launch_conv_wgrad_direct(dtype, g, sd, 2, dy, dw, db, nullptr, s);
+        }
+    })
+}
+int unet_op_wgrad_split(int dtype, int cin, int cout, int D, int H, int W, int ks, int stride, int transposed, int polite, int out[4]) {
+    try {
+        if (!out) throw std::runtime_error("unet_op_wgrad_split: null output");
+        if (cin < 1 || cout < 1 || D < 1 || H < 1 || W < 1) throw std::runtime_error("unet_op_wgrad_split: sizes must be positive");
+        const ConvGeom g = transposed ? op_geom(cin, cout, D, H, W, 2, 2, true) : op_geom(cin, cout, D, H, W, ks, stride, false);
+        SrcDesc sd; sd.C = cin;
+        out[0] = out[1] = out[2] = out[3] = 0;
+        if (choose_conv(dtype, UNET_IMPL_AUTO, g, &sd, 1, false, transposed != 0).wgrad != Wgrad::mfma) return 0;
+        const WgradGrid w = transposed ? mfma_convt_wgrad_grid(g, polite ? 1 : 0) : mfma_conv_wgrad_grid(g, polite ? 1 : 0);
+        out[0] = w.kernel; out[1] = w.ranges; out[2] = w.groups; out[3] = w.direct;
+        return 0;
+    } catch (const std::exception& e) { return fail(e.what()); }
+}
 int unet_op_convt_fwd(int dtype, int impl, const void* x, const float* w, const float* b, void* y, int cin, int cout, int D, int H,
                       int W, void* scratch, void* stream) {
     OP_TRY({
@@ -1695,7 +1739,7 @@
         ConvGeom g = op_geom(cin, cout, D, H, W, 2, 2, true);
         SrcDesc sd; sd.ptr = x; sd.C = cin;
         if (choose_conv(dtype, impl, g, &sd, 1, false, true).wgrad == Wgrad::mfma)
-            launch_mfma_convt_wgrad(g, &sd, dy, dw, scratch, (hipStream_t)stream, false, db);
+            launch_mfma_convt_wgrad(g, &sd, dy, dw, scratch, (hipStream_t)stream, false, db, env().op_polite ? 1 : 0);
         else
             launch_convt_wgrad_direct(dtype, g, &sd, 1, dy, dw, db, nullptr, (hipStream_t)stream);
     })
diff --git a/unet-studio_amd/csrc/kernels.h b/unet-studio_amd/csrc/kernels.h
--- a/unet-studio_amd/csrc/kernels.h
+++ b/unet-studio_amd/csrc/kernels.h
@@ -147,8 +147,13 @@
 bool mfma_wgrad_z_supported(int dtype, const ConvGeom& g, const SrcDesc* src, int nsrc);
 size_t mfma_wgrad_z_scratch_bytes(const ConvGeom& g, int polite = 0);
 int mfma_wgrad_z_splits(const ConvGeom& g, int polite = 0);
+bool mfma_wgrad_z_direct(const ConvGeom& g, int polite = 0);
 int launch_mfma_wgrad_z(const ConvGeom& g, const SrcDesc* src, int nsrc, const void* dy, bool want_bias, void* scratch, hipStream_t s,
-                        int polite = 0);
+                        int polite = 0, float* dw = nullptr, float* db = nullptr);
+struct WgradGrid { int kernel, ranges, groups, direct; };
+bool mfma_wgrad_z_grid(const ConvGeom& g, int polite, WgradGrid& w);
+WgradGrid mfma_conv_wgrad_grid(const ConvGeom& g, int polite);
+WgradGrid mfma_convt_wgrad_grid(const ConvGeom& g, int polite);
 void wgrad_reduce(const float* slab, const float* bias_slab, int nsplit, int64_t n, int Cb, float* dw, float* db, hipStream_t s);
 struct WgradReduceJob { long long slab_off, bias_off, dw_off, db_off, n; int nsplit, Cb, ly, blk0, nblk, op; };
 int wgrad_reduce_job_blocks(WgradReduceJob& j, int blk0);
@@ -157,9 +162,9 @@
 bool mfma_wgrad_supported(int dtype, const ConvGeom& g, const SrcDesc* src, int nsrc);
 size_t mfma_wgrad_scratch_bytes(const ConvGeom& g, int polite = 0);
 int mfma_conv_wgrad_splits(const ConvGeom& g, int polite = 0);
-int mfma_convt_wgrad_splits(const ConvGeom& g);
-bool mfma_conv_wgrad_direct(const ConvGeom& g);
-bool mfma_convt_wgrad_direct(const ConvGeom& g);
+int mfma_convt_wgrad_splits(const ConvGeom& g, int polite = 0);
+bool mfma_conv_wgrad_direct(const ConvGeom& g, int polite = 0);
+bool mfma_convt_wgrad_direct(const ConvGeom& g, int polite = 0);
 int conv_first_wgrad_splits(const ConvGeom& g);
 void launch_mfma_conv_wgrad(const ConvGeom& g, const SrcDesc* src, int nsrc, const void* dy, float* dw, float* db, void* scratch,
                             hipStream_t s, bool defer_reduce = false, int polite = 0);
@@ -180,7 +185,7 @@
 void launch_conv_wgrad_small(int dtype, const ConvGeom& g, const SrcDesc* src, int nsrc, const void* dy, float* dw, float* db,
                              void* scratch, hipStream_t s);
 bool mfma_convt_wgrad_supported(int dtype, const ConvGeom& g, const SrcDesc* src, int nsrc);
-size_t mfma_convt_wgrad_scratch_bytes(const ConvGeom& g);
+size_t mfma_convt_wgrad_scratch_bytes(const ConvGeom& g, int polite = 0);
 void launch_mfma_convt_wgrad(const ConvGeom& g, const SrcDesc* src, const void* dy, float* dw, void* scratch, hipStream_t s,
                              bool defer_reduce = false, float* db = nullptr, int polite = 0);
 int launch_colsum_partial8(int dtype, const void* x, int C, int64_t S, float* partial, hipStream_t s);
@@ -206,7 +211,7 @@
 int s2_conv_dgrad_rows_max();
 bool launch_s2_convt_fwd(const ConvGeom& g, const SrcDesc* src, int nsrc, const void* w_mfma, const float* bias, void* out, hipStream_t s);
 bool launch_s2_convt_dgrad(const ConvGeom& g, const void* dy, const void* w_mfma_dgrad, const DstGrad* dst, int ndst, hipStream_t s);
-int s2_wgrad_splits(int Ca, int Cb, int cD, int cH, int cW);
+int s2_wgrad_splits(int ks, int Ca, int Cb, int cD, int cH, int cW, int polite, int* gy = nullptr);
 int launch_s2_wgrad(int ks, const void* fine, const void* fine2, int C0, int Ca, int fD, int fH, int fW, const void* coarse, int Cb, int cD, int cH,
                     int cW, bool want_bias, int bias_from_a, void* scratch, hipStream_t s, int polite);
 constexpr int64_t DEEP_MAX_VOXELS = 512;
diff --git a/unet-studio_amd/csrc/kernels_mfma_s2_wgrad.hip b/unet-studio_amd/csrc/kernels_mfma_s2_wgrad.hip
--- a/unet-studio_amd/csrc/kernels_mfma_s2_wgrad.hip
+++ b/unet-studio_amd/csrc/kernels_mfma_s2_wgrad.hip
@@ -2,6 +2,7 @@
 #include <cstdlib>
 #include <type_traits>
 
+#include "conv_select.h"
 #include "mfma_util.h"
 
 namespace unet {
@@ -258,22 +259,20 @@
 }
 
 struct S2WCfg { int pa, pb, wk, byc, cols_x, cols_y, nseg, zlen, gx, gy; };
-static bool s2w_cfg(int Ca, int Cb, int cD, int cH, int cW, S2WCfg& c) {
+static bool s2w_cfg(int ks, int Ca, int Cb, int cD, int cH, int cW, int polite, S2WCfg& c) {
     if (sliding_window_off() || Ca % 16 || Cb % 16 || cW < 24 || cD < 4) return false;
     if ((size_t)(2 * cH + 1) * (2 * cW + 1) * Ca * 2 >= ((size_t)1 << 31) || (size_t)cH * cW * Cb * 2 >= ((size_t)1 << 31)) return false;
     const int cat = Ca / 16, cbt = Cb / 16;
+    if (cat % 2 != 0 && cbt % 2 != 0) return false;
+    c.byc = 2;
+    c.cols_x = (cW + 31) / 32; c.cols_y = (cH + c.byc - 1) / c.byc;
+    const int cols = c.cols_x * c.cols_y;
     if (cat % 2 == 0 && cbt % 2 == 0) { c.pa = 2; c.pb = 2; c.wk = 1; }
     else if (cbt % 2 == 0) { c.pa = 1; c.pb = 2; c.wk = 2; }
-    else if (cat % 2 == 0) { c.pa = 2; c.pb = 1; c.wk = 2; }
-    else return false;
-    c.byc = 2;
-    c.cols_x = (cW + 31) / 32; c.cols_y = (cH + c.byc - 1) / c.byc;
+    else { c.pa = 2; c.pb = 1; c.wk = 2; }
     c.gy = (cat / c.pa) * (cbt / c.pb);
-    const int cols = c.cols_x * c.cols_y;
-    int want = 512 / c.gy;
-    if (want < 1) want = 1;
-    int nseg = (want + cols - 1) / cols;
-    if (nseg < 1) nseg = 1;
+    const int want = wgrad_voxel_ranges(c.gy, 1 << 30, wgrad_fill_blocks(polite, 2));
+    const int nseg = (want + cols - 1) / cols;
     int zlen = (cD + nseg - 1) / nseg;
     if (zlen < 4) zlen = 4;
     if (zlen > cD) zlen = cD;
@@ -281,9 +280,11 @@
     c.gx = cols * c.nseg;
     return true;
 }
-int s2_wgrad_splits(int Ca, int Cb, int cD, int cH, int cW) {
+int s2_wgrad_splits(int ks, int Ca, int Cb, int cD, int cH, int cW, int polite, int* gy) {
     S2WCfg c;
-    return s2w_cfg(Ca, Cb, cD, cH, cW, c) ? c.gx : 0;
+    if (!s2w_cfg(ks, Ca, Cb, cD, cH, cW, polite, c)) return 0;
+    if (gy) *gy = c.gy;
+    return c.gx;
 }
 template <int KS, int PA, int PB, int WK>
 static void launch_s2w_t(const S2WgradArgs& a, const S2WCfg& c, hipStream_t s, int polite) {
@@ -298,7 +299,7 @@
 int launch_s2_wgrad(int ks, const void* fine, const void* fine2, int C0, int Ca, int fD, int fH, int fW, const void* coarse, int Cb, int cD, int cH,
                     int cW, bool want_bias, int bias_from_a, void* scratch, hipStream_t s, int polite) {
     S2WCfg c;
-    if (!s2w_cfg(Ca, Cb, cD, cH, cW, c)) return 0;
+    if (!s2w_cfg(ks, Ca, Cb, cD, cH, cW, polite, c)) return 0;
     S2WgradArgs a;
     a.fine = fine; a.fine2 = fine2; a.C0 = C0; a.coarse = coarse; a.Ca = Ca; a.Cb = Cb; a.fD = fD; a.fH = fH; a.fW = fW; a.cD = cD; a.cH = cH; a.cW = cW;
     const int T = ks * ks * ks;
diff --git a/unet-studio_amd/csrc/kernels_mfma_wgrad.hip b/unet-studio_amd/csrc/kernels_mfma_wgrad.hip
--- a/unet-studio_amd/csrc/kernels_mfma_wgrad.hip
+++ b/unet-studio_amd/csrc/kernels_mfma_wgrad.hip
@@ -1,4 +1,5 @@
 #include <type_traits>
+#include "conv_select.h"
 #include "mfma_util.h"
 
 namespace unet {
@@ -247,17 +248,7 @@
     }
 
     constexpr int RP = 16 * T + 4, ROW4 = 4 * T;
-    if constexpr (TS) {
-        __syncthreads();
-        float* stg = (float*)smem;
-#pragma unroll
-        for (int i = 0; i < TW; ++i)
-            if (wave + 4 * i < T) {
-#pragma unroll
-                for (int r = 0; r < 4; ++r) stg[il * RP + (gq * 4 + r) * T + wave + 4 * i] = acc[i][r];
-            }
-        __syncthreads();
-        float* base = a.slab + (size_t)blockIdx.x * T * g.Cin * g.Cout + ((size_t)coB * 16 * g.Cin + (size_t)ciB * 16) * T;
+    auto put_tile = [&](float* base, const float* stg) {
         if (a.direct) {
             if ((reinterpret_cast<uintptr_t>(base) & 15) == 0) {
                 for (int q = tid; q < 16 * ROW4; q += 256) {
@@ -273,11 +264,23 @@
                 }
             }
         } else {
-        for (int q = tid; q < 16 * ROW4; q += 256) {
-            const int row = q / ROW4, c4 = q % ROW4;
-            *(f32x4*)(base + (size_t)row * g.Cin * T + c4 * 4) = *(const f32x4*)(stg + row * RP + c4 * 4);
-        }
-        }
+            for (int q = tid; q < 16 * ROW4; q += 256) {
+                const int row = q / ROW4, c4 = q % ROW4;
+                *(f32x4*)(base + (size_t)row * g.Cin * T + c4 * 4) = *(const f32x4*)(stg + row * RP + c4 * 4);
+            }
+        }
+    };
+    if constexpr (TS) {
+        __syncthreads();
+        float* stg = (float*)smem;
+#pragma unroll
+        for (int i = 0; i < TW; ++i)
+            if (wave + 4 * i < T) {
+#pragma unroll
+                for (int r = 0; r < 4; ++r) stg[il * RP + (gq * 4 + r) * T + wave + 4 * i] = acc[i][r];
+            }
+        __syncthreads();
+        put_tile(a.slab + (size_t)blockIdx.x * T * g.Cin * g.Cout + ((size_t)coB * 16 * g.Cin + (size_t)ciB * 16) * T, stg);
     }
     if constexpr (!TS) {
     __syncthreads();
@@ -312,10 +315,7 @@
             __syncthreads();
             float* base = a.slab + (size_t)blockIdx.x * T * g.Cin * g.Cout +
                           ((size_t)(coB + pr % PJ) * 16 * g.Cin + (size_t)(ciB + pr / PJ) * 16) * T;
-            for (int q = tid; q < 16 * ROW4; q += 256) {
-                const int row = q / ROW4, c4 = q % ROW4;
-                *(f32x4*)(base + (size_t)row * g.Cin * T + c4 * 4) = *(const f32x4*)(stg + row * RP + c4 * 4);
-            }
+            put_tile(base, stg);
         }
     }
     }
@@ -670,14 +670,14 @@
     return dtype == 1 && nsrc == 1 && chan16(g, src, nsrc);
 }
 
-struct WgradCfg { int bz, by, bx, pi, pj, nsplit, gy, direct, polite = 0; };
+struct WgradCfg { int bz, by, bx, pi, pj, nsplit, gy, direct, polite = 0, ostat = 0; };
 static bool wgrad_direct_cfg(int kind, int bD, int bH, int bW, WgradCfg& c) {
     if (bD != bH || bH != bW) return false;
     if (bW == 4) { c.bz = 4; c.by = 4; c.bx = 4; }
     else if (bW == 8 && kind == 0) { c.bz = 8; c.by = 8; c.bx = 8; }
     else if (bW == 8) { c.bz = 2; c.by = 8; c.bx = 8; }
     else return false;
-    c.pi = c.pj = 1; c.nsplit = 1; c.direct = 1;
+    c.pi = c.pj = 1; c.nsplit = 1; c.direct = 1; c.ostat = 1;
     return true;
 }
 static WgradCfg wgrad_cfg(int kind, int Ca, int Cb, int bD, int bH, int bW) {
@@ -697,23 +697,28 @@
         else if (bW > 4) { c.bz = 2; c.by = 8; c.bx = 8; }
         else { c.bz = 4; c.by = 8; c.bx = 4; }
     }
+    const int T = kind == 2 ? 8 : 27;
+    const long long bvox = (long long)bD * bH * bW, operand_bytes = ((kind == 0 ? 1 : 8) * bvox * Ca + bvox * Cb) * 2;
+    const long long row_bytes = (long long)T * Ca * Cb * 4;
+    const int tiles = ((bW + c.bx - 1) / c.bx) * ((bH + c.by - 1) / c.by) * ((bD + c.bz - 1) / c.bz);
     c.gy = (cat / c.pi) * (cbt / c.pj);
-    int tiles = ((bW + c.bx - 1) / c.bx) * ((bH + c.by - 1) / c.by) * ((bD + c.bz - 1) / c.bz);
-    int want = 512 / c.gy;
-    if (want < 1) want = 1;
-    c.nsplit = tiles < want ? tiles : want;
+    c.nsplit = wgrad_voxel_ranges(c.gy, tiles, wgrad_fill_blocks(0, 2));
+    if (wgrad_rows_outweigh_operands(c.nsplit, row_bytes, operand_bytes)) c.nsplit = wgrad_voxel_ranges(c.gy, tiles, wgrad_fill_blocks(1, 2));
+    if (c.nsplit == 1) c.direct = 1;
     return c;
 }
-static int s2w_rows_conv(const ConvGeom& g) { return (g.ks == 3 && g.stride == 2) ? s2_wgrad_splits(g.Cin, g.Cout, g.Do, g.Ho, g.Wo) : 0; }
-static int s2w_rows_convt(const ConvGeom& g) { return s2_wgrad_splits(g.Cout, g.Cin, g.D, g.H, g.W); }
+static int s2w_rows_conv(const ConvGeom& g, int polite) {
+    return (g.ks == 3 && g.stride == 2) ? s2_wgrad_splits(3, g.Cin, g.Cout, g.Do, g.Ho, g.Wo, polite) : 0;
+}
+static int s2w_rows_convt(const ConvGeom& g, int polite) { return s2_wgrad_splits(2, g.Cout, g.Cin, g.D, g.H, g.W, polite); }
 size_t mfma_wgrad_scratch_bytes(const ConvGeom& g, int polite) {
     if (size_t z = mfma_wgrad_z_scratch_bytes(g, polite)) return z;
-    if (int r = s2w_rows_conv(g)) return ((size_t)r * 27 * g.Cin * g.Cout + (size_t)r * g.Cout) * 4 + 256;
+    if (int r = s2w_rows_conv(g, polite)) return ((size_t)r * 27 * g.Cin * g.Cout + (size_t)r * g.Cout) * 4 + 256;
     WgradCfg c = wgrad_cfg(g.stride == 1 ? 0 : 1, g.Cin, g.Cout, g.Do, g.Ho, g.Wo);
     return ((size_t)c.nsplit * 27 * g.Cin * g.Cout + (size_t)c.nsplit * g.Cout) * 4 + 256;
 }
-size_t mfma_convt_wgrad_scratch_bytes(const ConvGeom& g) {
-    if (int r = s2w_rows_convt(g)) return ((size_t)r * 8 * g.Cin * g.Cout + (size_t)r * g.Cout) * 4 + 256;
+size_t mfma_convt_wgrad_scratch_bytes(const ConvGeom& g, int polite) {
+    if (int r = s2w_rows_convt(g, polite)) return ((size_t)r * 8 * g.Cin * g.Cout + (size_t)r * g.Cout) * 4 + 256;
     WgradCfg c = wgrad_cfg(2, g.Cout, g.Cin, g.D, g.H, g.W);
     return ((size_t)c.nsplit * 8 * g.Cin * g.Cout + (size_t)c.nsplit * g.Cout) * 4 + 256;
 }
@@ -752,28 +757,44 @@
 
 int mfma_conv_wgrad_splits(const ConvGeom& g, int polite) {
     if (int z = mfma_wgrad_z_splits(g, polite)) return z;
-    if (int r = s2w_rows_conv(g)) return r;
+    if (int r = s2w_rows_conv(g, polite)) return r;
     return wgrad_cfg(g.stride == 1 ? 0 : 1, g.Cin, g.Cout, g.Do, g.Ho, g.Wo).nsplit;
 }
-int mfma_convt_wgrad_splits(const ConvGeom& g) {
-    if (int r = s2w_rows_convt(g)) return r;
+int mfma_convt_wgrad_splits(const ConvGeom& g, int polite) {
+    if (int r = s2w_rows_convt(g, polite)) return r;
     return wgrad_cfg(2, g.Cout, g.Cin, g.D, g.H, g.W).nsplit;
 }
-bool mfma_conv_wgrad_direct(const ConvGeom& g) {
-    if (mfma_wgrad_z_splits(g) || s2w_rows_conv(g)) return false;
+bool mfma_conv_wgrad_direct(const ConvGeom& g, int polite) {
+    if (mfma_wgrad_z_splits(g, polite)) return mfma_wgrad_z_direct(g, polite);
+    if (s2w_rows_conv(g, polite)) return false;
     return wgrad_cfg(g.stride == 1 ? 0 : 1, g.Cin, g.Cout, g.Do, g.Ho, g.Wo).direct != 0;
 }
-bool mfma_convt_wgrad_direct(const ConvGeom& g) { return !s2w_rows_convt(g) && wgrad_cfg(2, g.Cout, g.Cin, g.D, g.H, g.W).direct != 0; }
+bool mfma_convt_wgrad_direct(const ConvGeom& g, int polite) { return !s2w_rows_convt(g, polite) && wgrad_cfg(2, g.Cout, g.Cin, g.D, g.H, g.W).direct != 0; }
+WgradGrid mfma_conv_wgrad_grid(const ConvGeom& g, int polite) {
+    WgradGrid w;
+    if (mfma_wgrad_z_grid(g, polite, w)) return w;
+    int gy = 0;
+    if (g.ks == 3 && g.stride == 2)
+        if (int r = s2_wgrad_splits(3, g.Cin, g.Cout, g.Do, g.Ho, g.Wo, polite, &gy)) return WgradGrid{2, r, gy, 0};
+    const WgradCfg c = wgrad_cfg(g.stride == 1 ? 0 : 1, g.Cin, g.Cout, g.Do, g.Ho, g.Wo);
+    return WgradGrid{3, c.nsplit, c.gy, c.direct};
+}
+WgradGrid mfma_convt_wgrad_grid(const ConvGeom& g, int polite) {
+    int gy = 0;
+    if (int r = s2_wgrad_splits(2, g.Cout, g.Cin, g.D, g.H, g.W, polite, &gy)) return WgradGrid{2, r, gy, 0};
+    const WgradCfg c = wgrad_cfg(2, g.Cout, g.Cin, g.D, g.H, g.W);
+    return WgradGrid{3, c.nsplit, c.gy, c.direct};
+}
 void launch_mfma_conv_wgrad(const ConvGeom& g, const SrcDesc* src, int nsrc, const void* dy, float* dw, float* db, void* scratch,
                             hipStream_t s, bool defer_reduce, int polite) {
     if (mfma_wgrad_z_supported(1, g, src, nsrc)) {
-        const int ns = launch_mfma_wgrad_z(g, src, nsrc, dy, db != nullptr, scratch, s, polite);
+        const int ns = launch_mfma_wgrad_z(g, src, nsrc, dy, db != nullptr, scratch, s, polite, dw, db);
         const float* slab = (const float*)scratch;
-        if (!defer_reduce)
+        if (!defer_reduce && !mfma_wgrad_z_direct(g, polite))
             wgrad_reduce(slab, db ? slab + (size_t)ns * 27 * g.Cin * g.Cout : nullptr, ns, (int64_t)27 * g.Cin * g.Cout, g.Cout, dw, db, s);
         return;
     }
-    if (s2w_rows_conv(g)) {
+    if (s2w_rows_conv(g, polite)) {
         const int ns = launch_s2_wgrad(3, src[0].ptr, nsrc > 1 ? src[1].ptr : nullptr, src[0].C, g.Cin, g.D, g.H, g.W, dy, g.Cout, g.Do, g.Ho, g.Wo,
                                        db != nullptr, 0, scratch, s, polite);
         const float* slab = (const float*)scratch;
@@ -790,8 +811,8 @@
     a.slab = (float*)scratch;
     a.bias_slab = db ? a.slab + (size_t)c.nsplit * 27 * g.Cin * g.Cout : nullptr;
     a.tiles_x = a.tiles_y = a.tiles_z = 0;
-    if (c.direct) {
-        a.slab = dw; a.bias_slab = db;
+    if (c.direct) { a.slab = dw; a.bias_slab = db; }
+    if (c.ostat) {
         if (g.stride == 1 && c.bx == 4) launch_wgrad_cfg<1, 3, 1, 4, 4, 4, 1, 1>(a, c, s);
         else if (g.stride == 1) launch_wgrad_cfg<1, 3, 1, 8, 8, 8, 1, 1>(a, c, s);
         else if (c.bx == 4) launch_wgrad_cfg<2, 3, 1, 4, 4, 4, 1, 1>(a, c, s);
@@ -807,12 +828,12 @@
         else if (g.Wo > 4) launch_wgrad_p<2, 3, 1, 2, 8, 8>(a, c, s);
         else launch_wgrad_p<2, 3, 1, 4, 8, 4>(a, c, s);
     }
-    if (!defer_reduce) wgrad_reduce(a.slab, a.bias_slab, c.nsplit, (int64_t)27 * g.Cin * g.Cout, g.Cout, dw, db, s);
+    if (!defer_reduce && !c.direct) wgrad_reduce(a.slab, a.bias_slab, c.nsplit, (int64_t)27 * g.Cin * g.Cout, g.Cout, dw, db, s);
 }
 
 void launch_mfma_convt_wgrad(const ConvGeom& g, const SrcDesc* src, const void* dy, float* dw, void* scratch, hipStream_t s, bool defer_reduce,
                              float* db, int polite) {
-    if (s2w_rows_convt(g)) {
+    if (s2w_rows_convt(g, polite)) {
         const int ns = launch_s2_wgrad(2, dy, nullptr, g.Cout, g.Cout, g.Do, g.Ho, g.Wo, src[0].ptr, g.Cin, g.D, g.H, g.W, db != nullptr, 1, scratch, s, polite);
         const float* slab = (const float*)scratch;
         if (!defer_reduce)
@@ -830,8 +851,8 @@
     a.slab = (float*)scratch;
     a.bias_slab = db ? a.slab + (size_t)c.nsplit * 8 * g.Cin * g.Cout : nullptr;
     a.tiles_x = a.tiles_y = a.tiles_z = 0;
-    if (c.direct) {
-        a.slab = dw; a.bias_slab = db;
+    if (c.direct) { a.slab = dw; a.bias_slab = db; }
+    if (c.ostat) {
         if (c.bx == 4) launch_wgrad_cfg<2, 2, 0, 4, 4, 4, 1, 1>(a, c, s);
         else launch_wgrad_cfg<2, 2, 0, 2, 8, 8, 1, 1>(a, c, s);
         return;
@@ -839,7 +860,7 @@
     if (g.W >= 12) launch_wgrad_p<2, 2, 0, 2, 4, 16>(a, c, s);
     else if (g.W > 4) launch_wgrad_p<2, 2, 0, 2, 8, 8>(a, c, s);
     else launch_wgrad_p<2, 2, 0, 4, 8, 4>(a, c, s);
-    if (!defer_reduce) wgrad_reduce(a.slab, a.bias_slab, c.nsplit, (int64_t)8 * g.Cin * g.Cout, g.Cout, dw, db, s);
-}
-
-}
+    if (!defer_reduce && !c.direct) wgrad_reduce(a.slab, a.bias_slab, c.nsplit, (int64_t)8 * g.Cin * g.Cout, g.Cout, dw, db, s);
+}
+
+}
diff --git a/unet-studio_amd/csrc/kernels_mfma_wgrad_z.hip b/unet-studio_amd/csrc/kernels_mfma_wgrad_z.hip
--- a/unet-studio_amd/csrc/kernels_mfma_wgrad_z.hip
+++ b/unet-studio_amd/csrc/kernels_mfma_wgrad_z.hip
@@ -1,6 +1,7 @@
 #include <cstdio>
 #include <type_traits>
 
+#include "conv_select.h"
 #include "mfma_util.h"
 #ifndef WZ_RD
 #define WZ_RD 4
@@ -324,7 +325,7 @@
     }
 }
 
-struct WgradZCfg { int bx, wk, pa, pb, by, cols_x, cols_y, nseg, zlen, gx, gy; };
+struct WgradZCfg { int bx, wk, pa, pb, by, cols_x, cols_y, nseg, zlen, gx, gy; bool direct; };
 
 static bool wgrad_z_cfg(const ConvGeom& g, WgradZCfg& c, int polite = 0) {
     if (sliding_window_off() || g.ks != 3 || g.stride != 1 || g.Cin % 16 || g.Cout % 16) return false;
@@ -346,16 +347,16 @@
     c.gy = (cat / c.pa) * (cbt / c.pb);
     const int cols = c.cols_x * c.cols_y;
     const int nwaves = c.wk * c.pa * c.pb;
-    int want = nwaves == 4 ? (polite ? 256 : 512) : 256;
-    want /= c.gy;
-    if (want < 1) want = 1;
-    int nseg = (want + cols - 1) / cols;
-    if (nseg < 1) nseg = 1;
+    const long long vox = (long long)g.D * g.H * g.W;
+    const bool one = wgrad_one_range(cols, vox * (g.Cin + g.Cout) * 2, (long long)27 * g.Cin * g.Cout * 4);
+    const int want = wgrad_voxel_ranges(c.gy, one ? 1 : 1 << 30, nwaves == 4 ? wgrad_fill_blocks(polite, 2) : wgrad_fill_blocks(1, 1));
+    const int nseg = (want + cols - 1) / cols;
     int zlen = (g.D + nseg - 1) / nseg;
     if (zlen < 4) zlen = 4;
     if (zlen > g.D) zlen = g.D;
     c.nseg = (g.D + zlen - 1) / zlen; c.zlen = zlen;
     c.gx = cols * c.nseg;
+    c.direct = c.gx == 1 && nwaves == 4;
     return true;
 }
 bool mfma_wgrad_z_supported(int dtype, const ConvGeom& g, const SrcDesc* src, int nsrc) {
@@ -368,6 +369,16 @@
 int mfma_wgrad_z_splits(const ConvGeom& g, int polite) {
     WgradZCfg c;
     return wgrad_z_cfg(g, c, polite) ? c.gx : 0;
+}
+bool mfma_wgrad_z_direct(const ConvGeom& g, int polite) {
+    WgradZCfg c;
+    return wgrad_z_cfg(g, c, polite) && c.direct;
+}
+bool mfma_wgrad_z_grid(const ConvGeom& g, int polite, WgradGrid& w) {
+    WgradZCfg c;
+    if (!wgrad_z_cfg(g, c, polite)) return false;
+    w.kernel = 1; w.ranges = c.gx; w.groups = c.gy; w.direct = c.direct ? 1 : 0;
+    return true;
 }
 size_t mfma_wgrad_z_scratch_bytes(const ConvGeom& g, int polite) {
     WgradZCfg c;
@@ -388,16 +399,17 @@
 }
 
 int launch_mfma_wgrad_z(const ConvGeom& g, const SrcDesc* src, int nsrc, const void* dy, bool want_bias, void* scratch, hipStream_t s,
-                        int polite) {
+                        int polite, float* dw, float* db) {
     WgradZCfg c;
     if (!wgrad_z_cfg(g, c, polite)) return 0;
+    if (c.direct && (!dw || (want_bias && !db))) { fprintf(stderr, "launch_mfma_wgrad_z: a one-range launch needs the gradient buffers\n"); abort(); }
     WgradZArgs a;
     a.g = g; a.nasrc = nsrc; a.asrc[0] = src[0]; if (nsrc > 1) a.asrc[1] = src[1];
     a.dy = dy;
-    a.slab = (float*)scratch;
-    a.bias_slab = want_bias ? a.slab + (size_t)c.gx * 27 * g.Cin * g.Cout : nullptr;
+    a.slab = c.direct ? dw : (float*)scratch;
+    a.bias_slab = !want_bias ? nullptr : (c.direct ? db : a.slab + (size_t)c.gx * 27 * g.Cin * g.Cout);
     a.cols_x = c.cols_x; a.cols_y = c.cols_y; a.nseg = c.nseg; a.zlen = c.zlen;
-    if (launch_wgrad_zd(g, src, nsrc, dy, a.slab, a.bias_slab, c.wk, c.pa, c.pb, c.cols_x, c.cols_y, c.nseg, c.zlen, c.gx, c.gy, s, polite)) return c.gx;
+    if (launch_wgrad_zd(g, src, nsrc, dy, a.slab, a.bias_slab, c.wk, c.pa, c.pb, c.cols_x, c.cols_y, c.nseg, c.zlen, c.gx, c.gy, s, polite, c.direct)) return c.gx;
     if (c.pa == 2 && c.pb == 2) launch_wz<32, 2, 2, 2>(a, c, s, polite);
     else if (c.pa == 2) launch_wz<32, 4, 2, 1>(a, c, s, polite);
     else launch_wz<32, 4, 1, 2>(a, c, s, polite);
diff --git a/unet-studio_amd/csrc/kernels_mfma_wgrad_zd.hip b/unet-studio_amd/csrc/kernels_mfma_wgrad_zd.hip
--- a/unet-studio_amd/csrc/kernels_mfma_wgrad_zd.hip
+++ b/unet-studio_amd/csrc/kernels_mfma_wgrad_zd.hip
@@ -24,6 +24,7 @@
     float* slab;
     float* bias_slab;
     int cols_x, cols_y, nseg, zlen;
+    int direct;
 };
 
 #define WZD_DMA(src, dst)                                                                                                    \
@@ -228,9 +229,23 @@
             }
             __syncthreads();
             float* base = a.slab + (size_t)blockIdx.x * T * g.Cin * g.Cout + ((size_t)(cbB + pr % PB) * 16 * g.Cin + (size_t)(caB + pr / PB) * 16) * T;
-            for (int q = tid; q < 16 * 108; q += 256) {
-                const int row = q / 108, c4 = q % 108;
-                *(f32x4*)(base + (size_t)row * g.Cin * T + c4 * 4) = *(const f32x4*)(stg + row * RP + c4 * 4);
+            if (!a.direct) {
+                for (int q = tid; q < 16 * 108; q += 256) {
+                    const int row = q / 108, c4 = q % 108;
+                    *(f32x4*)(base + (size_t)row * g.Cin * T + c4 * 4) = *(const f32x4*)(stg + row * RP + c4 * 4);
+                }
+            } else if ((reinterpret_cast<uintptr_t>(base) & 15) == 0) {
+                for (int q = tid; q < 16 * 108; q += 256) {
+                    const int row = q / 108, c4 = q % 108;
+                    f32x4* d = (f32x4*)(base + (size_t)row * g.Cin * T + c4 * 4);
+                    const f32x4 o = *d, v = *(const f32x4*)(stg + row * RP + c4 * 4);
+                    *d = f32x4{o[0] + v[0], o[1] + v[1], o[2] + v[2], o[3] + v[3]};
+                }
+            } else {
+                for (int q = tid; q < 16 * 16 * T; q += 256) {
+                    const int row = q / (16 * T), c = q % (16 * T);
+                    base[(size_t)row * g.Cin * T + c] += stg[row * RP + c];
+                }
             }
         }
     }
@@ -255,7 +270,8 @@
 #pragma unroll
             for (int w = 0; w < 4; ++w)
                 if ((w * UPWB) / (NVB * 2) == tile) sacc += bred[(w * 2 + half) * 8 + e];
-            a.bias_slab[(size_t)blockIdx.x * g.Cout + (cbB + tile) * 16 + half * 8 + e] = sacc;
+            float* d = a.bias_slab + (size_t)blockIdx.x * g.Cout + (cbB + tile) * 16 + half * 8 + e;
+            *d = a.direct ? *d + sacc : sacc;
         }
     }
 }
@@ -269,13 +285,14 @@
     k_mfma_wgrad_zd<WK, PA, PB><<<dim3((unsigned)gx, (unsigned)gy), 256, polite_lds(lds, polite), s>>>(a);
 }
 bool launch_wgrad_zd(const ConvGeom& g, const SrcDesc* src, int nsrc, const void* dy, float* slab, float* bias_slab, int wk, int pa, int pb, int cols_x,
-                     int cols_y, int nseg, int zlen, int gx, int gy, hipStream_t s, int polite) {
+                     int cols_y, int nseg, int zlen, int gx, int gy, hipStream_t s, int polite, bool direct) {
     if (wk * pa * pb != 4) return false;
+    if (direct && gx != 1) { fprintf(stderr, "launch_wgrad_zd: only a one-range launch can add into the gradient\n"); abort(); }
     for (int k = 0; k < nsrc; ++k) if ((size_t)g.H * g.W * src[k].C * 2 >= ((size_t)1 << 40)) return false;
     WgradZdArgs a;
     a.g = g; a.nasrc = nsrc; a.asrc[0] = src[0]; if (nsrc > 1) a.asrc[1] = src[1];
     a.dy = dy; a.slab = slab; a.bias_slab = bias_slab;
-    a.cols_x = cols_x; a.cols_y = cols_y; a.nseg = nseg; a.zlen = zlen;
+    a.cols_x = cols_x; a.cols_y = cols_y; a.nseg = nseg; a.zlen = zlen; a.direct = direct ? 1 : 0;
     if (wk == 2 && pa == 2) launch_zd_t<2, 2, 1>(a, gx, gy, s, polite);
     else if (wk == 2) launch_zd_t<2, 1, 2>(a, gx, gy, s, polite);
     else launch_zd_t<4, 1, 1>(a, gx, gy, s, polite);
diff --git a/unet-studio_amd/csrc/mfma_util.h b/unet-studio_amd/csrc/mfma_util.h
--- a/unet-studio_amd/csrc/mfma_util.h
+++ b/unet-studio_amd/csrc/mfma_util.h
@@ -89,6 +89,6 @@
 int conv_z16_blocks(const MfmaConvArgs& a, ZWork* zw = nullptr);
 int launch_conv_z32(const MfmaConvArgs& a, hipStream_t s);
 bool launch_wgrad_zd(const ConvGeom& g, const SrcDesc* src, int nsrc, const void* dy, float* slab, float* bias_slab, int wk, int pa, int pb, int cols_x,
-                     int cols_y, int nseg, int zlen, int gx, int gy, hipStream_t s, int polite);
+                     int cols_y, int nseg, int zlen, int gx, int gy, hipStream_t s, int polite, bool direct);
 
 }
diff --git a/unet-studio_amd/engine.py b/unet-studio_amd/engine.py
--- a/unet-studio_amd/engine.py
+++ b/unet-studio_amd/engine.py
@@ -85,6 +85,9 @@
      _i, _i, _i, _i, _i, _vp, _vp)
 _sig("unet_op_conv3d_bwd_data_norm", _i, _i, _vp, _vp, _vp, _i, _vp, _vp, _vp, _i, _vp, _vp, _vp, _i, _i, _i, _i, _i, _vp, _vp)
 _sig("unet_op_conv3d_bwd_weight", _i, _i, _i, _vp, _vp, _vp, _vp, _i, _i, _i, _i, _i, _i, _i, _vp, _vp)
+_sig("unet_op_conv3d_bwd_weight_cat", _i, _i, _i, _vp, _i, _vp, _i, _vp, _vp, _vp, _i, _i, _i, _i, _i, _i, _vp, _vp)
+_sig("unet_plan_wgrad_grid", _i, _vp, _i, C.POINTER(_i))
+_sig("unet_op_wgrad_split",_i, _i, _i, _i, _i, _i, _i, _i, _i, _i, _i, C.POINTER(_i))
 _sig("unet_op_convt_fwd", _i, _i, _i, _vp, _vp, _vp, _vp, _i, _i, _i, _i, _i, _vp, _vp)
 _sig("unet_op_convt_bwd_data", _i, _i, _i, _vp, _vp, _vp, _i, _i, _i, _i, _i, _vp, _vp)
 _sig("unet_op_convt_bwd_weight", _i, _i, _i, _vp, _vp, _vp, _vp, _i, _i, _i, _i, _i, _vp, _vp)
@@ -98,6 +101,7 @@
     "unet_plan_flops", "unet_plan_describe", "unet_plan_op_count", "unet_plan_op_info", "unet_profile_begin", "unet_profile_end", "unet_forward", "unet_backward", "unet_backward_part", "unet_plan_backward_buckets", "unet_loss_scratch_bytes", "unet_loss", "unet_forward_loss", "unet_forward_loss_mode", "unet_sum_buffers",
     "unet_sgd_step", "unet_sgd_step_packed", "unet_pack_filters", "unet_stream_create_cu_range", "unet_stream_destroy", "unet_plan_side_cu_range", "unet_set_error", "unet_comm_unique_id", "unet_comm_create", "unet_comm_create_all", "unet_comm_destroy", "unet_comm_rank",
     "unet_allreduce_grads", "unet_allreduce_grads_all", "unet_comm_broadcast", "unet_comm_join", "unet_op_scratch_bytes", "unet_op_conv_choice", "unet_op_conv3d_fwd", "unet_op_conv3d_fwd_fused", "unet_op_conv3d_pack", "unet_op_conv3d_fwd_packed", "unet_op_conv3d_bwd_data", "unet_op_conv3d_fwd_norm", "unet_op_conv3d_bwd_data_norm", "unet_op_conv3d_bwd_weight",
+    "unet_op_conv3d_bwd_weight_cat", "unet_op_wgrad_split", "unet_plan_wgrad_grid",
     "unet_op_convt_fwd", "unet_op_convt_bwd_data", "unet_op_convt_bwd_weight", "unet_op_pack_ndhwc", "unet_op_unpack_ncdhw",
 ]
 
```
